# kkrt-labs/stwo-brainfuck

Measured on AMD Instinct MI355X. Metric: trace cells committed+proved/sec, higher is better.
Workload: dtype u32 (M31 / QM31 modular arithmetic)

## Files before the change

bindings/rust/bfhip_sys.rs:

```rust
#![allow(non_camel_case_types, dead_code)]
use std::ffi::{c_char, c_void};

#[repr(C)] pub struct BfhipCtx { _private: [u8; 0] }
#[repr(C)] pub struct BfhipTrace { _private: [u8; 0] }
#[repr(C)] #[derive(Clone, Copy, Default, Debug, PartialEq, Eq)] pub struct BfhipConventions { pub merkle_node_hash: u32, pub mix_u64: u32, pub logup_mask_order: u32, pub merkle_channel: u32, pub reserved: [u32; 4] }
#[repr(C)] #[derive(Clone, Copy, Debug, PartialEq, Eq)] pub struct BfhipPcsConfig { pub pow_bits: u32, pub log_blowup_factor: u32, pub log_last_layer_degree_bound: u32, pub n_queries: u32, pub reserved: [u32; 4] }
#[repr(C)] #[derive(Clone, Copy, Default, Debug, PartialEq, Eq)] pub struct BfhipCheckReport { pub component: u32, pub log_size: u32, pub n_bad_cells: u64, pub first_bad_cell: u64, pub first_bad_constraint: i32, pub first_bad_value: [u32; 4], pub bad_per_constraint: [u64; 16], pub claimed_sum: [u32; 4], pub reserved: [u32; 3] }
#[repr(C)] #[derive(Clone, Copy, Default, Debug, PartialEq, Eq)] pub struct BfhipRelationEntry { pub relation: u32, pub n_words: u32, pub tuple: [u32; 7], pub net: u32, pub n_yield: u64, pub n_use: u64, pub n_other: u64, pub first_yield_table: i32, pub first_use_table: i32, pub first_yield_row: u64, pub first_use_row: u64, pub reserved: [u32; 2] }
#[repr(C)] #[derive(Clone, Copy, Default, Debug, PartialEq, Eq)] pub struct BfhipRelationReport { pub relation: u32, pub n_words: u32, pub n_entries: u64, pub n_tuples: u64, pub n_unbalanced: u64, pub n_reported: u64, pub reserved: [u32; 2] }
#[repr(C)] #[derive(Clone, Copy, Debug)] pub struct BfhipRelationTable { pub component: i32, pub log_size: u32, pub main_rows_h: *const *const u32 }
#[repr(C)] pub struct BfhipLocalGroup { _private: [u8; 0] }
#[repr(C)] pub struct BfhipPool { _private: [u8; 0] }
#[repr(C)] #[derive(Clone, Copy, Debug)] pub struct BfhipPoolResult { pub ticket: u64, pub user_tag: u64, pub status: i32, pub worker: u32, pub flags: u32, pub log_max_rows: u32, pub proof_json: *mut c_char, pub proof_len: usize, pub error: *mut c_char, pub seconds_queued: f64, pub seconds_proving: f64, pub reserved: [u64; 2] }
#[repr(C)] #[derive(Clone, Copy, Debug)] pub struct BfhipPreflightReport { pub ran: u32, pub rejected: u32, pub n_bad_components: i32, pub n_entries: u32, pub logup_total: [u32; 4], pub components: [BfhipCheckReport; 13], pub relations: [BfhipRelationReport; 3], pub entries: [BfhipRelationEntry; 12], pub seconds: f64, pub reserved: [u64; 3] }
pub const BFHIP_TRACE_REJECTED: i32 = -3;
pub const BFHIP_JOB_CANCELLED: i32 = -2;
pub const BFHIP_POOL_MAX_OUTSTANDING: u32 = 4096;

#[link(name = "bfhip")]
extern "C" {
    pub fn bfhip_last_error() -> *const c_char;
    pub fn bfhip_device_count() -> i32;
    pub fn bfhip_device_memory(device_id: i32, free_bytes: *mut u64, total_bytes: *mut u64) -> i32;
    pub fn bfhip_ctx_create(device_id: i32, max_log_domain: u32, out: *mut *mut BfhipCtx) -> i32;
    pub fn bfhip_ctx_destroy(ctx: *mut BfhipCtx) -> i32;
    pub fn bfhip_ctx_sync(ctx: *mut BfhipCtx) -> i32;
    pub fn bfhip_ctx_set_overlap(ctx: *mut BfhipCtx, mask: u32) -> i32;
    pub fn bfhip_ctx_memory(ctx: *mut BfhipCtx, out: *mut u64) -> i32;
    pub fn bfhip_ctx_set_sync_policy(ctx: *mut BfhipCtx, blocking: i32) -> i32;
    pub fn bfhip_ctx_set_mailbox(ctx: *mut BfhipCtx, mode: i32, timeout_ms: u32, test_delay_ms: i32) -> i32;
    pub fn bfhip_ctx_set_conventions(ctx: *mut BfhipCtx, conv: *const BfhipConventions) -> i32;
    pub fn bfhip_ctx_get_conventions(ctx: *mut BfhipCtx, out: *mut BfhipConventions) -> i32;
    pub fn bfhip_ctx_set_pcs_config(ctx: *mut BfhipCtx, pcs: *const BfhipPcsConfig) -> i32;
    pub fn bfhip_ctx_get_pcs_config(ctx: *mut BfhipCtx, out: *mut BfhipPcsConfig) -> i32;
    pub fn bfhip_malloc(ctx: *mut BfhipCtx, bytes: usize, out_d: *mut *mut c_void) -> i32;
    pub fn bfhip_free(ctx: *mut BfhipCtx, ptr_d: *mut c_void) -> i32;
    pub fn bfhip_upload(ctx: *mut BfhipCtx, dst_d: *mut c_void, src_h: *const c_void, bytes: usize) -> i32;
    pub fn bfhip_download(ctx: *mut BfhipCtx, dst_h: *mut c_void, src_d: *const c_void, bytes: usize) -> i32;
    pub fn bfhip_memset_zero(ctx: *mut BfhipCtx, dst_d: *mut c_void, bytes: usize) -> i32;
    pub fn bfhip_twiddles(ctx: *mut BfhipCtx, tw_d: *mut *const u32, itw_d: *mut *const u32, root_log: *mut u32) -> i32;
    pub fn bfhip_interpolate(ctx: *mut BfhipCtx, src_cols_h: *const *mut u32, dst_cols_h: *const *mut u32, n_cols: u32, log_size: u32, replicated: i32) -> i32;
    pub fn bfhip_evaluate(ctx: *mut BfhipCtx, coeff_cols_h: *const *mut u32, dst_cols_h: *const *mut u32, n_cols: u32, log_size: u32, log_eval: u32, replicated: i32) -> i32;
    pub fn bfhip_is_first_coeffs(ctx: *mut BfhipCtx, log_min: u32, log_max: u32, dst_cols_h: *const *mut u32) -> i32;
    pub fn bfhip_broadcast16(ctx: *mut BfhipCtx, rows_d: *const u32, dst_d: *mut u32, n_rows: usize) -> i32;
    pub fn bfhip_bit_reverse(ctx: *mut BfhipCtx, src_d: *const u32, dst_d: *mut u32, log_size: u32) -> i32;
    pub fn bfhip_batch_inverse_m31(ctx: *mut BfhipCtx, src_d: *const u32, dst_d: *mut u32, n: usize) -> i32;
    pub fn bfhip_batch_inverse_qm31(ctx: *mut BfhipCtx, src_d: *const *const u32, dst_d: *const *mut u32, n: usize) -> i32;
    pub fn bfhip_accumulate(ctx: *mut BfhipCtx, dst_d: *mut u32, src_d: *const u32, n: usize) -> i32;
    pub fn bfhip_eval_at_point(ctx: *mut BfhipCtx, coeffs_d: *const u32, log_size: u32, replicated: i32, point_h: *const u32, out_h: *mut u32) -> i32;
    pub fn bfhip_merkle_commit_layer(ctx: *mut BfhipCtx, log_size: u32, prev_layer_d: *const c_void, cols_h: *const *const u32, col_shifts_h: *const u32, n_cols: u32, out_hashes_d: *mut c_void) -> i32;
    pub fn bfhip_merkle_commit_layer_poseidon252(ctx: *mut BfhipCtx, log_size: u32, prev_layer_d: *const c_void, cols_h: *const *const u32, col_shifts_h: *const u32, n_cols: u32, out_hashes_d: *mut c_void) -> i32;
    pub fn bfhip_hades_permutation(ctx: *mut BfhipCtx, in_h: *const u32, out_h: *mut u32) -> i32;
    pub fn bfhip_fold_line(ctx: *mut BfhipCtx, src_d: *const *const u32, dst_d: *const *mut u32, log_size: u32, alpha_h: *const u32) -> i32;
    pub fn bfhip_fold_circle_into_line(ctx: *mut BfhipCtx, dst_d: *const *mut u32, src_d: *const *const u32, log_size: u32, alpha_h: *const u32) -> i32;
    pub fn bfhip_fri_fold_leaf(ctx: *mut BfhipCtx, src_d: *const *const u32, quot_d: *const *const u32, dst_d: *const *mut u32, log_size: u32, alpha_h: *const u32, out_hashes_d: *mut c_void) -> i32;
    pub fn bfhip_grind(ctx: *mut BfhipCtx, digest_h: *const u8, pow_bits: u32, nonce: *mut u64) -> i32;
    pub fn bfhip_grind_poseidon252(ctx: *mut BfhipCtx, digest_h: *const u8, pow_bits: u32, start_nonce: u64, nonce: *mut u64, tried: *mut u64) -> i32;
    pub fn bfhip_gather(ctx: *mut BfhipCtx, col_d: *const u32, idx_h: *const u64, n: usize, out_h: *mut u32) -> i32;
    pub fn bfhip_component_shape(component: i32, n_main_cols: *mut u32, n_logup_cols: *mut u32, n_constraints: *mut u32) -> i32;
    pub fn bfhip_logup_generate(ctx: *mut BfhipCtx, component: i32, log_size: u32, main_rows_h: *const *const u32, lookup_h: *const u32, out_cols_h: *const *mut u32, claimed_sum_h: *mut u32) -> i32;
    pub fn bfhip_eval_constraints(ctx: *mut BfhipCtx, component: i32, log_size: u32, is_first_d: *const u32, main_lde_h: *const *const u32, main_shifts_h: *const u32, inter_lde_h: *const *const u32, inter_shifts_h: *const u32, lookup_h: *const u32, claimed_sum_h: *const u32, coeffs_h: *const u32, acc_d: *const *mut u32) -> i32;
    pub fn bfhip_check_constraints(ctx: *mut BfhipCtx, component: i32, log_size: u32, main_rows_h: *const *const u32, logup_cols_h: *const *const u32, lookup_h: *const u32, claimed_sum_h: *const u32, out: *mut BfhipCheckReport) -> i32;
    pub fn bfhip_accumulate_quotients(ctx: *mut BfhipCtx, log_size: u32, cols_h: *const *const u32, col_shifts_h: *const u32, n_cols: u32, n_samples_h: *const u32, sample_points_h: *const u32, sample_values_h: *const u32, random_coeff_h: *const u32, out_d: *const *mut u32) -> i32;
    pub fn bfhip_prove_brainfuck(ctx: *mut BfhipCtx, code: *const c_char, input_h: *const u8, n_input: usize, log_max_rows: u32, proof_json: *mut *mut c_char, proof_len: *mut usize, transcript: *mut *mut c_char, phase_seconds: *mut f64) -> i32;
    pub fn bfhip_free_host(p: *mut c_void);
    pub fn bfhip_ctx_last_proof_flags(ctx: *mut BfhipCtx, flags: *mut u32) -> i32;
    pub fn bfhip_local_group_create(count: u32, out: *mut *mut BfhipLocalGroup) -> i32;
    pub fn bfhip_local_group_destroy(group: *mut BfhipLocalGroup) -> i32;
    pub fn bfhip_ctx_join_local_group(ctx: *mut BfhipCtx, group: *mut BfhipLocalGroup, rank: u32) -> i32;
    pub fn bfhip_rccl_unique_id(id: *mut u8) -> i32;
    pub fn bfhip_ctx_join_rccl_group(ctx: *mut BfhipCtx, id: *const u8, rank: u32, count: u32) -> i32;
    pub fn bfhip_ctx_leave_group(ctx: *mut BfhipCtx) -> i32;
    pub fn bfhip_ctx_set_shard_policy(ctx: *mut BfhipCtx, policy: i32) -> i32;
    pub fn bfhip_ctx_group_stats(ctx: *mut BfhipCtx, out: *mut u64) -> i32;
    pub fn bfhip_ctx_group_times(ctx: *mut BfhipCtx, out_ms: *mut f64) -> i32;
    pub fn bfhip_ctx_group_latency(ctx: *mut BfhipCtx, reset: i32, out_us: *mut f64) -> i32;
    pub fn bfhip_rccl_exchange_raw(id: *const u8, rank: u32, count: u32, n_sends: u32, send_peer: *const u32, send_ptr: *const *mut c_void, send_bytes: *const usize, n_recvs: u32, recv_peer: *const u32, recv_ptr: *const *mut c_void, recv_bytes: *const usize, stats_out: *mut u64) -> i32;
    pub fn bfhip_rccl_selftest(ctx: *mut BfhipCtx) -> i32;
    pub fn bfhip_ctx_group_info(ctx: *mut BfhipCtx, rank: *mut u32, count: *mut u32, transport: *mut *const c_char) -> i32;
    pub fn bfhip_ctx_reuse_preprocessed(ctx: *mut BfhipCtx, on: i32) -> i32;
    pub fn bfhip_trace_create(ctx: *mut BfhipCtx, code: *const c_char, input_h: *const u8, n_input: usize, out: *mut *mut BfhipTrace, log_sizes: *mut u32, n_steps: *mut u64, main_cells: *mut u64, interaction_cells: *mut u64) -> i32;
    pub fn bfhip_trace_create_ram(ctx: *mut BfhipCtx, code: *const c_char, input_h: *const u8, n_input: usize, ram_size: usize, out: *mut *mut BfhipTrace, log_sizes: *mut u32, n_steps: *mut u64, main_cells: *mut u64, interaction_cells: *mut u64) -> i32;
    pub fn bfhip_trace_create_from_registers(ctx: *mut BfhipCtx, trace7_h: *const u32, n_rows: usize, code_words_h: *const u32, n_code: usize, out: *mut *mut BfhipTrace, log_sizes: *mut u32, main_cells: *mut u64, interaction_cells: *mut u64) -> i32;
    pub fn bfhip_trace_destroy(ctx: *mut BfhipCtx, trace: *mut BfhipTrace) -> i32;
    pub fn bfhip_ctx_set_table_builder(ctx: *mut BfhipCtx, on_gpu: i32) -> i32;
    pub fn bfhip_trace_column(ctx: *mut BfhipCtx, trace: *const BfhipTrace, component: u32, column: u32, out_h: *mut u32, cap: usize, n_rows: *mut usize) -> i32;
    pub fn bfhip_prove_trace(ctx: *mut BfhipCtx, trace: *const BfhipTrace, log_max_rows: u32, proof_json: *mut *mut c_char, proof_len: *mut usize, transcript: *mut *mut c_char, phase_seconds: *mut f64) -> i32;
    pub fn bfhip_prove_registers(ctx: *mut BfhipCtx, trace7_h: *const u32, n_rows: usize, code_words_h: *const u32, n_code: usize, log_max_rows: u32, proof_json: *mut *mut c_char, proof_len: *mut usize, transcript: *mut *mut c_char, phase_seconds: *mut f64) -> i32;
    pub fn bfhip_trace_check(ctx: *mut BfhipCtx, trace: *const BfhipTrace, lookup_h: *const u32, out: *mut BfhipCheckReport, logup_total_h: *mut u32, n_bad_components: *mut i32) -> i32;
    pub fn bfhip_relation_summary(ctx: *mut BfhipCtx, tables: *const BfhipRelationTable, n_tables: u32, out: *mut BfhipRelationReport, entries_h: *mut BfhipRelationEntry, cap_per_relation: u32) -> i32;
    pub fn bfhip_trace_relations(ctx: *mut BfhipCtx, trace: *const BfhipTrace, out: *mut BfhipRelationReport, entries_h: *mut BfhipRelationEntry, cap_per_relation: u32) -> i32;
    pub fn bfhip_ctx_set_preflight(ctx: *mut BfhipCtx, on: i32) -> i32;
    pub fn bfhip_ctx_get_preflight(ctx: *mut BfhipCtx, on: *mut i32) -> i32;
    pub fn bfhip_ctx_last_preflight(ctx: *mut BfhipCtx, out: *mut BfhipPreflightReport) -> i32;
    pub fn bfhip_format_preflight(rep: *const BfhipPreflightReport, buf: *mut c_char, cap: usize, need: *mut usize) -> i32;
    pub fn bfhip_pool_create(device_id: i32, n_in_flight: u32, max_log_domain: u32, out: *mut *mut BfhipPool) -> i32;
    pub fn bfhip_pool_destroy(pool: *mut BfhipPool) -> i32;
    pub fn bfhip_pool_size(pool: *mut BfhipPool, n_in_flight: *mut u32) -> i32;
    pub fn bfhip_pool_ctx(pool: *mut BfhipPool, i: u32, out: *mut *mut BfhipCtx) -> i32;
    pub fn bfhip_pool_set_conventions(pool: *mut BfhipPool, conv: *const BfhipConventions) -> i32;
    pub fn bfhip_pool_set_preprocessed(pool: *mut BfhipPool, mode: i32) -> i32;
    pub fn bfhip_pool_set_pcs_config(pool: *mut BfhipPool, pcs: *const BfhipPcsConfig) -> i32;
    pub fn bfhip_pool_set_preflight(pool: *mut BfhipPool, on: i32) -> i32;
    pub fn bfhip_prove_batch(pool: *mut BfhipPool, traces: *const *const BfhipTrace, n: u32, log_max_rows: u32, proofs_json: *mut *mut c_char, proof_lens: *mut usize, statuses: *mut i32, seconds: *mut f64) -> i32;
    pub fn bfhip_prove_batch_brainfuck(pool: *mut BfhipPool, codes: *const *const c_char, inputs_h: *const *const u8, n_inputs: *const usize, n: u32, log_max_rows: u32, proofs_json: *mut *mut c_char, proof_lens: *mut usize, statuses: *mut i32, seconds: *mut f64) -> i32;
    pub fn bfhip_pool_submit_trace(pool: *mut BfhipPool, trace: *const BfhipTrace, log_max_rows: u32, user_tag: u64, ticket: *mut u64) -> i32;
    pub fn bfhip_pool_submit_brainfuck(pool: *mut BfhipPool, code: *const c_char, input_h: *const u8, n_input: usize, log_max_rows: u32, user_tag: u64, ticket: *mut u64) -> i32;
    pub fn bfhip_pool_submit_registers(pool: *mut BfhipPool, trace7_h: *const u32, n_rows: usize, code_words_h: *const u32, n_code: usize, log_max_rows: u32, user_tag: u64, ticket: *mut u64) -> i32;
    pub fn bfhip_pool_wait(pool: *mut BfhipPool, timeout_ms: u32, out: *mut BfhipPoolResult) -> i32;
    pub fn bfhip_pool_outstanding(pool: *mut BfhipPool, queued: *mut u32, running: *mut u32, finished_not_taken: *mut u32) -> i32;
    pub fn bfhip_pool_cancel(pool: *mut BfhipPool, ticket: u64) -> i32;
    pub fn bfhip_verify_brainfuck(proof_json: *const c_char, proof_len: usize, log_max_rows: u32, err: *mut c_char, err_cap: usize) -> i32;
    pub fn bfhip_verify_brainfuck_conv(proof_json: *const c_char, proof_len: usize, log_max_rows: u32, conv: *const BfhipConventions, err: *mut c_char, err_cap: usize) -> i32;
    pub fn bfhip_verify_brainfuck_pcs(proof_json: *const c_char, proof_len: usize, log_max_rows: u32, conv: *const BfhipConventions, pcs: *const BfhipPcsConfig, err: *mut c_char, err_cap: usize) -> i32;
    pub fn bfhip_host_compile(code: *const c_char, out: *mut u32, cap: usize, n: *mut usize) -> i32;
    pub fn bfhip_host_run(code: *const c_char, input_h: *const u8, n_input: usize, out: *mut u8, out_cap: usize, n_out: *mut usize, trace7: *mut u32, trace_cap_rows: usize, n_rows: *mut usize) -> i32;
    pub fn bfhip_host_run_ram(code: *const c_char, input_h: *const u8, n_input: usize, ram_size: usize, out: *mut u8, out_cap: usize, n_out: *mut usize, trace7: *mut u32, trace_cap_rows: usize, n_rows: *mut usize) -> i32;
    pub fn bfhip_host_table(trace7: *const u32, n_trace: usize, code: *const u32, n_code: usize, component: i32, out_row_major: *mut u32, cap: usize, n_rows: *mut usize, n_cols: *mut usize) -> i32;
    pub fn bfhip_profile_enable(ctx: *mut BfhipCtx, mode: i32) -> i32;
    pub fn bfhip_profile_reset(ctx: *mut BfhipCtx) -> i32;
    pub fn bfhip_profile_report(ctx: *mut BfhipCtx, json: *mut *mut c_char) -> i32;
    pub fn bfhip_clock_probe(ctx: *mut BfhipCtx, seconds: f64, out: *mut f64) -> i32;
    pub fn bfhip_clock_probe_mix(ctx: *mut BfhipCtx, seconds: f64, log_nodes: u32, out: *mut f64) -> i32;
}
```

include/bfhip.h:

```cpp
#ifndef BFHIP_H
#define BFHIP_H
#include <stdint.h>
#include <stddef.h>

#ifdef __cplusplus
extern "C" {
#endif

typedef struct bfhip_ctx bfhip_ctx;
typedef struct bfhip_trace bfhip_trace;

enum { BFHIP_MERKLE_STWO_COMPRESS = 0, BFHIP_MERKLE_RFC7693 = 1 };
enum { BFHIP_MIX_U64_COMPRESS = 0, BFHIP_MIX_U64_HASH = 1 };
enum { BFHIP_LOGUP_MASK_CUR_PREV = 0, BFHIP_LOGUP_MASK_PREV_CUR = 1 };
enum { BFHIP_CHANNEL_BLAKE2S = 0, BFHIP_CHANNEL_POSEIDON252 = 1 };
typedef struct bfhip_conventions {
    uint32_t merkle_node_hash;
    uint32_t mix_u64;
    uint32_t logup_mask_order;
    uint32_t merkle_channel;
    uint32_t reserved[4];
} bfhip_conventions;

const char* bfhip_last_error(void);
int32_t bfhip_device_count(void);
int32_t bfhip_device_memory(int32_t device_id, uint64_t* free_bytes, uint64_t* total_bytes);

int32_t bfhip_ctx_create(int32_t device_id, uint32_t max_log_domain, bfhip_ctx** out);
int32_t bfhip_ctx_destroy(bfhip_ctx* ctx);
int32_t bfhip_ctx_sync(bfhip_ctx* ctx);
int32_t bfhip_ctx_set_overlap(bfhip_ctx* ctx, uint32_t mask);
int32_t bfhip_ctx_memory(bfhip_ctx* ctx, uint64_t out[4]);
int32_t bfhip_ctx_set_sync_policy(bfhip_ctx* ctx, int32_t blocking);
int32_t bfhip_ctx_set_mailbox(bfhip_ctx* ctx, int32_t mode, uint32_t timeout_ms, int32_t test_delay_ms);

int32_t bfhip_ctx_set_conventions(bfhip_ctx* ctx, const bfhip_conventions* conv);
int32_t bfhip_ctx_get_conventions(bfhip_ctx* ctx, bfhip_conventions* out);

enum { BFHIP_MAX_QUERIES = 256, BFHIP_MAX_LOG_BLOWUP = 16, BFHIP_MAX_POW_BITS = 32 };
typedef struct bfhip_pcs_config {
    uint32_t pow_bits;
    uint32_t log_blowup_factor;
    uint32_t log_last_layer_degree_bound;
    uint32_t n_queries;
    uint32_t reserved[4];
} bfhip_pcs_config;
int32_t bfhip_ctx_set_pcs_config(bfhip_ctx* ctx, const bfhip_pcs_config* pcs);
int32_t bfhip_ctx_get_pcs_config(bfhip_ctx* ctx, bfhip_pcs_config* out);

int32_t bfhip_malloc(bfhip_ctx* ctx, size_t bytes, void** out_d);
int32_t bfhip_free(bfhip_ctx* ctx, void* ptr_d);
int32_t bfhip_upload(bfhip_ctx* ctx, void* dst_d, const void* src_h, size_t bytes);
int32_t bfhip_download(bfhip_ctx* ctx, void* dst_h, const void* src_d, size_t bytes);
int32_t bfhip_memset_zero(bfhip_ctx* ctx, void* dst_d, size_t bytes);

int32_t bfhip_twiddles(bfhip_ctx* ctx, const uint32_t** tw_d, const uint32_t** itw_d, uint32_t* root_log);

int32_t bfhip_interpolate(bfhip_ctx* ctx, uint32_t* const* src_cols_h, uint32_t* const* dst_cols_h, uint32_t n_cols, uint32_t log_size, int32_t replicated);
int32_t bfhip_evaluate(bfhip_ctx* ctx, uint32_t* const* coeff_cols_h, uint32_t* const* dst_cols_h, uint32_t n_cols, uint32_t log_size, uint32_t log_eval, int32_t replicated);

int32_t bfhip_is_first_coeffs(bfhip_ctx* ctx, uint32_t log_min, uint32_t log_max, uint32_t* const* dst_cols_h);


int32_t bfhip_broadcast16(bfhip_ctx* ctx, const uint32_t* rows_d, uint32_t* dst_d, size_t n_rows);
int32_t bfhip_bit_reverse(bfhip_ctx* ctx, const uint32_t* src_d, uint32_t* dst_d, uint32_t log_size);
int32_t bfhip_batch_inverse_m31(bfhip_ctx* ctx, const uint32_t* src_d, uint32_t* dst_d, size_t n);
int32_t bfhip_batch_inverse_qm31(bfhip_ctx* ctx, const uint32_t* const src_d[4], uint32_t* const dst_d[4], size_t n);
int32_t bfhip_accumulate(bfhip_ctx* ctx, uint32_t* dst_d, const uint32_t* src_d, size_t n);
int32_t bfhip_eval_at_point(bfhip_ctx* ctx, const uint32_t* coeffs_d, uint32_t log_size, int32_t replicated, const uint32_t point_h[8], uint32_t out_h[4]);
int32_t bfhip_merkle_commit_layer(bfhip_ctx* ctx, uint32_t log_size, const void* prev_layer_d, const uint32_t* const* cols_h, const uint32_t* col_shifts_h,
                                  uint32_t n_cols, void* out_hashes_d);
int32_t bfhip_merkle_commit_layer_poseidon252(bfhip_ctx* ctx, uint32_t log_size, const void* prev_layer_d, const uint32_t* const* cols_h,
                                             const uint32_t* col_shifts_h, uint32_t n_cols, void* out_hashes_d);
int32_t bfhip_hades_permutation(bfhip_ctx* ctx, const uint32_t in_h[24], uint32_t out_h[24]);
int32_t bfhip_fold_line(bfhip_ctx* ctx, const uint32_t* const src_d[4], uint32_t* const dst_d[4], uint32_t log_size, const uint32_t alpha_h[4]);
int32_t bfhip_fold_circle_into_line(bfhip_ctx* ctx, uint32_t* const dst_d[4], const uint32_t* const src_d[4], uint32_t log_size, const uint32_t alpha_h[4]);
int32_t bfhip_fri_fold_leaf(bfhip_ctx* ctx, const uint32_t* const src_d[4], const uint32_t* const quot_d[4], uint32_t* const dst_d[4], uint32_t log_size,
                            const uint32_t alpha_h[4], void* out_hashes_d);
int32_t bfhip_grind(bfhip_ctx* ctx, const uint8_t digest_h[32], uint32_t pow_bits, uint64_t* nonce);
int32_t bfhip_grind_poseidon252(bfhip_ctx* ctx, const uint8_t digest_h[32], uint32_t pow_bits, uint64_t start_nonce,
                                uint64_t* nonce, uint64_t* tried);
int32_t bfhip_gather(bfhip_ctx* ctx, const uint32_t* col_d, const uint64_t* idx_h, size_t n, uint32_t* out_h);


int32_t bfhip_component_shape(int32_t component, uint32_t* n_main_cols, uint32_t* n_logup_cols, uint32_t* n_constraints);
int32_t bfhip_logup_generate(bfhip_ctx* ctx, int32_t component, uint32_t log_size, const uint32_t* const* main_rows_h, const uint32_t lookup_h[24],
                             uint32_t* const* out_cols_h, uint32_t claimed_sum_h[4]);
int32_t bfhip_eval_constraints(bfhip_ctx* ctx, int32_t component, uint32_t log_size, const uint32_t* is_first_d, const uint32_t* const* main_lde_h,
                               const uint32_t* main_shifts_h, const uint32_t* const* inter_lde_h, const uint32_t* inter_shifts_h, const uint32_t lookup_h[24],
                               const uint32_t claimed_sum_h[4], const uint32_t* coeffs_h, uint32_t* const acc_d[4]);
typedef struct bfhip_check_report {
    uint32_t component, log_size;
    uint64_t n_bad_cells;
    uint64_t first_bad_cell;
    int32_t  first_bad_constraint;
    uint32_t first_bad_value[4];
    uint64_t bad_per_constraint[16];
    uint32_t claimed_sum[4];
    uint32_t reserved[3];
} bfhip_check_report;
int32_t bfhip_check_constraints(bfhip_ctx* ctx, int32_t component, uint32_t log_size, const uint32_t* const* main_rows_h, const uint32_t* const* logup_cols_h,
                                const uint32_t lookup_h[24], const uint32_t claimed_sum_h[4], bfhip_check_report* out);
int32_t bfhip_accumulate_quotients(bfhip_ctx* ctx, uint32_t log_size, const uint32_t* const* cols_h, const uint32_t* col_shifts_h, uint32_t n_cols,
                                   const uint32_t* n_samples_h, const uint32_t* sample_points_h, const uint32_t* sample_values_h,
                                   const uint32_t random_coeff_h[4], uint32_t* const out_d[4]);

int32_t bfhip_prove_brainfuck(bfhip_ctx* ctx, const char* code, const uint8_t* input_h, size_t n_input, uint32_t log_max_rows,
                              char** proof_json, size_t* proof_len, char** transcript, double* phase_seconds);
void bfhip_free_host(void* p);
int32_t bfhip_ctx_last_proof_flags(bfhip_ctx* ctx, uint32_t* flags);
typedef struct bfhip_local_group bfhip_local_group;
int32_t bfhip_local_group_create(uint32_t count, bfhip_local_group** out);
int32_t bfhip_local_group_destroy(bfhip_local_group* group);
int32_t bfhip_ctx_join_local_group(bfhip_ctx* ctx, bfhip_local_group* group, uint32_t rank);
int32_t bfhip_rccl_unique_id(uint8_t id[128]);
int32_t bfhip_ctx_join_rccl_group(bfhip_ctx* ctx, const uint8_t id[128], uint32_t rank, uint32_t count);
int32_t bfhip_ctx_leave_group(bfhip_ctx* ctx);
int32_t bfhip_ctx_set_shard_policy(bfhip_ctx* ctx, int32_t policy);
int32_t bfhip_ctx_group_stats(bfhip_ctx* ctx, uint64_t out[4]);
int32_t bfhip_ctx_group_times(bfhip_ctx* ctx, double out_ms[3]);
int32_t bfhip_ctx_group_latency(bfhip_ctx* ctx, int32_t reset, double out_us[21]);
int32_t bfhip_rccl_exchange_raw(const uint8_t id[128], uint32_t rank, uint32_t count, uint32_t n_sends, const uint32_t* send_peer, void* const* send_ptr,
                                const size_t* send_bytes, uint32_t n_recvs, const uint32_t* recv_peer, void* const* recv_ptr, const size_t* recv_bytes,
                                uint64_t stats_out[4]);
int32_t bfhip_rccl_selftest(bfhip_ctx* ctx);
int32_t bfhip_ctx_group_info(bfhip_ctx* ctx, uint32_t* rank, uint32_t* count, const char** transport);

int32_t bfhip_ctx_reuse_preprocessed(bfhip_ctx* ctx, int32_t on);

int32_t bfhip_trace_create(bfhip_ctx* ctx, const char* code, const uint8_t* input_h, size_t n_input, bfhip_trace** out,
                           uint32_t log_sizes[13], uint64_t* n_steps, uint64_t* main_cells, uint64_t* interaction_cells);
int32_t bfhip_trace_create_ram(bfhip_ctx* ctx, const char* code, const uint8_t* input_h, size_t n_input, size_t ram_size, bfhip_trace** out,
                               uint32_t log_sizes[13], uint64_t* n_steps, uint64_t* main_cells, uint64_t* interaction_cells);
int32_t bfhip_trace_create_from_registers(bfhip_ctx* ctx, const uint32_t* trace7_h, size_t n_rows, const uint32_t* code_words_h, size_t n_code,
                                          bfhip_trace** out, uint32_t log_sizes[13], uint64_t* main_cells, uint64_t* interaction_cells);
int32_t bfhip_trace_destroy(bfhip_ctx* ctx, bfhip_trace* trace);
int32_t bfhip_ctx_set_table_builder(bfhip_ctx* ctx, int32_t on_gpu);
int32_t bfhip_trace_column(bfhip_ctx* ctx, const bfhip_trace* trace, uint32_t component, uint32_t column, uint32_t* out_h, size_t cap, size_t* n_rows);
int32_t bfhip_prove_trace(bfhip_ctx* ctx, const bfhip_trace* trace, uint32_t log_max_rows, char** proof_json, size_t* proof_len,
                          char** transcript, double* phase_seconds);
int32_t bfhip_prove_registers(bfhip_ctx* ctx, const uint32_t* trace7_h, size_t n_rows, const uint32_t* code_words_h, size_t n_code,
                              uint32_t log_max_rows, char** proof_json, size_t* proof_len, char** transcript, double* phase_seconds);
// ... 106 lines not shown
```

stwo-brainfuck_amd/__init__.py:

```python
import ctypes
import os
import weakref

import numpy as np

_HERE = os.path.dirname(os.path.abspath(__file__))
_LIB_PATH = os.environ.get("BFHIP_LIBRARY") or os.path.join(_HERE, "libbfhip.so")
TESTHOOKS_LIBRARY = os.path.join(_HERE, "libbfhip_testhooks.so")
_lib = None

P = (1 << 31) - 1


class BfhipError(RuntimeError):
    pass


def lib():
    global _lib
    if _lib is None:
        if not os.path.exists(_LIB_PATH):
            raise BfhipError(f"{_LIB_PATH} is missing: build it with __graft_entry__.build(); there is no CPU fallback")
        _lib = ctypes.CDLL(_LIB_PATH)
        _lib.bfhip_last_error.restype = ctypes.c_char_p
# ... 229 lines not shown
    if not getattr(check, "ran", True):
        return ["preflight: did not run"]
    if not getattr(check, "rejected", not check.ok):
        return ["preflight: ok"]
    what = []
    if check.n_bad_components:
        what.append("%d of 13 components violate their constraints" % check.n_bad_components)
    if any(check.logup_total):
        what.append("the logUp total is not zero")
    return ["TraceRejected: " + " and ".join(what)] + check.failures() + (relations.lines() if relations is not None else [])


def format_preflight(report):
    need = ctypes.c_size_t()
    rc = lib().bfhip_format_preflight(ctypes.byref(report), None, ctypes.c_size_t(0), ctypes.byref(need))
    if rc not in (0, -2):
        raise BfhipError(lib().bfhip_last_error().decode())
    buf = ctypes.create_string_buffer(need.value)
    _check(lib().bfhip_format_preflight(ctypes.byref(report), buf, ctypes.c_size_t(need.value), None))
    return buf.value.decode()


def _relation_result(call, max_entries, table_names=None):
    reps = (RelationReport * 3)()
    ents = (RelationEntry * (3 * max_entries))() if max_entries else None
    _check(call(reps, ents, max_entries))
    return RelationResult([r.as_dict() for r in reps], [ents[k * max_entries + i].as_dict() for k in range(3) for i in range(reps[k].n_reported)], table_names)


class Context:

    def __init__(self, device_id=0, max_log_domain=22):
        self._h = ctypes.c_void_p()
        _check(lib().bfhip_ctx_create(device_id, max_log_domain, ctypes.byref(self._h)))
        self.max_log_domain = max_log_domain
        _live_contexts.add(self)
        if _default_conventions != (0, 0, 0, 0):
            self.set_conventions(*_default_conventions)

    def close(self):
        if self._h:
            lib().bfhip_ctx_destroy(self._h)
            self._h = ctypes.c_void_p()

    def __del__(self):
        try:
            self.close()
        except Exception:
            pass

    def sync(self):
        _check(lib().bfhip_ctx_sync(self._h))

    def set_conventions(self, merkle_node_hash=0, mix_u64=0, logup_mask_order=0, merkle_channel=0):
        cv = Conventions(merkle_node_hash, mix_u64, logup_mask_order, merkle_channel)
        _check(lib().bfhip_ctx_set_conventions(self._h, ctypes.byref(cv)))

    def get_conventions(self):
        cv = Conventions()
        _check(lib().bfhip_ctx_get_conventions(self._h, ctypes.byref(cv)))
        return cv.merkle_node_hash, cv.mix_u64, cv.logup_mask_order, cv.merkle_channel

    def set_pcs_config(self, pcs_config=None):
        _check(lib().bfhip_ctx_set_pcs_config(self._h, _pcs_ref(pcs_config)))

    def pcs_config(self):
        out = PcsConfig()
        _check(lib().bfhip_ctx_get_pcs_config(self._h, ctypes.byref(out)))
        return out

    def set_overlap(self, mask=1):
        _check(lib().bfhip_ctx_set_overlap(self._h, int(mask)))

    def set_sync_policy(self, blocking):
        _check(lib().bfhip_ctx_set_sync_policy(self._h, 1 if blocking else 0))

    def set_mailbox(self, mode=-2, timeout_ms=0, test_delay_ms=-1):
        _check(lib().bfhip_ctx_set_mailbox(self._h, int(mode), int(timeout_ms), int(test_delay_ms)))

    def last_proof_flags(self):
        f = ctypes.c_uint32()
        _check(lib().bfhip_ctx_last_proof_flags(self._h, ctypes.byref(f)))
        return {"mailbox_order": bool(f.value & 1), "kept_preprocessed": bool(f.value & 2), "shared_preprocessed": bool(f.value & 4), "replicated_transforms": bool(f.value & 8),
                "split_gather": bool(f.value & 16), "fri_fold_leaf": bool(f.value & 32), "preflight": bool(f.value & 64)}

    def set_preflight(self, on=True):
        _check(lib().bfhip_ctx_set_preflight(self._h, 1 if on else 0))

    def preflight(self):
        on = ctypes.c_int32()
        _check(lib().bfhip_ctx_get_preflight(self._h, ctypes.byref(on)))
        return bool(on.value)

    def last_preflight_report(self):
        rep = PreflightReport()
        _check(lib().bfhip_ctx_last_preflight(self._h, ctypes.byref(rep)))
        return rep

    def last_preflight(self):
        return self.last_preflight_report().results()

    def clock_probe(self, seconds=0.6):
        out = (ctypes.c_double * 6)()
        _check(lib().bfhip_clock_probe(self._h, ctypes.c_double(seconds), out))
        return dict(zip(("ghz", "ghz_min", "ghz_max", "G_compressions_per_s", "launches", "ms_per_launch"), [float(v) for v in out]))

    def clock_probe_mix(self, seconds=0.5, log_nodes=22):
        out = (ctypes.c_double * 6)()
        _check(lib().bfhip_clock_probe_mix(self._h, ctypes.c_double(seconds), int(log_nodes), out))
        d = dict(zip(("ghz", "G_compressions_per_s", "launches", "us_per_launch", "sampler_spanned_the_window", "sampler_seconds"), [float(v) for v in out]))
        d["sampler_spanned_the_window"] = bool(d["sampler_spanned_the_window"])
        return d

    def memory(self):
        out = (ctypes.c_uint64 * 4)()
        _check(lib().bfhip_ctx_memory(self._h, out))
        return dict(zip(("arena_reserved", "arena_peak", "twiddles", "arena_in_use"), [int(v) for v in out]))

    def set_table_builder(self, on_gpu=True):
        _check(lib().bfhip_ctx_set_table_builder(self._h, int(on_gpu)))

    def join_local_group(self, group, rank):
        _check(lib().bfhip_ctx_join_local_group(self._h, group._h, rank))
        self._group = group

    def join_rccl_group(self, unique_id: bytes, rank, count):
        if len(unique_id) != 128:
            raise BfhipError("an RCCL unique id has 128 bytes")
        _check(lib().bfhip_ctx_join_rccl_group(self._h, unique_id, rank, count))

    def set_shard_policy(self, policy=-1):
        _check(lib().bfhip_ctx_set_shard_policy(self._h, int(policy)))

    def leave_group(self):
        _check(lib().bfhip_ctx_leave_group(self._h))
        self._group = None

    def group_stats(self):
        out = (ctypes.c_uint64 * 4)()
        _check(lib().bfhip_ctx_group_stats(self._h, out))
        return dict(zip(("all_gathers", "max_reduces", "exchanges", "bytes_sent"), [int(v) for v in out]))

    def group_times(self):
        out = (ctypes.c_double * 3)()
        _check(lib().bfhip_ctx_group_times(self._h, out))
        return dict(zip(("all_gather_ms", "max_reduce_ms", "exchange_ms"), [float(v) for v in out]))

    def group_latency(self, reset=False):
        out = (ctypes.c_double * 21)()
        _check(lib().bfhip_ctx_group_latency(self._h, 1 if reset else 0, out))
        res = {}
        for k, name in enumerate(("all_gather", "max_reduce", "exchange")):
            v = [float(x) for x in out[7 * k:7 * k + 7]]
            res[name] = {"count": int(v[0]), "gpu_us": {"p50": round(v[1], 1), "p90": round(v[2], 1), "max": round(v[3], 1)},
                         "host_us": {"p50": round(v[4], 1), "p90": round(v[5], 1), "max": round(v[6], 1)}}
        return res

    def group_info(self):
        r, n, t = ctypes.c_uint32(), ctypes.c_uint32(), ctypes.c_char_p()
        _check(lib().bfhip_ctx_group_info(self._h, ctypes.byref(r), ctypes.byref(n), ctypes.byref(t)))
        return r.value, n.value, (t.value or b"").decode()

    def malloc(self, nbytes):
        p = ctypes.c_void_p()
        _check(lib().bfhip_malloc(self._h, ctypes.c_size_t(nbytes), ctypes.byref(p)))
        return p.value

    def free(self, ptr):
        _check(lib().bfhip_free(self._h, ctypes.c_void_p(ptr)))

    def upload(self, arr):
        arr = np.ascontiguousarray(arr)
        ptr = self.malloc(arr.nbytes)
        _check(lib().bfhip_upload(self._h, ctypes.c_void_p(ptr), arr.ctypes.data_as(ctypes.c_void_p), ctypes.c_size_t(arr.nbytes)))
        return ptr

    def download(self, ptr, n, dtype=np.uint32):
        out = np.empty(n, dtype=dtype)
        _check(lib().bfhip_download(self._h, out.ctypes.data_as(ctypes.c_void_p), ctypes.c_void_p(ptr), ctypes.c_size_t(out.nbytes)))
        return out

    @staticmethod
    def _ptr_array(ptrs):
        return (ctypes.c_void_p * len(ptrs))(*ptrs)

    def interpolate(self, src_ptrs, dst_ptrs, log_size, replicated=False):
        _check(lib().bfhip_interpolate(self._h, self._ptr_array(src_ptrs), self._ptr_array(dst_ptrs), len(src_ptrs), log_size, int(replicated)))

    def evaluate(self, coeff_ptrs, dst_ptrs, log_size, log_eval, replicated=False):
        _check(lib().bfhip_evaluate(self._h, self._ptr_array(coeff_ptrs), self._ptr_array(dst_ptrs), len(coeff_ptrs), log_size, log_eval, int(replicated)))

    def is_first_coeffs(self, log_min, log_max, dst_ptrs):
        arr = (ctypes.c_void_p * len(dst_ptrs))(*[p or None for p in dst_ptrs])
        _check(lib().bfhip_is_first_coeffs(self._h, log_min, log_max, arr))

    def eval_at_point(self, coeff_ptr, log_size, point8, replicated=False):
        pt = (ctypes.c_uint32 * 8)(*[int(v) for v in point8])
        out = (ctypes.c_uint32 * 4)()
        _check(lib().bfhip_eval_at_point(self._h, ctypes.c_void_p(coeff_ptr), log_size, int(replicated), pt, out))
        return list(out)

    def broadcast16(self, rows_ptr, dst_ptr, n_rows):
        _check(lib().bfhip_broadcast16(self._h, ctypes.c_void_p(rows_ptr), ctypes.c_void_p(dst_ptr), ctypes.c_size_t(n_rows)))

    def bit_reverse(self, src_ptr, dst_ptr, log_size):
        _check(lib().bfhip_bit_reverse(self._h, ctypes.c_void_p(src_ptr), ctypes.c_void_p(dst_ptr), log_size))

    def batch_inverse_m31(self, src_ptr, dst_ptr, n):
        _check(lib().bfhip_batch_inverse_m31(self._h, ctypes.c_void_p(src_ptr), ctypes.c_void_p(dst_ptr), ctypes.c_size_t(n)))

    def batch_inverse_qm31(self, src_ptrs, dst_ptrs, n):
        _check(lib().bfhip_batch_inverse_qm31(self._h, self._ptr_array(src_ptrs), self._ptr_array(dst_ptrs), ctypes.c_size_t(n)))

    def accumulate(self, dst_ptr, src_ptr, n):
        _check(lib().bfhip_accumulate(self._h, ctypes.c_void_p(dst_ptr), ctypes.c_void_p(src_ptr), ctypes.c_size_t(n)))

    def merkle_commit_layer(self, log_size, prev_ptr, col_ptrs, out_ptr, col_shifts=None):
        sh = None if col_shifts is None else (ctypes.c_uint32 * len(col_shifts))(*col_shifts)
        _check(lib().bfhip_merkle_commit_layer(self._h, log_size, ctypes.c_void_p(prev_ptr) if prev_ptr else None, self._ptr_array(col_ptrs), sh, len(col_ptrs), ctypes.c_void_p(out_ptr)))

    def merkle_commit_layer_poseidon252(self, log_size, prev_ptr, col_ptrs, out_ptr, col_shifts=None):
        sh = None if col_shifts is None else (ctypes.c_uint32 * len(col_shifts))(*col_shifts)
        _check(lib().bfhip_merkle_commit_layer_poseidon252(self._h, log_size, ctypes.c_void_p(prev_ptr) if prev_ptr else None, self._ptr_array(col_ptrs), sh, len(col_ptrs), ctypes.c_void_p(out_ptr)))

    def hades_permutation(self, state3):
        words = []
        for x in state3:
            words += [(int(x) >> (32 * i)) & 0xFFFFFFFF for i in range(8)]
        out = (ctypes.c_uint32 * 24)()
        _check(lib().bfhip_hades_permutation(self._h, (ctypes.c_uint32 * 24)(*words), out))
        return [sum(int(out[8 * k + i]) << (32 * i) for i in range(8)) for k in range(3)]

    def fold_line(self, src_ptrs, dst_ptrs, log_size, alpha4):
        _check(lib().bfhip_fold_line(self._h, self._ptr_array(src_ptrs), self._ptr_array(dst_ptrs), log_size, (ctypes.c_uint32 * 4)(*[int(v) for v in alpha4])))

    def fri_fold_leaf(self, src_ptrs, quot_ptrs, dst_ptrs, log_size, alpha4, out_ptr):
        _check(lib().bfhip_fri_fold_leaf(self._h, self._ptr_array(src_ptrs) if src_ptrs is not None else None, self._ptr_array(quot_ptrs) if quot_ptrs is not None else None,
                                         self._ptr_array(dst_ptrs), log_size, (ctypes.c_uint32 * 4)(*[int(v) for v in alpha4]), ctypes.c_void_p(out_ptr)))

    def fold_circle_into_line(self, dst_ptrs, src_ptrs, log_size, alpha4):
        _check(lib().bfhip_fold_circle_into_line(self._h, self._ptr_array(dst_ptrs), self._ptr_array(src_ptrs), log_size, (ctypes.c_uint32 * 4)(*[int(v) for v in alpha4])))

    def grind(self, digest32, pow_bits):
        nonce = ctypes.c_uint64()
        _check(lib().bfhip_grind(self._h, bytes(digest32), pow_bits, ctypes.byref(nonce)))
        return nonce.value

    def grind_poseidon252(self, digest32, pow_bits, start_nonce=0, with_tried=False):
        digest32 = bytes(digest32)
        if len(digest32) != 32:
            raise ValueError("grind_poseidon252: the digest is 32 bytes")
        nonce, tried = ctypes.c_uint64(), ctypes.c_uint64()
        _check(lib().bfhip_grind_poseidon252(self._h, digest32, ctypes.c_uint32(pow_bits), ctypes.c_uint64(start_nonce), ctypes.byref(nonce), ctypes.byref(tried)))
        return (nonce.value, tried.value) if with_tried else nonce.value

    def gather(self, col_ptr, indices):
        idx = np.ascontiguousarray(indices, dtype=np.uint64)
        out = np.empty(idx.size, dtype=np.uint32)
        _check(lib().bfhip_gather(self._h, ctypes.c_void_p(col_ptr), idx.ctypes.data_as(ctypes.c_void_p), ctypes.c_size_t(idx.size), out.ctypes.data_as(ctypes.c_void_p)))
        return out

    @staticmethod
    def _u32s(values):
        values = [int(v) for v in values]
        return (ctypes.c_uint32 * len(values))(*values)

    def logup_generate(self, component, log_size, main_row_ptrs, lookup24, out_col_ptrs):
        claimed = (ctypes.c_uint32 * 4)()
        _check(lib().bfhip_logup_generate(self._h, component, log_size, self._ptr_array(main_row_ptrs), self._u32s(lookup24), self._ptr_array(out_col_ptrs), claimed))
        return list(claimed)

    def eval_constraints(self, component, log_size, is_first_ptr, main_lde_ptrs, inter_lde_ptrs, lookup24, claimed4, coeffs, acc_ptrs, main_shifts=None, inter_shifts=None):
        _check(lib().bfhip_eval_constraints(self._h, component, log_size, ctypes.c_void_p(is_first_ptr), self._ptr_array(main_lde_ptrs),
# ... 189 lines not shown
        arr = (ctypes.c_void_p * max(n, 1))(*[t._h for t in traces])
        js, lens, st, sec = self._outputs(n, want_json)
        rc = lib().bfhip_prove_batch(self._h, arr, n, log_max_rows, js, lens, st, sec)
        return self._collect(rc, n, js, lens, st, sec, want_json)

    def prove_batch_brainfuck(self, programs, log_max_rows=24, want_json=True):
        n = len(programs)
        codes = (ctypes.c_char_p * max(n, 1))(*[c.encode() for c, _ in programs])
        bufs = [ctypes.create_string_buffer(bytes(i), max(len(i), 1)) for _, i in programs]
        inputs = (ctypes.c_void_p * max(n, 1))(*[ctypes.addressof(b) for b in bufs])
        nin = (ctypes.c_size_t * max(n, 1))(*[len(i) for _, i in programs])
        js, lens, st, sec = self._outputs(n, want_json)
        rc = lib().bfhip_prove_batch_brainfuck(self._h, codes, inputs, nin, n, log_max_rows, js, lens, st, sec)
        return self._collect(rc, n, js, lens, st, sec, want_json)


PHASES = ("preprocessed", "tables_host", "main_trace", "interaction", "composition", "oods", "quotients", "fri", "decommit", "total")


def prove_brainfuck(code, input_bytes=b"", ctx=None, log_max_rows=24, with_transcript=False, with_timings=False, pcs_config=None):
    own = ctx is None
    if own:
        blowup = 1 if pcs_config is None else pcs_config.log_blowup_factor
        ctx = Context(0, max_log_domain=log_max_rows + blowup + 1)
    try:
        if pcs_config is not None:
            ctx.set_pcs_config(pcs_config)
        js, n, tr = ctypes.c_void_p(), ctypes.c_size_t(), ctypes.c_void_p()
        times = (ctypes.c_double * 10)()
        _check_proof(lib().bfhip_prove_brainfuck(ctx._h, code.encode(), input_bytes, ctypes.c_size_t(len(input_bytes)), log_max_rows,
                                                 ctypes.byref(js), ctypes.byref(n), ctypes.byref(tr) if with_transcript else None, times), ctx)
        proof = ctypes.string_at(js, n.value)
        lib().bfhip_free_host(js)
        out = [proof]
        if with_transcript:
            t = ctypes.string_at(tr).decode()
            lib().bfhip_free_host(tr)
            out.append(dict(line.split(":") for line in t.strip().split("\n")))
        if with_timings:
            out.append(dict(zip(PHASES, list(times))))
        return out[0] if len(out) == 1 else tuple(out)
    finally:
        if own:
            ctx.close()


def prove_registers(rows, code_words, ctx=None, log_max_rows=24, with_transcript=False, with_timings=False):
    own = ctx is None
    if own:
        ctx = Context(0, max_log_domain=log_max_rows + 2)
    try:
        tr = np.ascontiguousarray(rows, dtype=np.uint32).reshape(-1, 7)
        code = np.ascontiguousarray(code_words, dtype=np.uint32)
        js, n, t = ctypes.c_void_p(), ctypes.c_size_t(), ctypes.c_void_p()
        times = (ctypes.c_double * 10)()
        _check_proof(lib().bfhip_prove_registers(ctx._h, tr.ctypes.data_as(ctypes.c_void_p), ctypes.c_size_t(tr.shape[0]), code.ctypes.data_as(ctypes.c_void_p),
                                                 ctypes.c_size_t(code.size), log_max_rows, ctypes.byref(js), ctypes.byref(n),
                                                 ctypes.byref(t) if with_transcript else None, times), ctx)
        proof = ctypes.string_at(js, n.value)
        lib().bfhip_free_host(js)
        out = [proof]
        if with_transcript:
            text = ctypes.string_at(t).decode()
            lib().bfhip_free_host(t)
            out.append(dict(line.split(":") for line in text.strip().split("\n")))
        if with_timings:
            out.append(dict(zip(PHASES, list(times))))
        return out[0] if len(out) == 1 else tuple(out)
    finally:
        if own:
            ctx.close()


def verify_brainfuck(proof_json: bytes, log_max_rows=24, conventions=None, pcs_config=None):
    err = ctypes.create_string_buffer(512)
    cv = ctypes.byref(Conventions(*(_default_conventions if conventions is None else conventions)))
    rc = lib().bfhip_verify_brainfuck_pcs(proof_json, ctypes.c_size_t(len(proof_json)), log_max_rows, cv, _pcs_ref(pcs_config), err,
                                          ctypes.c_size_t(512))
    if rc < 0:
        raise BfhipError(lib().bfhip_last_error().decode())
    return rc == 0, err.value.decode()


def host_compile(code):
    out = np.zeros(2 * len(code) + 4, dtype=np.uint32)
    n = ctypes.c_size_t()
    _check(lib().bfhip_host_compile(code.encode(), out.ctypes.data_as(ctypes.c_void_p), ctypes.c_size_t(out.size), ctypes.byref(n)))
    return out[: n.value].copy()


def host_run(code, input_bytes=b"", ram_size=0):
    n_out, n_rows = ctypes.c_size_t(), ctypes.c_size_t()
    args = (code.encode(), input_bytes, ctypes.c_size_t(len(input_bytes)), ctypes.c_size_t(ram_size))
    _check(lib().bfhip_host_run_ram(*args, None, ctypes.c_size_t(0), ctypes.byref(n_out), None, ctypes.c_size_t(0), ctypes.byref(n_rows)))
    out = (ctypes.c_ubyte * max(1, n_out.value))()
    rows = np.zeros((n_rows.value, 7), dtype=np.uint32)
    _check(lib().bfhip_host_run_ram(*args, out, ctypes.c_size_t(n_out.value), ctypes.byref(n_out), rows.ctypes.data_as(ctypes.c_void_p),
                                    ctypes.c_size_t(rows.shape[0]), ctypes.byref(n_rows)))
    return bytes(out[: n_out.value]), rows


class Trace:

    def __init__(self, ctx, code, input_bytes=b"", ram_size=0):
        self.ctx = ctx
        self._h = ctypes.c_void_p()
        ls = (ctypes.c_uint32 * 13)()
        steps, mc, ic = ctypes.c_uint64(), ctypes.c_uint64(), ctypes.c_uint64()
        _check(lib().bfhip_trace_create_ram(ctx._h, code.encode(), input_bytes, ctypes.c_size_t(len(input_bytes)), ctypes.c_size_t(ram_size),
                                            ctypes.byref(self._h), ls, ctypes.byref(steps), ctypes.byref(mc), ctypes.byref(ic)))
        self.log_sizes = list(ls)
        self.n_steps, self.main_cells, self.interaction_cells = steps.value, mc.value, ic.value

    @classmethod
    def from_registers(cls, ctx, trace7, code_words):
        self = cls.__new__(cls)
        self.ctx = ctx
        self._h = ctypes.c_void_p()
        tr = np.ascontiguousarray(trace7, dtype=np.uint32).reshape(-1, 7)
        code = np.ascontiguousarray(code_words, dtype=np.uint32)
        ls = (ctypes.c_uint32 * 13)()
        mc, ic = ctypes.c_uint64(), ctypes.c_uint64()
        _check(lib().bfhip_trace_create_from_registers(ctx._h, tr.ctypes.data_as(ctypes.c_void_p), ctypes.c_size_t(tr.shape[0]), code.ctypes.data_as(ctypes.c_void_p),
                                                       ctypes.c_size_t(code.size), ctypes.byref(self._h), ls, ctypes.byref(mc), ctypes.byref(ic)))
        self.log_sizes = list(ls)
        self.n_steps, self.main_cells, self.interaction_cells = tr.shape[0], mc.value, ic.value
        return self

    @property
    def cells(self):
        return self.main_cells + self.interaction_cells

    def prove(self, log_max_rows=24, want_json=True):
        js, n = ctypes.c_void_p(), ctypes.c_size_t()
        times = (ctypes.c_double * 10)()
        _check_proof(lib().bfhip_prove_trace(self.ctx._h, self._h, log_max_rows, ctypes.byref(js) if want_json else None, ctypes.byref(n), None, times), self.ctx)
        proof = None
        if want_json:
            proof = ctypes.string_at(js, n.value)
            lib().bfhip_free_host(js)
        return proof, dict(zip(PHASES, list(times)))

    def check(self, lookup24=None):
        reps = (CheckReport * 13)()
        total = (ctypes.c_uint32 * 4)()
        n_bad = ctypes.c_int32()
        _check(lib().bfhip_trace_check(self.ctx._h, self._h, None if lookup24 is None else Context._u32s(lookup24), reps, total, ctypes.byref(n_bad)))
        res = CheckResult(r.as_dict() for r in reps)
        res.logup_total, res.n_bad_components = tuple(int(v) for v in total), n_bad.value
        return res

    def relations(self, max_entries=64):
        return _relation_result(lambda reps, ents, cap: lib().bfhip_trace_relations(self.ctx._h, self._h, reps, ents, cap), max_entries)

    def column(self, component, column):
        n = ctypes.c_size_t()
        _check(lib().bfhip_trace_column(self.ctx._h, self._h, component, column, None, ctypes.c_size_t(0), ctypes.byref(n)))
        out = np.empty(n.value, dtype=np.uint32)
        _check(lib().bfhip_trace_column(self.ctx._h, self._h, component, column, out.ctypes.data_as(ctypes.c_void_p), ctypes.c_size_t(out.size), ctypes.byref(n)))
        return out

    def close(self):
        if self._h:
            lib().bfhip_trace_destroy(self.ctx._h, self._h)
            self._h = ctypes.c_void_p()
```

stwo-brainfuck_amd/csrc/api.hip:

```cpp
#include "../../include/bfhip.h"
#include "api_guard.h"
#include "prover.h"
#include <cstdlib>
#include "host/circle.h"
#include "host/quotients.h"
#include "host/hash.h"
#include <cstdio>
#include <vector>
#include <algorithm>
#include <chrono>

using namespace bf;

static thread_local std::string g_err;
void bfhip_set_error(const std::string& s) { g_err = s; }

namespace bf {

void Ctx::ensure_aux() { for (auto& a : aux) if (!a) BF_HIP(hipStreamCreateWithFlags(&a, hipStreamNonBlocking)); }
void Ctx::ensure_side() { if (!stream2) BF_HIP(hipStreamCreateWithFlags(&stream2, hipStreamNonBlocking)); }

void Ctx::init(int dev, u32 max_log_domain, const Ctx* tables_from) {
    int n = 0;
    if (hipGetDeviceCount(&n) != hipSuccess || n == 0) throw HipError("no HIP device: the bfhip backend has no CPU fallback");
// ... 415 lines not shown
    ctx->c.overlap_user_set = true;
    return 0;
    API_CATCH
}
int32_t bfhip_ctx_memory(bfhip_ctx* ctx, uint64_t out[4]) {
    API_CTX(ctx)
    if (!out) throw HipError("null argument");
    uint64_t reserved = 0;
    for (auto& ch : ctx->c.arena.chunks) reserved += ch.size;
    out[0] = reserved; out[1] = ctx->c.arena.peak; out[2] = ctx->c.owns_tables ? (uint64_t)(2 * sizeof(u32)) << ctx->c.tw_root_log : 0;
    return 0;
    API_CATCH
}
int32_t bfhip_ctx_get_conventions(bfhip_ctx* ctx, bfhip_conventions* out) {
    API_CTX(ctx)
    if (!out) throw HipError("null argument");
    bfhip_conventions r{};
    r.merkle_node_hash = ctx->c.conv.merkle_node_hash; r.mix_u64 = ctx->c.conv.mix_u64; r.logup_mask_order = ctx->c.conv.logup_mask_order; r.merkle_channel = ctx->c.conv.merkle_channel;
    *out = r;
    return 0;
    API_CATCH
}
int32_t bfhip_ctx_sync(bfhip_ctx* ctx) { API_CTX(ctx) ctx->c.sync(); return 0; API_CATCH }

int32_t bfhip_malloc(bfhip_ctx* ctx, size_t bytes, void** out_d) { API_CTX(ctx) BF_HIP(hipSetDevice(ctx->c.device)); BF_HIP(hipMalloc(out_d, bytes ? bytes : 4)); return 0; API_CATCH }
int32_t bfhip_free(bfhip_ctx* ctx, void* p) { API_CTX(ctx) (void)ctx; BF_HIP(hipFree(p)); return 0; API_CATCH }
int32_t bfhip_upload(bfhip_ctx* ctx, void* dst_d, const void* src_h, size_t bytes) {
    API_CTX(ctx) BF_HIP(hipMemcpyAsync(dst_d, src_h, bytes, hipMemcpyHostToDevice, ctx->c.stream)); ctx->c.sync(); return 0; API_CATCH
}
int32_t bfhip_download(bfhip_ctx* ctx, void* dst_h, const void* src_d, size_t bytes) {
    API_CTX(ctx) BF_HIP(hipMemcpyAsync(dst_h, src_d, bytes, hipMemcpyDeviceToHost, ctx->c.stream)); ctx->c.sync(); return 0; API_CATCH
}
int32_t bfhip_memset_zero(bfhip_ctx* ctx, void* dst_d, size_t bytes) { API_CTX(ctx) BF_HIP(hipMemsetAsync(dst_d, 0, bytes, ctx->c.stream)); return 0; API_CATCH }

int32_t bfhip_twiddles(bfhip_ctx* ctx, const uint32_t** tw_d, const uint32_t** itw_d, uint32_t* root_log) {
    API_CTX(ctx) if (!tw_d || !itw_d || !root_log) throw HipError("null argument"); *tw_d = ctx->c.d_tw; *itw_d = ctx->c.d_itw; *root_log = ctx->c.tw_root_log; return 0; API_CATCH
}

int32_t bfhip_interpolate(bfhip_ctx* ctx, uint32_t* const* src_cols_h, uint32_t* const* dst_cols_h, uint32_t n_cols, uint32_t log_size, int32_t replicated) {
    API_CTX(ctx)
    Ctx& c = ctx->c;
    if (replicated && log_size < 4) throw HipError("replicated columns need log_size >= 4");
    if (!replicated && log_size < 3) throw HipError("circle transforms need log_size >= 3");
    if (log_size > c.tw_root_log + 1) throw HipError("log_size exceeds the context's twiddle tree");
    u32 log = replicated ? log_size - 4 : log_size;
    c.stage_checkpoint();
    StageBatch sb(c);
    auto* s = c.stage(src_cols_h, n_cols);
    auto* d = c.stage(dst_cols_h, n_cols);
    const FftJob job{(const u32* const*)s, (u32* const*)d, n_cols, log, log, !replicated};
    FftPlan plan;
    fft_plan(plan, true, &job, 1, c.d_tw, c.d_itw, c.tw_root_log);
    plan.d_groups = c.stage(plan.groups.data(), plan.groups.size());
    sb.end();
    fft_run(c.stream, plan);
    BF_HIP(hipGetLastError());
    return 0;
    API_CATCH
}

int32_t bfhip_evaluate(bfhip_ctx* ctx, uint32_t* const* coeff_cols_h, uint32_t* const* dst_cols_h, uint32_t n_cols, uint32_t log_size, uint32_t log_eval, int32_t replicated) {
    API_CTX(ctx)
    Ctx& c = ctx->c;
    if (log_eval < log_size) throw HipError("log_eval < log_size");
    if (replicated && log_size < 4) throw HipError("replicated columns need log_size >= 4");
    if (!replicated && log_eval < 3) throw HipError("circle transforms need log_eval >= 3");
    if (log_eval > c.tw_root_log + 1) throw HipError("log_eval exceeds the context's twiddle tree");
    u32 sh = replicated ? 4 : 0;
    c.stage_checkpoint();
    StageBatch sb(c);
    auto* s = c.stage(coeff_cols_h, n_cols);
    auto* d = c.stage(dst_cols_h, n_cols);
    const FftJob job{(const u32* const*)s, (u32* const*)d, n_cols, log_eval - sh, log_size - sh, !replicated};
    FftPlan plan;
    fft_plan(plan, false, &job, 1, c.d_tw, c.d_itw, c.tw_root_log);
    plan.d_groups = c.stage(plan.groups.data(), plan.groups.size());
    sb.end();
    fft_run(c.stream, plan);
    BF_HIP(hipGetLastError());
    return 0;
    API_CATCH
}


int32_t bfhip_is_first_coeffs(bfhip_ctx* ctx, uint32_t log_min, uint32_t log_max, uint32_t* const* dst_cols_h) {
    API_CTX(ctx)
    if (!dst_cols_h) throw HipError("null argument");
    if (log_min < 4 || log_max < log_min || log_max - log_min >= 28) throw HipError("is_first_coeffs: need 4 <= log_min <= log_max < log_min + 28");
    if (log_max > ctx->c.tw_root_log + 1) throw HipError("log_max exceeds the context's twiddle tree");
    IsFirstCols a{}; a.log_min = log_min; a.log_max = log_max;
    for (u32 n = log_min; n <= log_max; n++) a.ptr[n - log_min] = dst_cols_h[n - log_min];
    is_first_coeffs(ctx->c.stream, a, ctx->c.d_itw, ctx->c.tw_root_log);
    BF_HIP(hipGetLastError());
    return 0;
    API_CATCH
}
int32_t bfhip_broadcast16(bfhip_ctx* ctx, const uint32_t* rows_d, uint32_t* dst_d, size_t n_rows) {
    API_CTX(ctx) broadcast16(ctx->c.stream, rows_d, dst_d, (u32)(n_rows * 16)); BF_HIP(hipGetLastError()); return 0; API_CATCH
}
int32_t bfhip_bit_reverse(bfhip_ctx* ctx, const uint32_t* src_d, uint32_t* dst_d, uint32_t log_size) {
    API_CTX(ctx) if (src_d == dst_d) throw HipError("bit_reverse is out of place"); bit_reverse(ctx->c.stream, src_d, dst_d, log_size); BF_HIP(hipGetLastError()); return 0; API_CATCH
}
int32_t bfhip_batch_inverse_m31(bfhip_ctx* ctx, const uint32_t* src_d, uint32_t* dst_d, size_t n) {
    API_CTX(ctx) batch_inverse_m31(ctx->c.stream, src_d, dst_d, (u32)n); BF_HIP(hipGetLastError()); return 0; API_CATCH
}
int32_t bfhip_batch_inverse_qm31(bfhip_ctx* ctx, const uint32_t* const src_d[4], uint32_t* const dst_d[4], size_t n) {
    API_CTX(ctx) batch_inverse_qm31(ctx->c.stream, src_d, dst_d, (u32)n); BF_HIP(hipGetLastError()); return 0; API_CATCH
}
int32_t bfhip_accumulate(bfhip_ctx* ctx, uint32_t* dst_d, const uint32_t* src_d, size_t n) {
    API_CTX(ctx) accumulate(ctx->c.stream, dst_d, src_d, (u32)n); BF_HIP(hipGetLastError()); return 0; API_CATCH
}
int32_t bfhip_eval_at_point(bfhip_ctx* ctx, const uint32_t* coeffs_d, uint32_t log_size, int32_t replicated, const uint32_t point_h[8], uint32_t out_h[4]) {
    API_CTX(ctx)
    Ctx& c = ctx->c;
    if (replicated && log_size < 4) throw HipError("replicated columns need log_size >= 4");
    c.stage_checkpoint();
    uint4 factors[32];
    Q31 x = q_make(point_h[0], point_h[1], point_h[2], point_h[3]);
    factors[0] = make_uint4(point_h[4], point_h[5], point_h[6], point_h[7]);
    for (u32 b = 1; b < 32; b++) { factors[b] = make_uint4(x.a.a, x.a.b, x.b.a, x.b.b); Q31 s = q_mul(x, x); x = q_subm(q_add(s, s), 1); }
    EvalJob job{coeffs_d, replicated ? log_size - 4 : log_size, 0, replicated ? 4u : 0u, 0};
    const EvalJob* dj = c.stage(&job, 1);
    const uint4* df = c.stage(factors, 32);
    u32 nchunks = job.log_n > 12 ? 1u << (job.log_n - 12) : 1u;
    uint4* partials = nullptr; uint4* dout = nullptr;
    BF_HIP(hipMalloc((void**)&partials, sizeof(uint4) * (nchunks + 1)));
    dout = partials + nchunks;
    eval_at_points(c.stream, dj, 1, nchunks, df, partials, dout);
    uint4 r;
    hipError_t e = hipMemcpyAsync(&r, dout, sizeof(uint4), hipMemcpyDeviceToHost, c.stream);
    if (e == hipSuccess) e = hipStreamSynchronize(c.stream);
    (void)hipFree(partials);
    BF_HIP(e);
    out_h[0] = r.x; out_h[1] = r.y; out_h[2] = r.z; out_h[3] = r.w;
    return 0;
    API_CATCH
}
int32_t bfhip_merkle_commit_layer(bfhip_ctx* ctx, uint32_t log_size, const void* prev_layer_d, const uint32_t* const* cols_h, const uint32_t* col_shifts_h,
                                  uint32_t n_cols, void* out_hashes_d) {
    API_CTX(ctx)
    Ctx& c = ctx->c;
    c.stage_checkpoint();
    std::vector<ColDesc> d(n_cols);
    for (u32 k = 0; k < n_cols; k++) d[k] = ColDesc{cols_h[k], col_shifts_h ? col_shifts_h[k] : 0u, 0};
    const ColDesc* dd = n_cols ? c.stage(d.data(), n_cols) : nullptr;
    merkle_layer(c.stream, out_hashes_d, prev_layer_d, dd, n_cols, log_size, 0.0, 0, 0, c.conv.merkle_node_hash);
    BF_HIP(hipGetLastError());
    return 0;
    API_CATCH
}
int32_t bfhip_merkle_commit_layer_poseidon252(bfhip_ctx* ctx, uint32_t log_size, const void* prev_layer_d, const uint32_t* const* cols_h, const uint32_t* col_shifts_h,
                                             uint32_t n_cols, void* out_hashes_d) {
    API_CTX(ctx)
    Ctx& c = ctx->c;
    c.stage_checkpoint();
    std::vector<ColDesc> d(n_cols);
    for (u32 k = 0; k < n_cols; k++) d[k] = ColDesc{cols_h[k], col_shifts_h ? col_shifts_h[k] : 0u, 0};
    const ColDesc* dd = n_cols ? c.stage(d.data(), n_cols) : nullptr;
    merkle_layer_poseidon(c.stream, out_hashes_d, prev_layer_d, dd, n_cols, log_size);
    BF_HIP(hipGetLastError());
    return 0;
    API_CATCH
}
int32_t bfhip_hades_permutation(bfhip_ctx* ctx, const uint32_t in_h[24], uint32_t out_h[24]) {
    API_CTX(ctx)
    Ctx& c = ctx->c;
// ... 378 lines not shown
```

stwo-brainfuck_amd/csrc/fft.hip:

```cpp
#include "kernels.h"
#include <cstdio>
#include <cstdlib>
#include <stdexcept>
#include <algorithm>
#include <vector>
#include <mutex>
#include <set>
#include <string>

namespace bf {

static constexpr int TILE_LOG = 12;
static constexpr int TILE = 1 << TILE_LOG;
static constexpr int CHUNK_LOG = 5;
static constexpr int STRIDED_K = TILE_LOG - CHUNK_LOG;
static constexpr int FFT_THREADS = 256;
__device__ __forceinline__ u32 scale_shift(u32 scale) { return (u32)__builtin_ctz(scale); }

__device__ __forceinline__ void point_of_index(u32 idx, const uint2* __restrict__ tlo, const uint2* __restrict__ thi, u32& x, u32& y) {
    uint2 a = tlo[idx & 0xffffu], b = thi[(idx >> 16) & 0x7fffu];
    x = m_sub(m_mul(a.x, b.x), m_mul(a.y, b.y));
    y = m_add(m_mul(a.x, b.y), m_mul(a.y, b.x));
}

__global__ void k_gen_twiddles(u32* __restrict__ tw, u32* __restrict__ itw, u32 R, const uint2* __restrict__ tlo, const uint2* __restrict__ thi) {
    u32 g = blockIdx.x * blockDim.x + threadIdx.x;
    u32 total = 1u << R;
    if (g >= total) return;
    if (g == total - 1) { tw[g] = 1; itw[g] = 1; return; }
    u32 j = __clz(~(g << (32 - R)));
    u32 off = total - (1u << (R - j));
    u32 k = g - off;
    u32 bits = R - 1 - j;
    u32 init = (1u << (31 - R - 2)) << j, step = (1u << (31 - R)) << j;
    u32 idx = (init + step * bit_rev(k, bits)) & 0x7fffffffu;
    u32 x, y;
    point_of_index(idx, tlo, thi, x, y);
    tw[g] = x;
    itw[g] = m_inv(x);
}

__global__ void __launch_bounds__(256) k_is_first_coeffs(IsFirstCols a, const u32* __restrict__ itw, u32 tw_total) {
    const u32 u = blockIdx.x * blockDim.x + threadIdx.x + (1u << (a.log_min - 4));
    if (u >= (1u << (a.log_max - 3))) return;
    const u32 n = 35u - __clz(u);
    u32* __restrict__ dst = a.ptr[n - a.log_min];
    if (!dst) return;
    const u32 jhi = u - (1u << (n - 4));
    auto t = [&](u32 i) -> u32 { return i == 0 ? itw[tw_total - (1u << (n - 1)) + 1] : itw[tw_total - (1u << (n - i))]; };
    u32 v[16];
    v[0] = m_inv_pow2(n);
    for (u32 i = 4; i < n; i++) if ((jhi >> (i - 4)) & 1) v[0] = m_mul(v[0], t(i));
#pragma unroll
    for (u32 b = 0; b < 4; b++) {
        const u32 tb = t(b);
#pragma unroll
        for (u32 e = 0; e < (1u << b); e++) v[e + (1u << b)] = m_mul(v[e], tb);
    }
    uint4* o = reinterpret_cast<uint4*>(dst + 16 * (size_t)jhi);
#pragma unroll
    for (int q = 0; q < 4; q++) o[q] = make_uint4(v[4 * q], v[4 * q + 1], v[4 * q + 2], v[4 * q + 3]);
}
void is_first_coeffs(hipStream_t stream, const IsFirstCols& a, const u32* itw, u32 tw_root_log) {
    if (a.log_min < 4 || a.log_max < a.log_min || a.log_max - a.log_min >= 28 || a.log_max > tw_root_log + 1) throw std::runtime_error("is_first_coeffs: unsupported sizes");
    const u32 lanes = (1u << (a.log_max - 3)) - (1u << (a.log_min - 4));
    hipLaunchKernelGGL(k_is_first_coeffs, dim3((lanes + 255) / 256), dim3(256), 0, stream, a, itw, 1u << tw_root_log);
}

enum { K_TILE12 = 0, K_STRIDED5 = 1, K_STRIDED6 = 2, K_PASS = 3, K_TINY = 4, K_STRIDED_K8 = 5, K_STRIDED_K9 = 6, K_STRIDED_K10 = 7, K_KINDS = 8 };
struct BlockOfGroup { u32 g, tile, by; };
template <bool INV> __device__ __forceinline__ void fft_tiny_body(const PassArgs& a, const BlockOfGroup& bg);
__device__ __forceinline__ BlockOfGroup find_group(const PassArgs* __restrict__ groups, u32 ngroups) {
    u32 g = 0;
    while (g + 1 < ngroups && groups[g + 1].block0 <= blockIdx.x) g++;
    const u32 local = blockIdx.x - groups[g].block0, gx = groups[g].grid_x;
    return {g, local % gx, local / gx};
}
__device__ __forceinline__ const u32* layer_table(const PassArgs& a, u32 layer) {
    u32 eff = a.circle ? layer : layer + 1;
    u32 lg = a.circle ? a.log : a.log + 1;
    u32 len = 1u << (lg - 1 - eff);
    return a.tw + (a.tw_total - 2 * len);
}

template <bool INV>
__device__ __forceinline__ void fft_pass_body(const PassArgs& a, const BlockOfGroup& bg, u32* __restrict__ s_val, u32* __restrict__ s_tw) {
    const u32 t = threadIdx.x;
    const u32 lo = a.lo, k = a.k;
    const u32 c = lo == 0 ? 0 : CHUNK_LOG;
    const u32 tile_log = lo == 0 ? a.tile_log : k + c;
    const u32 tile_n = 1u << tile_log;
    const u32 kt = tile_log - c;
    const u32 tile = bg.tile;
    const u32 n_lhi_log = lo - c;
    const u32 H = lo ? (tile >> n_lhi_log) : 0, Lhi = lo ? (tile & ((1u << n_lhi_log) - 1)) : 0;
    const u32 base = lo ? ((H << (lo + k)) | (Lhi << c)) : (tile << tile_log);

    for (u32 e = t; e < (1u << kt) - (1u << (kt - k)); e += FFT_THREADS) {
        u32 j = __clz(~((e) << (32 - kt)));
        u32 off = (1u << kt) - (1u << (kt - j));
        u32 q = e - off;
        u32 gl = lo + j;
        u32 hbase = lo ? (H << (kt - 1 - j)) : (tile << (kt - 1 - j));
        u32 v;
        if (a.circle && gl == 0) {
            const u32* l0 = layer_table(a, 1);
            u32 h = hbase + q;
            u32 x = l0[(h >> 2) * 2], y = l0[(h >> 2) * 2 + 1];
            u32 sel = h & 3;
            v = sel == 0 ? y : sel == 1 ? m_neg(y) : sel == 2 ? m_neg(x) : x;
        } else {
            v = layer_table(a, gl)[hbase + q];
        }
        s_tw[e] = v;
    }

    const u32 col0 = bg.by * a.cols_per_block;
    const u32 col1 = min(a.ncols, col0 + a.cols_per_block);
    for (u32 col = col0; col < col1; col++) {
        g_cu32p src = as_global(a.src[col]);
        g_u32p dst = as_global(a.dst[col]);
        __syncthreads();
        for (u32 e4 = t * 4; e4 < tile_n; e4 += 4 * FFT_THREADS) {
            u32 gidx = lo ? (base | ((e4 >> c) << lo) | (e4 & ((1u << c) - 1))) : (base + e4);
            uint4 v = a.src_mask < 3u ? make_uint4(src[0], a.src_mask ? src[1] : 0u, 0u, 0u) : ld16(src + (gidx & a.src_mask));
            *reinterpret_cast<uint4*>(&s_val[e4]) = v;
        }
        __syncthreads();
        const u32 nb = tile_n >> 1;
        if (INV) {
            for (u32 j = 0; j < k; j++) {
                u32 dist = 1u << (j + c);
                u32 toff = (1u << kt) - (1u << (kt - j));
                for (u32 b = t; b < nb; b += FFT_THREADS) {
                    u32 i0 = ((b >> (j + c)) << (j + c + 1)) | (b & (dist - 1));
                    u32 tw = s_tw[toff + (b >> (j + c))];
                    u32 v0 = s_val[i0], v1 = s_val[i0 + dist];
                    s_val[i0] = m_add(v0, v1);
                    s_val[i0 + dist] = m_mul(m_sub(v0, v1), tw);
                }
                __syncthreads();
            }
        } else {
            for (int j = (int)k - 1; j >= 0; j--) {
                u32 dist = 1u << (j + c);
                u32 toff = (1u << kt) - (1u << (kt - j));
                for (u32 b = t; b < nb; b += FFT_THREADS) {
                    u32 i0 = ((b >> (j + c)) << (j + c + 1)) | (b & (dist - 1));
                    u32 tw = s_tw[toff + (b >> (j + c))];
                    u32 v0 = s_val[i0], v1 = m_mul(s_val[i0 + dist], tw);
                    s_val[i0] = m_add(v0, v1);
                    s_val[i0 + dist] = m_sub(v0, v1);
// ... 171 lines not shown
    else if (k == 11) fft_tile12_body<INV, 11>(a, bg, s_val, s_tw);
    else if (k == 10) fft_tile12_body<INV, 10>(a, bg, s_val, s_tw);
    else if (k == 9) fft_tile12_body<INV, 9>(a, bg, s_val, s_tw);
    else fft_tile12_body<INV, 0>(a, bg, s_val, s_tw);
}

template <bool INV, int CL>
__global__ void __launch_bounds__(4 << CL, 3) k_fft_strided7(const PassArgs* __restrict__ groups, u32 ngroups) {
    const BlockOfGroup bg = find_group(groups, ngroups);
    const PassArgs a = groups[bg.g];
    constexpr u32 C = 1u << CL, NT = 4u << CL;
    __shared__ __attribute__((aligned(16))) u32 s_val[128 * C];
    __shared__ u32 s_tw[128];
    const u32 t = threadIdx.x, lo = a.lo, tile = bg.tile;
    const u32 n_lhi_log = lo - CL;
    const u32 H = tile >> n_lhi_log, Lhi = tile & ((1u << n_lhi_log) - 1);
    const u32 base = (H << (lo + 7)) | (Lhi << CL);
    if (t < 127) {
        u32 j = __clz(~(t << 25));
        u32 q = t - (128u - (128u >> j));
        s_tw[t] = 2u * layer_table(a, lo + j)[(H << (6 - j)) + q];
    }
    auto TW = [&](u32 layer, u32 idx) -> u32 { return s_tw[128u - (128u >> layer) + idx]; };
    const u32 col0 = bg.by * a.cols_per_block, col1 = min(a.ncols, col0 + a.cols_per_block);
    const u32 l4 = 4 * (t & (C / 4 - 1)), r4 = t >> (CL - 2);
    for (u32 col = col0; col < col1; col++) {
        g_cu32p src = as_global(a.src[col]);
        g_u32p dst = as_global(a.dst[col]);
        __syncthreads();
        auto wide_stage = [&](u32 (&r)[8][4]) {
#pragma unroll
            for (int s = 0; s < 3; s++) {
                const int jl = INV ? s : 2 - s;
#pragma unroll
                for (int b = 0; b < 4; b++) {
                    const int q0 = ((b >> jl) << (jl + 1)) | (b & ((1 << jl) - 1));
                    u32 w = TW(jl, (8 * r4 + q0) >> (jl + 1));
#pragma unroll
                    for (int j = 0; j < 4; j++) bfly<INV>(r[q0][j], r[q0 | (1 << jl)][j], w);
                }
            }
        };
        auto narrow_task = [&](u32 id, bool from_global, bool to_global) {
            u32 l = id & (C - 1), mlow = id >> CL;
            u32 v[16];
#pragma unroll
            for (int e = 0; e < 16; e++) {
                u32 m = 8 * e + mlow;
                v[e] = from_global ? __builtin_nontemporal_load(src + ((base | (m << lo) | l) & a.src_mask)) : s_val[C * m + l];
            }
            radix16<INV>(v, 4, [&](int jl, int pe) -> u32 { return TW(3 + jl, pe); });
#pragma unroll
            for (int e = 0; e < 16; e++) {
                u32 m = 8 * e + mlow;
                if (to_global) __builtin_nontemporal_store((INV && a.scale != 1) ? m_mul_pow2(v[e], scale_shift(a.scale)) : v[e], dst + (base | (m << lo) | l));
                else s_val[C * m + l] = v[e];
            }
        };
        if (INV) {
            u32 r[8][4];
#pragma unroll
            for (int q = 0; q < 8; q++) { uint4 v = ld16_stream(src + ((base | ((8 * r4 + q) << lo) | l4) & a.src_mask)); r[q][0] = v.x; r[q][1] = v.y; r[q][2] = v.z; r[q][3] = v.w; }
            wide_stage(r);
#pragma unroll
            for (int q = 0; q < 8; q++) *reinterpret_cast<uint4*>(&s_val[C * (8 * r4 + q) + l4]) = make_uint4(r[q][0], r[q][1], r[q][2], r[q][3]);
            __syncthreads();
            narrow_task(t, false, true);
            narrow_task(t + NT, false, true);
        } else {
            narrow_task(t, true, false);
            __builtin_amdgcn_sched_barrier(0);
            narrow_task(t + NT, true, false);
            __syncthreads();
            u32 r[8][4];
#pragma unroll
            for (int q = 0; q < 8; q++) { uint4 v = *reinterpret_cast<uint4*>(&s_val[C * (8 * r4 + q) + l4]); r[q][0] = v.x; r[q][1] = v.y; r[q][2] = v.z; r[q][3] = v.w; }
            wide_stage(r);
#pragma unroll
            for (int q = 0; q < 8; q++) st16(dst + (base | ((8 * r4 + q) << lo) | l4), make_uint4(r[q][0], r[q][1], r[q][2], r[q][3]));
        }
    }
}

template <bool INV, class TW> __device__ __forceinline__ void radix16_range(u32 (&v)[16], int jl_lo, TW tw) {
#pragma unroll
    for (int s = 0; s < 4; s++) {
        const int jl = INV ? s : 3 - s;
        if (jl >= jl_lo) {
#pragma unroll
            for (int b = 0; b < 8; b++) {
                const int e0 = ((b >> jl) << (jl + 1)) | (b & ((1 << jl) - 1));
                bfly<INV>(v[e0], v[e0 | (1 << jl)], tw(jl, e0 >> (jl + 1)));
            }
        }
    }
}
template <bool INV, int K, int CL>
__global__ void __launch_bounds__((1 << (K + CL)) / 32) k_fft_stridedK(const PassArgs* __restrict__ groups, u32 ngroups) {
    constexpr u32 C = 1u << CL, ROWS = 1u << K, CELLS = ROWS * C, NT = CELLS / 32;
    constexpr int NR = (K + 3) / 4;
    const BlockOfGroup bg = find_group(groups, ngroups);
    const PassArgs a = groups[bg.g];
    __shared__ __attribute__((aligned(16))) u32 s_val[CELLS];
    __shared__ u32 s_tw[ROWS];
    const u32 t = threadIdx.x, lo = a.lo, tile = bg.tile;
    const u32 n_lhi_log = lo - CL;
    const u32 H = tile >> n_lhi_log, Lhi = tile & ((1u << n_lhi_log) - 1);
    const u32 base = (H << (lo + K)) | (Lhi << CL);
    for (u32 e = t; e < ROWS - 1; e += NT) {
        const u32 j = __clz(~(e << (32 - K)));
        const u32 q = e - (ROWS - (ROWS >> j));
        s_tw[e] = 2u * layer_table(a, lo + j)[(H << (K - 1 - j)) + q];
    }
    auto TW = [&](u32 layer, u32 idx) -> u32 { return s_tw[ROWS - (ROWS >> layer) + idx]; };
    const u32 col0 = bg.by * a.cols_per_block, col1 = min(a.ncols, col0 + a.cols_per_block);
    for (u32 col = col0; col < col1; col++) {
        g_cu32p src = as_global(a.src[col]);
        g_u32p dst = as_global(a.dst[col]);
        __syncthreads();
#pragma unroll
        for (u32 i = 0; i < 8; i++) {
            const u32 idx = 4 * (t + NT * i), m = idx >> CL, l = idx & (C - 1);
            const uint4 v = ld16_stream(src + ((base | (m << lo) | l) & a.src_mask));
            *reinterpret_cast<uint4*>(&s_val[idx]) = v;
        }
        __syncthreads();
#pragma unroll
        for (int rr = 0; rr < NR; rr++) {
            const int r = INV ? rr : NR - 1 - rr;
            const int b = (4 * r + 4 <= K) ? 4 * r : K - 4;
            const int jl_lo = 4 * r - b;
#pragma unroll
            for (u32 g2 = 0; g2 < 2; g2++) {
                const u32 id = t + NT * g2, l = id & (C - 1), rest = id >> CL;
                const u32 rest_lo = rest & ((1u << b) - 1), rest_hi = rest >> b;
                const u32 m0 = (rest_hi << (b + 4)) | rest_lo;
                u32 v[16];
#pragma unroll
                for (int e = 0; e < 16; e++) v[e] = s_val[((m0 | ((u32)e << b)) << CL) | l];
                radix16_range<INV>(v, jl_lo, [&](int jl, int pe) -> u32 { return TW(b + jl, (rest_hi << (3 - jl)) + pe); });
#pragma unroll
                for (int e = 0; e < 16; e++) s_val[((m0 | ((u32)e << b)) << CL) | l] = v[e];
            }
            __syncthreads();
        }
#pragma unroll
        for (u32 i = 0; i < 8; i++) {
            const u32 idx = 4 * (t + NT * i), m = idx >> CL, l = idx & (C - 1);
            uint4 v = *reinterpret_cast<uint4*>(&s_val[idx]);
            if (INV && a.scale != 1) { const u32 sk = scale_shift(a.scale); v.x = m_mul_pow2(v.x, sk); v.y = m_mul_pow2(v.y, sk); v.z = m_mul_pow2(v.z, sk); v.w = m_mul_pow2(v.w, sk); }
            st16(dst + (base | (m << lo) | l), v);
        }
    }
}

template <bool INV>
__device__ __forceinline__ void fft_tiny_body(const PassArgs& a, const BlockOfGroup& bg) {
    const u32 n = 1u << a.log, wave = threadIdx.x >> 6, lane = threadIdx.x & 63u, i = lane & (n - 1);
    const u32 col = (bg.tile * (blockDim.x >> 6) + wave) * (64u >> a.log) + (lane >> a.log);
    const bool act = col < a.ncols;
    u32 v = act ? a.src[col][i & a.src_mask] : 0u;
    u32 tw[5];
#pragma unroll
    for (u32 j = 0; j < 5; j++) {
        tw[j] = 1u;
        if (j < a.k) {
            const u32 h = i >> (j + 1);
            if (a.circle && j == 0) {
                const u32* l0 = layer_table(a, 1);
                const u32 x = l0[(h >> 2) * 2], y = l0[(h >> 2) * 2 + 1], sel = h & 3;
                tw[j] = sel == 0 ? y : sel == 1 ? m_neg(y) : sel == 2 ? m_neg(x) : x;
            } else tw[j] = layer_table(a, j)[h];
        }
    }
#pragma unroll
    for (u32 jj = 0; jj < 5; jj++) {
        if (jj >= a.k) break;
        const u32 j = INV ? jj : a.k - 1 - jj;
        const u32 other = (u32)__shfl_xor((int)v, 1 << j);
        const bool hi = (i >> j) & 1u;
        const u32 x = hi ? other : v, y = hi ? v : other;
        u32 t = 0;
#pragma unroll
        for (u32 q = 0; q < 5; q++) if (q == j) t = tw[q];
        if (INV) v = hi ? m_mul(m_sub(x, y), t) : m_add(x, y);
        else { const u32 w = m_mul(y, t); v = hi ? m_sub(x, w) : m_add(x, w); }
    }
    if (act) a.dst[col][i] = INV ? m_mul(v, a.scale) : v;
}
template <bool INV>
__global__ void __launch_bounds__(256) k_fft_tiny(const PassArgs* __restrict__ groups, u32 ngroups) {
    const BlockOfGroup bg = find_group(groups, ngroups);
    const PassArgs a = groups[bg.g];
    fft_tiny_body<INV>(a, bg);
}


void fft_plan(FftPlan& plan, bool inverse, const FftJob* jobs, size_t njobs, const u32* tw, const u32* itw, u32 tw_root_log) {
    plan.inverse = inverse; plan.groups.clear(); plan.launches.clear(); plan.d_groups = nullptr;
    struct Item { int pi, kind; PassArgs a; double bytes, alg; bool single = false; double bfly() const { return 0.5 * a.ncols * (double)(1u << a.log) * a.k; } };
    std::vector<Item> items;
    int max_np = 0;
    for (size_t ji = 0; ji < njobs; ji++) {
        const FftJob& job = jobs[ji];
        const u32 ncols = job.ncols, log = job.log, src_log = job.src_log;
        if (ncols == 0) continue;
        PassArgs a{};
        a.ncols = ncols; a.log = log; a.circle = job.circle ? 1 : 0; a.tw = inverse ? itw : tw; a.tw_total = 1u << tw_root_log; a.scale = 1;
        const u32 nl = inverse ? log : (log > 5 && src_log < 2) ? 2u : src_log;
        if (log <= 5) {
            a.dst = job.d_dst; a.src = job.d_src; a.src_mask = (1u << src_log) - 1; a.lo = 0; a.k = nl;
            a.scale = inverse ? m_inv(1u << log) : 1;
            a.grid_x = (ncols + (256u >> log) - 1) / (256u >> log); a.cols_per_block = 1;
            items.push_back({0, K_TINY, a, 0.0, 0.0, true});
            max_np = std::max(max_np, 1);
            continue;
        }
        if (log >= 12 && nl >= 6) {
            u32 ns = nl > 12 ? (nl - 12 + 6) / 7 : 0;
            u32 k0 = nl - 7 * ns;
            static const bool two_pass = [] { const char* v = getenv("BFHIP_FFT_TWO_PASS"); return !v || v[0] != '0'; }();
            const u32 big_k = (two_pass && nl >= 20 && nl <= 22) ? nl - 12 : 0;
            if (big_k) { ns = 1; k0 = 12; }
            int np = 1 + (int)ns;
            max_np = std::max(max_np, np);
            const double alg = 4.0 * ncols * ((double)(1u << src_log) + (double)(1u << log)) / np;
            for (int pi = 0; pi < np; pi++) {
                int p = inverse ? pi : np - 1 - pi;
                bool first = pi == 0, last = pi == np - 1;
                a.src = first ? job.d_src : (const u32* const*)job.d_dst;
                a.dst = job.d_dst;
                a.src_mask = first ? ((1u << src_log) - 1) : 0xffffffffu;
                a.scale = (inverse && last) ? m_inv(1u << log) : 1;
                u32 ntiles = 1u << (log - 12);
                u32 cpb = ncols;
                while (cpb > 1 && (u64)ntiles * ((ncols + cpb - 1) / cpb) < 2048) cpb = (cpb + 1) / 2;
                a.cols_per_block = cpb;
                const u32 gy = (ncols + cpb - 1) / cpb;
                const double bytes = 8.0 * ncols * (double)(1u << log);
                if (p == 0) {
                    a.lo = 0; a.k = k0; a.tile_log = 12; a.grid_x = ntiles;
                    PassArgs b = a; b.block0 = gy;
                    items.push_back({pi, K_TILE12, b, bytes, alg});
                } else if (big_k) {
                    a.lo = 12; a.k = big_k;
                    const u32 cl = big_k == 10 ? 4 : 5;
                    PassArgs b = a; b.grid_x = 1u << (log - big_k - cl); b.block0 = gy;
                    items.push_back({pi, big_k == 8 ? K_STRIDED_K8 : big_k == 9 ? K_STRIDED_K9 : K_STRIDED_K10, b, bytes, alg});
                } else {
                    a.lo = k0 + 7 * (p - 1); a.k = 7;
#ifndef BF_STRIDED_WIDE_MIN_LOG
#define BF_STRIDED_WIDE_MIN_LOG 20
#endif
                    const bool wide = a.lo >= 6 && log >= BF_STRIDED_WIDE_MIN_LOG;
                    PassArgs b = a; b.grid_x = wide ? ntiles / 2 : ntiles; b.block0 = gy;
                    items.push_back({pi, wide ? K_STRIDED6 : K_STRIDED5, b, bytes, alg});
                }
            }
            continue;
        }
        u32 bounds[8]; int np = 0;
        bounds[0] = 0;
        a.tile_log = log < (u32)TILE_LOG ? log : (u32)TILE_LOG;
        u32 k0 = nl < a.tile_log ? nl : a.tile_log;
        bounds[++np] = k0;
        while (bounds[np] < nl) {
            u32 rem = nl - bounds[np];
            u32 passes_left = (rem + STRIDED_K - 1) / STRIDED_K;
            u32 kk = (rem + passes_left - 1) / passes_left;
            bounds[np + 1] = bounds[np] + kk; np++;
        }
        max_np = std::max(max_np, np);
        const double alg = 4.0 * ncols * ((double)(1u << src_log) + (double)(1u << log)) / np;
        for (int pi = 0; pi < np; pi++) {
            int p = inverse ? pi : np - 1 - pi;
            bool first = pi == 0, last = pi == np - 1;
            a.lo = bounds[p]; a.k = bounds[p + 1] - bounds[p];
            u32 tl = a.lo == 0 ? a.tile_log : a.k + CHUNK_LOG;
            u32 ntiles = 1u << (log - tl);
            a.src = first ? job.d_src : (const u32* const*)job.d_dst;
            a.dst = job.d_dst;
            a.src_mask = first ? ((1u << src_log) - 1) : 0xffffffffu;
            a.scale = (inverse && last) ? m_inv(1u << log) : 1;
            u32 cpb = 1;
            while ((u64)ntiles * ((ncols + cpb - 1) / cpb) > 8192 && cpb < ncols) cpb *= 2;
            a.cols_per_block = cpb;
            PassArgs b = a; b.grid_x = ntiles; b.block0 = (ncols + cpb - 1) / cpb;
            items.push_back({pi, K_PASS, b, 8.0 * ncols * (double)(1u << log), alg, np == 1 && log < (u32)TILE_LOG});
        }
    }
    {
        static const bool fuse = [] { const char* v = getenv("BFHIP_FFT_FUSE_SMALL"); return !v || v[0] != '0'; }();
        int host_pi = -1;
        for (auto& it : items) if (it.kind == K_TILE12 && (host_pi < 0 || it.pi < host_pi)) host_pi = it.pi;
        if (fuse && host_pi >= 0)
            for (auto& it : items)
                if (it.single && (it.kind == K_PASS || it.kind == K_TINY)) { it.a.kind = (u32)it.kind; it.kind = K_TILE12; it.pi = host_pi; }
    }
    for (int pi = 0; pi < max_np; pi++)
        for (int kind = 0; kind < K_KINDS; kind++) {
            FftLaunch L{}; L.kind = kind; L.first_group = (u32)plan.groups.size();
            u32 blocks = 0;
            for (auto& it : items) {
                if (it.pi != pi || it.kind != kind) continue;
                PassArgs a = it.a;
                const u32 gy = (kind == K_TINY || a.kind == K_TINY) ? 1u : a.block0;
                a.block0 = blocks; blocks += a.grid_x * gy;
                plan.groups.push_back(a);
                L.bytes += it.bytes; L.alg += it.alg; L.bfly += it.bfly();
            }
            L.ngroups = (u32)plan.groups.size() - L.first_group; L.total_blocks = blocks;
            if (L.ngroups) plan.launches.push_back(L);
        }
}

static const char* fft_prof_name(const char* base, const FftLaunch& L) {
    static const bool detail = [] { const char* v = getenv("BFHIP_FFT_PROF_DETAIL"); return v && v[0] == '1'; }();
    if (!detail) return base;
    static std::mutex mu; static std::set<std::string> names;
    std::lock_guard<std::mutex> g(mu);
    return names.insert(std::string(base) + "/b" + std::to_string(L.total_blocks) + "/g" + std::to_string(L.ngroups)).first->c_str();
}

void fft_run(hipStream_t stream, const FftPlan& plan) {
    if (plan.launches.empty()) return;
    if (!plan.d_groups) throw std::runtime_error("fft_run: the plan's group table has not been staged");
    const bool inverse = plan.inverse;
    for (const FftLaunch& L : plan.launches) {
        const PassArgs* g = plan.d_groups + L.first_group;
        const dim3 grid(L.total_blocks);
        switch (L.kind) {
            case K_TILE12: {
                ProfScope ps(stream, fft_prof_name(inverse ? "k_fft_tile12<true>" : "k_fft_tile12<false>", L), L.bytes, L.alg, false, L.bfly);
                static const u32 generic = [] { const char* v = getenv("BFHIP_FFT_TILE12_GENERIC"); return (v && v[0] == '1') ? 1u : 0u; }();
                if (inverse) hipLaunchKernelGGL(k_fft_tile12<true>, grid, dim3(256), 0, stream, g, L.ngroups, generic);
                else hipLaunchKernelGGL(k_fft_tile12<false>, grid, dim3(256), 0, stream, g, L.ngroups, generic);
                break; }
            case K_STRIDED5: {
                ProfScope ps(stream, fft_prof_name(inverse ? "k_fft_strided7<true>" : "k_fft_strided7<false>", L), L.bytes, L.alg, false, L.bfly);
                if (inverse) hipLaunchKernelGGL((k_fft_strided7<true, 5>), grid, dim3(128), 0, stream, g, L.ngroups);
                else hipLaunchKernelGGL((k_fft_strided7<false, 5>), grid, dim3(128), 0, stream, g, L.ngroups);
                break; }
            case K_STRIDED6: {
                ProfScope ps(stream, fft_prof_name(inverse ? "k_fft_strided7<true>" : "k_fft_strided7<false>", L), L.bytes, L.alg, false, L.bfly);
                if (inverse) hipLaunchKernelGGL((k_fft_strided7<true, 6>), grid, dim3(256), 0, stream, g, L.ngroups);
                else hipLaunchKernelGGL((k_fft_strided7<false, 6>), grid, dim3(256), 0, stream, g, L.ngroups);
                break; }
            case K_STRIDED_K8: {
                ProfScope ps(stream, fft_prof_name(inverse ? "k_fft_stridedK<true>" : "k_fft_stridedK<false>", L), L.bytes, L.alg, false, L.bfly);
                if (inverse) hipLaunchKernelGGL((k_fft_stridedK<true, 8, 5>), grid, dim3(256), 0, stream, g, L.ngroups);
                else hipLaunchKernelGGL((k_fft_stridedK<false, 8, 5>), grid, dim3(256), 0, stream, g, L.ngroups);
                break; }
            case K_STRIDED_K9: {
                ProfScope ps(stream, fft_prof_name(inverse ? "k_fft_stridedK<true>" : "k_fft_stridedK<false>", L), L.bytes, L.alg, false, L.bfly);
                if (inverse) hipLaunchKernelGGL((k_fft_stridedK<true, 9, 5>), grid, dim3(512), 0, stream, g, L.ngroups);
                else hipLaunchKernelGGL((k_fft_stridedK<false, 9, 5>), grid, dim3(512), 0, stream, g, L.ngroups);
                break; }
            case K_STRIDED_K10: {
                ProfScope ps(stream, fft_prof_name(inverse ? "k_fft_stridedK<true>" : "k_fft_stridedK<false>", L), L.bytes, L.alg, false, L.bfly);
                if (inverse) hipLaunchKernelGGL((k_fft_stridedK<true, 10, 4>), grid, dim3(512), 0, stream, g, L.ngroups);
                else hipLaunchKernelGGL((k_fft_stridedK<false, 10, 4>), grid, dim3(512), 0, stream, g, L.ngroups);
                break; }
            case K_PASS: {
                ProfScope ps(stream, fft_prof_name(inverse ? "k_fft_pass<true>" : "k_fft_pass<false>", L), L.bytes, L.alg, false, L.bfly);
                if (inverse) hipLaunchKernelGGL(k_fft_pass<true>, grid, dim3(FFT_THREADS), 0, stream, g, L.ngroups);
                else hipLaunchKernelGGL(k_fft_pass<false>, grid, dim3(FFT_THREADS), 0, stream, g, L.ngroups);
                break; }
            default:
                if (inverse) hipLaunchKernelGGL(k_fft_tiny<true>, grid, dim3(256), 0, stream, g, L.ngroups);
                else hipLaunchKernelGGL(k_fft_tiny<false>, grid, dim3(256), 0, stream, g, L.ngroups);
        }
    }
}

void gen_twiddles(hipStream_t stream, u32* d_tw, u32* d_itw, u32 R, const uint2* d_tlo, const uint2* d_thi) {
    u32 total = 1u << R;
    hipLaunchKernelGGL(k_gen_twiddles, dim3((total + 255) / 256), dim3(256), 0, stream, d_tw, d_itw, R, d_tlo, d_thi);
}

}
```

stwo-brainfuck_amd/csrc/kernels.h:

```cpp
#pragma once
#include <hip/hip_runtime.h>
#include "m31.h"
#include "air.h"
#include <string>
#include <vector>

struct bfhip_trace;

namespace bf {

struct ColDesc { const u32* ptr; u32 shift; u32 pad_; };

int prof_mode(hipStream_t s);
void prof_enable(hipStream_t s, int mode);
void prof_run_begin(hipStream_t s, const char* name);
void prof_run_end(hipStream_t s);
void prof_begin(hipStream_t s, const char* name, double bytes, double units, double aux = 0.0);
void prof_end(hipStream_t s);
void prof_reset(hipStream_t s);
std::string prof_report_json(const hipStream_t* streams, int n);
void prof_forget(hipStream_t s);
struct ProfScope {
    hipStream_t s; bool on;
    ProfScope(hipStream_t s_, const char* name, double bytes, double units = 0.0, bool dominant = false, double aux = 0.0) : s(s_) {
        int m = prof_mode(s);
        on = m == 1 || (m == 2 && dominant);
        if (on) prof_begin(s, name, bytes, units, aux);
    }
    ~ProfScope() { if (on) prof_end(s); }
};

#if defined(__HIPCC__)
#define BF_GLOBAL __attribute__((address_space(1)))
typedef u32 bf_u32x4 __attribute__((ext_vector_type(4)));
typedef BF_GLOBAL u32* g_u32p;
typedef const BF_GLOBAL u32* g_cu32p;
__device__ __forceinline__ g_cu32p as_global(const u32* p) { return (g_cu32p)(unsigned long long)p; }
__device__ __forceinline__ g_u32p as_global(u32* p) { return (g_u32p)(unsigned long long)p; }
__device__ __forceinline__ uint4 ld16(g_cu32p p) { bf_u32x4 v = *(const BF_GLOBAL bf_u32x4*)p; return make_uint4(v.x, v.y, v.z, v.w); }
__device__ __forceinline__ uint4 ld16_stream(g_cu32p p) { bf_u32x4 v = __builtin_nontemporal_load((const BF_GLOBAL bf_u32x4*)p); return make_uint4(v.x, v.y, v.z, v.w); }
__device__ __forceinline__ void st16(g_u32p p, uint4 v) { bf_u32x4 w = {v.x, v.y, v.z, v.w}; __builtin_nontemporal_store(w, (BF_GLOBAL bf_u32x4*)p); }
#define BF_CONSTANT __attribute__((address_space(4)))
template <class T> __device__ __forceinline__ T ld_constant(const T* p) {
    static_assert(sizeof(T) % 4 == 0 && alignof(T) >= 4, "word-sized parameter blocks only");
    T out;
    const BF_CONSTANT u32* s = (const BF_CONSTANT u32*)(unsigned long long)p;
#pragma unroll
    for (u32 i = 0; i < sizeof(T) / 4; i++) reinterpret_cast<u32*>(&out)[i] = s[i];
    return out;
}
__device__ __forceinline__ u32 ld_col(const ColDesc& d, u32 i) {
    const u32 byte_off = (i >> d.shift) << 2;
    return *(g_cu32p)((const BF_GLOBAL char*)(unsigned long long)d.ptr + byte_off);
}
#endif

void gen_twiddles(hipStream_t stream, u32* d_tw, u32* d_itw, u32 R, const uint2* d_tlo, const uint2* d_thi);
struct FftJob { const u32* const* d_src; u32* const* d_dst; u32 ncols, log, src_log; bool circle; };
struct PassArgs {
    u32* const* dst;
    const u32* const* src;
    u32 ncols, cols_per_block;
    u32 log;
    u32 lo, k;
    u32 tile_log;
    u32 src_mask;
    u32 circle;
    u32 scale;
    u32 tw_total;
    const u32* tw;
    u32 block0, grid_x;
    u32 kind;
};
struct FftLaunch { int kind; u32 first_group, ngroups, total_blocks; double bytes, alg, bfly; };
struct FftPlan { bool inverse = false; std::vector<PassArgs> groups; std::vector<FftLaunch> launches; const PassArgs* d_groups = nullptr; };
void fft_plan(FftPlan& plan, bool inverse, const FftJob* jobs, size_t njobs, const u32* tw, const u32* itw, u32 tw_root_log);
void fft_run(hipStream_t stream, const FftPlan& plan);

struct IsFirstCols { u32* ptr[28]; u32 log_min, log_max; };
void is_first_coeffs(hipStream_t stream, const IsFirstCols& a, const u32* itw, u32 tw_root_log);

void merkle_layer(hipStream_t stream, void* out, const void* prev, const ColDesc* d_cols, u32 ncols, u32 log, double col_bytes, u32 out_shift, u32 prev_shift,
                  u32 node_conv, u32 first = 0, u32 count = 0);
struct MerkleTreeDesc { uint4* layers[32]; u32 shifts[32]; u32 col_off[32]; const ColDesc* cols; u32 n_cols, max_log; };
static constexpr u32 MERKLE_SUBTREE_ROOT_LEVEL = 9;
void merkle_subtree(hipStream_t stream, const MerkleTreeDesc& tree, u32 hi, u32 node_conv, double bytes, double compressions);
void merkle_subtree_share(hipStream_t stream, const MerkleTreeDesc& tree, u32 hi, u32 stop, u32 lo, u32 wg0, u32 n_wg, u32 node_conv, double bytes, double compressions);
void merkle_top(hipStream_t stream, const MerkleTreeDesc& tree, u32 top_hi, u32 node_conv, u32* d_chan, u32* d_alpha8, u32* d_root_copy, double bytes, double compressions,
                u32* d_stamp = nullptr, u32 stamp_value = 0);
struct FriTailLayer {
    u32* ev[4];
    const u32* quot[4];
    uint4* tree[11];
};
struct FriTailArgs {
    u32 n_layers, top_log;
    u32 alpha_idx, root_idx;
    u32* ev_last[4];
    u32* chan; u32* alpha; u32* roots;
    const u32* itw; u32 tw_total, rfc;
    FriTailLayer layer[10];
};
void fri_tail(hipStream_t stream, const FriTailArgs* d_args, double bytes, double compressions);
struct FriLayerArgs {
    const u32* src[4]; const u32* quot[4]; u32* dst[4]; uint4* tree[18];
    const u32* alpha8; const u32* itw; u32 tw_total, log, rfc, pad_;
    u32* counter; u32* chan; u32* alpha_out; u32* root_out;
};
void fri_layer(hipStream_t stream, const FriLayerArgs& a);
enum FriFoldMode : int { FF_LINE = 0, FF_LINE_CIRCLE = 1, FF_CIRCLE = 2 };
struct FriFoldLeafArgs { const u32* src[4]; const u32* quot[4]; u32* dst[4]; const u32* alpha8; const u32* itw; u32 tw_total, log; };
void fri_fold_leaf(hipStream_t stream, void* out, const FriFoldLeafArgs& a, int mode, u32 node_conv);
void grind_span(hipStream_t stream, const u32* d_digest, u64 base, u32 span, u32 pow_bits, unsigned long long* d_best, u32 mix_u64_conv);
void clock_probe_launch(hipStream_t stream, uint4* d_stamps, u32* d_sink, u32 blocks, u32 iters);
void clock_sampler_launch(hipStream_t stream, uint4* d_out, const u32* d_stop_alias, unsigned long long max_ticks);
void fill_mix(hipStream_t stream, u32* p, size_t n);
void channel_mix_root_draw(hipStream_t stream, u32* d_chan, const u32* d_root, u32* d_alpha8, u32* d_root_copy);

void merkle_layer_poseidon(hipStream_t stream, void* out, const void* prev, const ColDesc* d_cols, u32 ncols, u32 log, u32 out_shift = 0, u32 prev_shift = 0,
                           u32 first = 0, u32 count = 0);
void hades_once(hipStream_t stream, const u32* d_in24, u32* d_out24);
void grind_poseidon_span(hipStream_t stream, const u32* d_digest, u64 base, u32 span, u32 pow_bits, unsigned long long* d_best);

struct ConstraintLaunch {
    const u32* is_first; ColDesc trace[13]; ColDesc inter[12]; u32* acc[4]; Q31 coeff[12]; Lookups el; Q31 total_sum; u32 denom_inv[2]; u32 log_size;
    u32 overwrite;
    u32 row0, n_rows;
    const u32* inter_prev[4];
};
void eval_constraints(hipStream_t stream, int comp, const ConstraintLaunch* d_args, u32 log_size, u32 n_rows = 0, u32 group_rows = 0);
u32 constraint_group_rows(const ConstraintLaunch& L, int comp);
struct ConstraintClass { u32 n_comps, block0, group_rows, pad_; u32 comp[13]; u32 pad2_[3]; };
struct ConstraintBatch { u32 n_classes, total_blocks, pad_[2]; ConstraintClass cls[13]; };
void constraint_batch_init(ConstraintBatch& b, const ConstraintLaunch* launches, u32 n);
void eval_constraints_batch(hipStream_t stream, const ConstraintBatch* d_batch, const ConstraintBatch& h_batch, const ConstraintLaunch* d_args);
struct LogupLaunch {
    const u32* cols[13];
    u32* out_rep[8];
    u32* out_last[4];
    void* vrow; void* wloc; void* totals; void* claimed;
    Lookups el; u32 log_rows; int comp;
};
struct LogupItem { const u32* cols[13]; u32* out_rep[8]; u32* out_last[4]; uint4* vrow; uint4* wloc; uint4* totals; uint4* claimed; u32 log_rows; int comp; u32 nb; u32 pad_; };
struct LogupBatch { Lookups el; u32 n; u32 rows_blk0[14], scan_blk0[14], last_blk0[14]; u32 pad_; LogupItem item[13]; };
void logup_batch_init(LogupBatch& b, const Lookups& el, const LogupLaunch* L, u32 n);
void logup_batch_run(hipStream_t stream, const LogupBatch* d_batch, const LogupBatch& h_batch);
void broadcast16(hipStream_t stream, const u32* d_rows, u32* d_out, u32 n_cells);

struct CheckReportDev { u64 n_bad_cells, first_bad_cell; u64 bad_per_constraint[16]; u32 first_bad_constraint; u32 first_bad_value[4]; u32 pad_[3]; };
struct CheckLaunch { ColDesc trace[13]; ColDesc inter[12]; Lookups el; Q31 total_sum; u32 log_size; u32 pad_; CheckReportDev* report; };
void check_constraints_launch(hipStream_t stream, int comp, const CheckLaunch* d_args, u32 log_size);
struct CheckReadback { CheckReportDev report[N_COMPONENTS]; uint4 claimed[N_COMPONENTS]; uint4 total; };
struct CheckBatch { u32 blk0[N_COMPONENTS + 1]; u32 pad_[2]; CheckReadback* out; };
void check_batch_init(CheckBatch& b, const u32 log_sizes[N_COMPONENTS], CheckReadback* d_out);
void check_batch_run(hipStream_t stream, const CheckBatch* d_batch, const CheckBatch& h_batch, const CheckLaunch* d_launches);
// ... 35 lines not shown
```

stwo-brainfuck_amd/csrc/prover.h:

```cpp
#pragma once
#include "../../include/bfhip.h"
#include "ctx.h"
#include "host/circle.h"
#include "host/quotients.h"
#include "host/proof.h"
#include <chrono>
#include <functional>
#include <map>
#include <string>
#include <vector>

namespace bf {

void build_tables_device(Ctx& c, const std::vector<u32> trace7_soa[7], u32 n, const std::vector<u32>& code, const std::function<u32*(size_t)>& alloc,
                         std::vector<std::vector<u32*>>& cols_out, u32 log_sizes_out[13]);
void build_tables_device(Ctx& c, const TraceSoA& t, const std::vector<u32>& code, const std::function<u32*(size_t)>& alloc,
                         std::vector<std::vector<u32*>>& cols_out, u32 log_sizes_out[13]);

static constexpr u32 OWNER_ALL = 0xFFFFFFFFu;

struct DCol {
    u32* ptr = nullptr; u32 log_size = 0; u32 shift = 0;
    u32 lc = 0;
    bool sliced() const { return lc != 0; }
    size_t stored() const { return size_t(1) << (log_size - shift - lc); }
    ColDesc desc() const { return ColDesc{ptr, shift, 0}; }
    bool mine(u64 cell, u32 rank) const { return lc == 0 || (cell >> (log_size - lc)) == rank; }
};
struct DevMerkle { std::vector<u32*> layers; std::vector<u32> shifts; u32 max_log = 0; Hash32 root; int band_lo = 0, band_hi = -1; std::vector<DCol> cols; };
struct DTree { std::vector<DCol> polys, evals, prev; std::vector<u32> owner; DevMerkle mk; };
struct DSecure {
    u32* c[4]; u32 log_size; u32 lc = 0;
    bool mine(u64 cell, u32 rank) const { return lc == 0 || (cell >> (log_size - lc)) == rank; }
};

struct Gather {
    std::vector<GatherReq> reqs;
    u32 n_words = 0;
    size_t add(const u32* base, u64 idx, bool mine = true) { reqs.push_back({mine ? base : nullptr, idx, n_words, 1u}); n_words += 1; return n_words - 1; }
    size_t add_hash(const u32* layer, u64 node_slot, bool mine) { reqs.push_back({mine ? layer : nullptr, node_slot * 8, n_words, 8u}); n_words += 8; return n_words - 8; }
    size_t add_col(const DCol& col, u64 cell, u32 rank) { return add(col.ptr, cell >> col.shift, col.mine(cell, rank)); }
    std::vector<u32> run(Ctx& c, int stamp_slot = -1);
};

struct TraceInput {
    std::vector<std::vector<DCol>> rows;
    u32 log_sizes[N_COMPONENTS];
    u64 n_steps = 0, main_cells = 0, interaction_cells = 0;
    std::vector<u32*> owned;
    void release() { for (u32* p : owned) (void)hipFree(p); owned.clear(); rows.clear(); }
};

struct PreprocessedCache {
    bool enabled = false, valid = false, replicate = false; u32 lmr = 0, node_conv = 0, channel = 0, log_blowup = 0, shard_rank = 0, shard_count = 1; DTree tree; Arena keep;
    bool matches(const Ctx& c, u32 log_max_rows) const {
        return enabled && valid && lmr == log_max_rows && node_conv == c.conv.merkle_node_hash && channel == c.conv.merkle_channel && log_blowup == c.pcs.log_blowup &&
               shard_rank == c.shard.rank && shard_count == c.shard.count && replicate == (c.shard.count > 1 && c.shard_replicate);
    }
};

struct SharedPreprocessed {
    bool valid = false; u32 lmr = 0, node_conv = 0, channel = 0, log_blowup = 0;
    DTree tree;
    hipEvent_t ready = nullptr;
    const Hash32* pinned_root = nullptr;
    u32 root_slot = 0;
    bool matches(const Ctx& c, u32 log_max_rows) const {
        return valid && lmr == log_max_rows && node_conv == c.conv.merkle_node_hash && channel == c.conv.merkle_channel && log_blowup == c.pcs.log_blowup &&
               c.shard.count == 1;
    }
};

inline CheckReportDev check_report_init() { CheckReportDev r{}; r.first_bad_cell = ~u64(0); r.first_bad_constraint = 0xffffffffu; return r; }
inline void check_report_fill(bfhip_check_report& out, const CheckReportDev& r, int component, u32 log_size, Q31 claimed) {
    out = bfhip_check_report{};
    out.component = (u32)component; out.log_size = log_size;
    out.n_bad_cells = r.n_bad_cells; out.first_bad_cell = r.first_bad_cell; out.first_bad_constraint = (int32_t)r.first_bad_constraint;
    for (int w = 0; w < 4; w++) out.first_bad_value[w] = r.first_bad_value[w];
    for (int j = 0; j < 16; j++) out.bad_per_constraint[j] = r.bad_per_constraint[j];
    out.claimed_sum[0] = claimed.a.a; out.claimed_sum[1] = claimed.a.b; out.claimed_sum[2] = claimed.b.a; out.claimed_sum[3] = claimed.b.b;
}
inline CheckLaunch check_launch_of(int component, u32 log_size, const u32* const* main_rows, const u32* const* logup_cols, const Lookups& el, Q31 total_sum,
                                   CheckReportDev* d_report) {
    CheckLaunch L{};
    const u32 n_inter = 4 * n_logup_cols(component);
    for (u32 j = 0; j < n_main_cols(component); j++) L.trace[j] = ColDesc{main_rows[j], LOG_N_LANES, 0};
    for (u32 j = 0; j < n_inter; j++) L.inter[j] = ColDesc{logup_cols[j], j + 4 < n_inter ? LOG_N_LANES : 0u, 0};
    L.el = el; L.total_sum = total_sum; L.log_size = log_size; L.report = d_report;
    return L;
}
inline Lookups default_check_lookups() {
    Lookups el;
    Channel ch;
    { Q31 z, a; ch.draw_two_felts(z, a); el.memory = make_lookup(z, a); }
    { Q31 z, a; ch.draw_two_felts(z, a); el.instruction = make_lookup(z, a); }
    { Q31 z, a; ch.draw_two_felts(z, a); el.processor = make_lookup(z, a); }
    return el;
}

inline void sync_both(Ctx& c) { c.sync(); if (c.stream2) BF_HIP(hipStreamSynchronize(c.stream2)); for (auto a : c.aux) if (a) BF_HIP(hipStreamSynchronize(a)); }

struct PhaseTimes { double preprocessed = 0, main_trace = 0, interaction = 0, composition = 0, oods = 0, quotients = 0, fri = 0, decommit = 0, tables = 0, total = 0; };

struct HipProver {
    Ctx& c;
    PcsConfig cfg;
    u32 log_max_rows;
    Channel ch;
    PhaseTimes tm;
    std::string transcript;
    bool want_transcript = false;

    HipProver(Ctx& ctx, u32 lmr) : c(ctx), cfg(ctx.pcs), log_max_rows(lmr) {}

    void tap(const char* name);
    static double now() { return std::chrono::duration<double>(std::chrono::steady_clock::now().time_since_epoch()).count(); }
    std::vector<std::pair<const char*, double>> host_marks;
    bool trace_host = [] { const char* v = getenv("BFHIP_TRACE_HOST"); return v && (v[0] == '1' || v[0] == '2'); }();
    bool trace_host_mean = [] { const char* v = getenv("BFHIP_TRACE_HOST"); return v && v[0] == '2'; }();
    double mark_t0 = 0;
    void mark(const char* label) { if (trace_host) host_marks.push_back({label, (now() - mark_t0) * 1e6}); }
    void print_marks();
    void check_config() const;
    BrainfuckProof prove(const TraceInput& in) { return prove([&]() -> const TraceInput& { return in; }); }
    BrainfuckProof prove(const std::function<const TraceInput&()>& get_input);
    void preflight(const TraceInput& in);

    FftPlan fft_prepare(bool inverse, const std::vector<DCol>& src, const std::vector<DCol>& dst);
    void fft_launch(const FftPlan& plan);
    void fft_cols(bool inverse, const std::vector<DCol>& src, const std::vector<DCol>& dst);
    template <class F> void stage_blocks(Mailbox* mbx, F&& f) {
        if (mbx) { mbx->begin(); f(); mbx->arm(); }
        else { StageBatch sb(c); f(); sb.end(); }
    }

    struct ChannelStep { u32* chan; u32* alpha8; u32* root_copy; };
    struct MerklePlan {
        DevMerkle mk; std::vector<DCol> cols; std::vector<size_t> off; std::vector<double> bytes; size_t n_all = 0;
        const ColDesc* d_all = nullptr; MerkleTreeDesc tree{}; bool poseidon = false;
        u32 fused_top = 0, sub_hi = 0;
        double top_bytes = 0, top_comp = 0, sub_bytes = 0, sub_comp = 0;
        int band_fuse_hi = -1; u32 band_fuse_r = 0; double band_bytes = 0, band_comp = 0;
        bool folded_leaves = false; FriFoldLeafArgs fold{}; int fold_mode = -1;
    };
    MerklePlan merkle_plan(const std::vector<DCol>& cols_in, bool folded_leaves = false);
    struct LevelWait { int level; hipEvent_t ev; };
    DevMerkle merkle_run(MerklePlan& p, Hash32* pinned_root = nullptr, bool no_readback = false, const ChannelStep* step = nullptr, const std::vector<LevelWait>* waits = nullptr,
                         int stamp_slot = -1, bool* stamped = nullptr);
    DevMerkle merkle_commit(const std::vector<DCol>& cols_in, Hash32* pinned_root = nullptr, bool no_readback = false, const ChannelStep* step = nullptr);

    static constexpr u32 SLICE_MIN_LOG_PER_RANK = 14;
    static constexpr u32 SHARE_MIN_LOG_PER_RANK = 14;
    bool sharded() const { return c.shard.count > 1; }
    u32 lc() const { return c.shard.log_count; }
    bool slice_log(u32 log) const { return sharded() && log >= lc() + SLICE_MIN_LOG_PER_RANK; }
    bool replicate() const { return sharded() && c.shard_replicate; }
    bool transforms_here(u32 owner) const { return owner == OWNER_ALL || owner == c.shard.rank || replicate(); }
    bool slice_col(u32 log, u32 shift) const { return sharded() && log >= shift + lc() + SLICE_MIN_LOG_PER_RANK; }
    size_t slice_cells(u32 log) const { return size_t(1) << (log - lc()); }
    size_t slice_first(u32 log) const { return (size_t)c.shard.rank << (log - lc()); }
    u32* alloc_slice(u32 log, u32 shift = 0);
    std::vector<u32> assign_owners(const std::vector<DCol>& polys, u32 log_blowup) const;
    void commit_tree(DTree& t, Hash32* pinned_root = nullptr, bool with_prev = false);
    void commit_tree_overlapped(DTree& t, Hash32* pinned_root, const std::vector<DCol>* interp_src = nullptr, int stamp_slot = -1);
    static void upload_trace(Ctx& c, const std::vector<Registers>& vm_trace, const std::vector<u32>& code, TraceInput& in, bool use_arena = false, bool on_gpu = true);
    static void upload_registers(Ctx& c, const u32* trace7_h, size_t n_rows, const u32* code_words_h, size_t n_code, TraceInput& in, bool use_arena, bool with_place);
    void build_preprocessed(DTree& tree, Hash32* pinned_root);
    void build_shared_preprocessed(SharedPreprocessed& sp);

    struct CompositionPlan {
        std::vector<ConstraintLaunch> launches; std::vector<DSecure> acc; std::vector<bool> have; u32 total = 0, max_log = 0;
        ConstraintLaunch* h_staged = nullptr;
    };
    CompositionPlan composition_prepare(std::vector<DTree>& trees, const BrainfuckProof& bp, const size_t* main_off, const size_t* inter_off, const Lookups& el);
    static void composition_challenge_fields(const BrainfuckProof& bp, u32 total, Q31 random_coeff, ConstraintLaunch* launches);
    void composition_fill(const BrainfuckProof& bp, CompositionPlan& cp, Q31 random_coeff);
    void compute_composition(std::vector<DTree>& trees, const BrainfuckProof& bp, CompositionPlan& cp, Q31 random_coeff, Mailbox* mbx = nullptr);
    struct SamplePlan { std::vector<EvalJob> jobs; u32 partial_off = 0, n_all = 0; };
    SamplePlan sample_prepare(const std::vector<DTree>& trees, const std::vector<std::vector<std::vector<u32>>>& mask);
    static void sample_factors(const std::vector<PtQ>& points, uint4* factors);
    struct SampleRun { uint4* h_factors = nullptr; uint4* d_out = nullptr; };
    SampleRun sample_launch(const SamplePlan& sp, const std::vector<PtQ>& points, Mailbox* mbx);
    const uint4* sample_results() const { return reinterpret_cast<const uint4*>(c.h_small + 4096); }
    void sample_unpack(const std::vector<DTree>& trees, const std::vector<std::vector<std::vector<u32>>>& mask, const uint4* out, u32 n_all, StarkProof& pf);
    void sample(const std::vector<DTree>& trees, const std::vector<std::vector<std::vector<u32>>>& mask, const std::vector<PtQ>& points, StarkProof& pf, const SamplePlan& sp);
    struct QuotientGroup {
        u32 log = 0; std::vector<ColDesc> descs; std::vector<ColSamples> cols; std::vector<std::pair<size_t, size_t>> src;
        QuotientBatch* h_batches = nullptr; QuotientEntry* h_entries = nullptr; size_t n_batches = 0, n_entries = 0;
    };
    struct QuotientRun { std::vector<QuotientGroup> groups; std::vector<DSecure> out; };
    std::vector<QuotientGroup> quotient_groups(const std::vector<DTree>& trees, const std::vector<std::vector<std::vector<u32>>>& mask);
    static void quotient_constants(QuotientGroup& g, const std::vector<PtQ>& points, const StarkProof* pf, Q31 random_coeff,
                                   std::vector<QuotientBatch>& batches, std::vector<QuotientEntry>& entries);
    QuotientRun compute_quotients(const std::vector<DTree>& trees, const std::vector<std::vector<std::vector<u32>>>& mask, const std::vector<PtQ>& points,
                                  const StarkProof* pf, Q31 random_coeff, std::vector<LevelWait>* q_waits, Mailbox* mb0 = nullptr, Mailbox* mb1 = nullptr);
    void quotients_fill(QuotientRun& qr, const std::vector<PtQ>& points, const StarkProof& pf, Q31 random_coeff, Mailbox* mb0, Mailbox* mb1);

    typedef std::function<void(const std::vector<u32>&)> Finisher;
    Finisher decommit(Gather& g, const DevMerkle& mk, const std::vector<DCol>& cols_in, const std::map<u32, std::vector<size_t>>& queries_per_log,
                      std::vector<u32>* queried_values, MerkleDecommitment* dec);
    static std::vector<size_t> fold_queries(const std::vector<size_t>& q, u32 n);
    static void positions_and_witness(const std::vector<size_t>& queries, std::vector<size_t>& positions, std::vector<size_t>& witness_pos);
    Finisher gather_secure_deferred(Gather& g, const DSecure& s, const std::vector<size_t>& pos, std::vector<Q31>* out);
    static std::vector<DCol> secure_cols(const DSecure& s);
    struct FriCommitted { struct Inner { DSecure ev; DevMerkle tree; }; DevMerkle first_tree; std::vector<DCol> first_cols; std::vector<Inner> inner; };
    FriCommitted fri_commit(std::vector<DSecure>& quotients, StarkProof& pf, const std::vector<LevelWait>& q_waits, const std::function<void()>& while_the_commit_phase_runs);
    void grind(StarkProof& pf);
    void decommit_queries(std::vector<DTree>& trees, const std::vector<DSecure>& quotients, const FriCommitted& fc, StarkProof& pf);
};

}
// ... 3 lines not shown
```

stwo-brainfuck_amd/csrc/prover.hip:

```cpp
#include <atomic>
#include "prover.h"
#include "host/verifier.h"
#include <algorithm>
#include <cstdio>
#include <mutex>
#include <thread>

namespace bf {

void HipProver::tap(const char* name) {
    if (!want_transcript) return;
    char buf[3]; transcript += name; transcript += ':';
    for (int i = 0; i < 32; i++) { snprintf(buf, sizeof buf, "%02x", ch.digest.b[i]); transcript += buf; }
    transcript += '\n';
}
void HipProver::print_marks() {
    if (!trace_host) return;
    if (trace_host_mean) {
        static std::mutex mu; static std::vector<std::pair<const char*, double>> sum; static int n = 0;
        std::lock_guard<std::mutex> g(mu);
        if (sum.size() != host_marks.size()) { sum.assign(host_marks.size(), {nullptr, 0.0}); n = 0; }
        double prev = 0;
        for (size_t i = 0; i < host_marks.size(); i++) { sum[i].first = host_marks[i].first; sum[i].second += host_marks[i].second - prev; prev = host_marks[i].second; }
        if (++n == 20) {
// ... 323 lines not shown
        tap("root3");
        tm.composition = now() - t0;
        t0 = now();
        draw_oods();
        sample_factors(points, sr.h_factors);
        mb_samples.post();
        mark("out-of-domain point posted");
        QuotientRun qr = compute_quotients(trees, mask, points, nullptr, q_one(), nullptr, &mb_quot0, &mb_quot1);
        BF_HIP(hipEventRecord(c.ev[5], c.stream));
        quotients = qr.out;
        mark("quotients enqueued behind their mailboxes");
        c.wait_stamp(4);
        sample_unpack(trees, mask, sample_results(), sample_plan.n_all, bp.proof);
        mark("sampled values arrived");
        mix_samples();
        tap("sampled");
        tm.oods = now() - t0;
        t0 = now();
        Q31 q_coeff = ch.draw_felt();
        mark("sampled values mixed, quotient coefficient drawn");
        quotients_fill(qr, points, bp.proof, q_coeff, &mb_quot0, &mb_quot1);
        mark("quotient constants posted");
    } else {
        if (!sharded()) {
            c.sync();
            mark("composition root arrived");
            trees[3].mk.root = *pinned_root3;
            ch.mix_root(trees[3].mk.root);
        }
        tap("root3");
        tm.composition = now() - t0;
        t0 = now();
        draw_oods();
        if (sharded()) sample_plan = sample_prepare(trees, mask);
        sample(trees, mask, points, bp.proof, sample_plan);
        mark("sampled values arrived");
        mix_samples();
        tap("sampled");
        tm.oods = now() - t0;

        t0 = now();
        Q31 q_coeff = ch.draw_felt();
        mark("sampled values mixed, quotient coefficient drawn");
        BF_HIP(hipEventRecord(c.ev[4], c.stream));
        quotients = compute_quotients(trees, mask, points, &bp.proof, q_coeff, &q_waits).out;
        BF_HIP(hipEventRecord(c.ev[5], c.stream));
        mark("quotients launched");
    }


    auto mailbox_gave_up = [&]() { for (int k = 1; k <= 5; k++) if (c.mailbox_err_host()[2 * k]) return true; return false; };
    const char* mailbox_msg = "a mailbox kernel gave up waiting for the host (BFHIP_MAILBOX_TIMEOUT_MS): the proof was computed from stale challenge words";
    auto sanity_check = [&]() {
        if (mb && mailbox_gave_up()) throw HipError(mailbox_msg);
        Q31 want = eval_composition_at_point(bp.log_sizes, bp.claimed_sums, log_max_rows, el, oods, bp.proof.sampled_values, random_coeff, c.conv);
        const auto& cv = bp.proof.sampled_values[3];
        std::vector<Q31> ce[4] = {cv[0], cv[1], cv[2], cv[3]};
        if (!q_eq(HostPointEval::combine(ce, 0), want)) throw HipError("ConstraintsNotSatisfied");
    };
    const FriCommitted fri = fri_commit(quotients, bp.proof, q_waits, sanity_check);
    grind(bp.proof);
    decommit_queries(trees, quotients, fri, bp.proof);
    for (int k = 1; k <= 5; k++) if (c.mailbox_err_host()[2 * k]) *c.mailbox_err_host() = c.mailbox_err_host()[2 * k];
    if (mb && trace_host) {
        static const char* const waited[5] = {"mailbox 1 waited for the host (GPU clock, 10 ns ticks):", "mailbox 2 waited", "mailbox 3 waited", "mailbox 4 waited", "mailbox 5 waited"};
        for (int k = 1; k <= 5; k++) host_marks.push_back({waited[k - 1], host_marks.back().second + c.mailbox_err_host()[2 * k + 1] * 0.01});
    }
    if (*c.mailbox_err_host()) throw HipError(mailbox_msg);
    {
        float ms0 = 0.f, ms1 = 0.f;
        if (!reuse) BF_HIP(hipEventElapsedTime(&ms0, c.ev[0], c.ev[1]));
        BF_HIP(hipEventElapsedTime(&ms1, c.ev[0], c.ev[2]));
        const double tot = (double)ms0 + (double)ms1;
        tm.preprocessed = tot > 0 ? wall_phase01 * ms0 / tot : 0.0;
        tm.main_trace = wall_phase01 - tm.preprocessed;
    }
    {
        float ms_q = 0.f;
        BF_HIP(hipEventElapsedTime(&ms_q, c.ev[4], c.ev[5]));
        tm.quotients = ms_q * 1e-3;
        tm.fri = (now() - t0) - tm.quotients;
    }

    c.last_proof_flags = (c.last_proof_flags & 48u) | (mb ? 1u : 0u) | (reuse && !shared ? 2u : 0u) | (shared ? 4u : 0u) | (replicate() ? 8u : 0u) | (preflight_ran ? 64u : 0u);
    tm.total = now() - t_start;
    mark("done");
    print_marks();
    return bp;
}

}

void bf::trace_columns(const bfhip_trace* t, const u32* cols[N_COMPONENTS][13], u32 log_sizes[N_COMPONENTS]) {
    for (int k = 0; k < N_COMPONENTS; k++) {
        log_sizes[k] = t->in.log_sizes[k];
        for (u32 j = 0; j < n_main_cols(k); j++) cols[k][j] = t->in.rows[k][j].ptr;
    }
}
```

stwo-brainfuck_amd/csrc/prover_commit.hip:

```cpp
#include "prover.h"
#include <algorithm>

namespace bf {

FftPlan HipProver::fft_prepare(bool inverse, const std::vector<DCol>& src, const std::vector<DCol>& dst) {
    std::map<std::pair<u32, u32>, std::vector<size_t>> groups;
    for (size_t i = 0; i < dst.size(); i++) groups[{dst[i].log_size, dst[i].shift}].push_back(i);
    struct Job { size_t off, n; u32 log, src_log, sh; };
    std::vector<Job> jobs; std::vector<const u32*> ptrs;
    for (auto it = groups.rbegin(); it != groups.rend(); ++it) {
        const auto& idx = it->second;
        u32 log = it->first.first, sh = it->first.second;
        std::map<u32, std::vector<size_t>> by_src;
        for (size_t i : idx) by_src[src[i].log_size].push_back(i);
        for (auto& kv : by_src) {
            jobs.push_back({ptrs.size(), kv.second.size(), log, kv.first, sh});
            for (size_t i : kv.second) ptrs.push_back(src[i].ptr);
            for (size_t i : kv.second) ptrs.push_back(dst[i].ptr);
        }
    }
    FftPlan plan;
    if (jobs.empty()) return plan;
    StageBatch sb(c);
    const u32* const* d_ptrs = c.stage(ptrs.data(), ptrs.size());
    std::vector<FftJob> fj;
    for (auto& j : jobs) fj.push_back({d_ptrs + j.off, (u32* const*)(d_ptrs + j.off + j.n), (u32)j.n, j.log - j.sh, j.src_log - j.sh, j.sh == 0});
    fft_plan(plan, inverse, fj.data(), fj.size(), c.d_tw, c.d_itw, c.tw_root_log);
    plan.d_groups = c.stage(plan.groups.data(), plan.groups.size());
    sb.end();
    return plan;
}
void HipProver::fft_launch(const FftPlan& plan) { fft_run(c.stream, plan); BF_HIP(hipGetLastError()); }
void HipProver::fft_cols(bool inverse, const std::vector<DCol>& src, const std::vector<DCol>& dst) {
    c.stage_checkpoint();
    fft_launch(fft_prepare(inverse, src, dst));
}

HipProver::MerklePlan HipProver::merkle_plan(const std::vector<DCol>& cols_in, bool folded_leaves) {
    if (cols_in.empty()) throw HipError("merkle_commit: no columns");
    MerklePlan p;
    p.cols = cols_in;
    std::vector<DCol>& cols = p.cols;
    std::stable_sort(cols.begin(), cols.end(), [](const DCol& a, const DCol& b) { return a.log_size > b.log_size; });
    DevMerkle& mk = p.mk;
    mk.cols = cols;
    mk.max_log = cols[0].log_size;
    mk.layers.resize(mk.max_log + 1);
    mk.shifts.assign(mk.max_log + 1, 0);
    u32 min_col_log = cols.back().log_size;
    std::vector<ColDesc> all; p.off.assign(mk.max_log + 2, 0); p.bytes.assign(mk.max_log + 1, 0.0);
    {
        size_t ci = 0;
        for (int log = (int)mk.max_log; log >= 0; log--) {
            p.off[log] = all.size();
            u32 sh = log < (int)mk.max_log ? (mk.shifts[log + 1] ? mk.shifts[log + 1] - 1 : 0) : 32;
            while (ci < cols.size() && cols[ci].log_size == (u32)log) { sh = std::min(sh, cols[ci].shift); p.bytes[log] += 4.0 * cols[ci].stored(); all.push_back(cols[ci++].desc()); }
            mk.shifts[log] = std::min<u32>(sh == 32 ? 0 : sh, (u32)log);
        }
    }
    p.n_all = all.size();
    p.poseidon = c.conv.merkle_channel == 1;
    (void)min_col_log;
    u32 fused_top = std::min<u32>(mk.max_log + 1, 10);
    while (fused_top > 0 && mk.shifts[std::min(fused_top, mk.max_log)] != 0) fused_top--;
    if (p.poseidon) fused_top = 0;
    p.fused_top = fused_top;
    const ShardGroup& sg = c.shard;
    if (sg.count > 1) {
        const int share_min = p.poseidon ? 8 : (int)SHARE_MIN_LOG_PER_RANK;
        int lo = std::max<int>((int)sg.log_count + share_min, (int)fused_top);
        while (lo <= (int)mk.max_log && (int)lo - (int)mk.shifts[lo] < (int)sg.log_count + share_min) lo++;
        const bool worth = (int)mk.max_log - (int)mk.shifts[mk.max_log] >= (int)sg.log_count + (int)SLICE_MIN_LOG_PER_RANK;
        if (worth && lo <= (int)mk.max_log) { mk.band_hi = (int)mk.max_log; mk.band_lo = lo; }
        for (auto& col : cols) if (col.sliced() && ((int)col.log_size < mk.band_lo || (int)col.log_size > mk.band_hi)) throw HipError("shard group: a row-sharded column lies outside the share-wise Merkle band");
    }
    const bool banded = mk.band_hi >= mk.band_lo;
    for (int log = (int)mk.max_log; log >= 0; log--) {
        const size_t stored = (size_t(1) << log) >> mk.shifts[log];
        if (banded && log > mk.band_lo && log <= mk.band_hi) {
            const size_t per_rank = stored >> sg.log_count;
            mk.layers[log] = reinterpret_cast<u32*>(reinterpret_cast<uintptr_t>(c.arena.alloc(32 * per_rank)) - 32 * per_rank * sg.rank);
        } else mk.layers[log] = (u32*)c.arena.alloc(32 * stored);
    }
    if (fused_top == 10 && mk.max_log >= 11) {
        u32 hi = std::min<u32>(banded ? (u32)mk.band_lo - 1 : mk.max_log, 17);
        if (folded_leaves && hi == mk.max_log) hi--;
        while (hi > 10 && mk.shifts[hi] != 0) hi--;
        if (hi > 10) { p.sub_hi = hi; p.fused_top = fused_top = MERKLE_SUBTREE_ROOT_LEVEL; }
    }
    auto level_cols = [&](int log) { return (log > 0 ? p.off[log - 1] : all.size()) - p.off[log]; };
    auto level_cost = [&](int log, double& bytes, double& comp) {
        const double nodes = (double)(1u << log), nc = (double)level_cols(log);
        const bool has = log < (int)mk.max_log;
        bytes += nodes * ((has ? 64.0 : 0.0) + 32.0) + p.bytes[log];
        comp += nodes * ((has ? 1.0 : 0.0) + (double)(((u32)nc + 15) / 16) + ((!has && nc == 0) ? 1.0 : 0.0));
    };
    if (banded && !p.poseidon && fused_top > 0 && mk.band_hi > mk.band_lo && c.shard.band_fusion) {
        const int hi = std::min(mk.band_hi, mk.band_lo + 3);
        bool plain = true;
        for (int lg = mk.band_lo; lg <= std::min(hi + 1, (int)mk.max_log); lg++) plain = plain && mk.shifts[lg] == 0;
        const u32 r = 8 - (u32)(hi - mk.band_lo);
        if (plain && (u32)mk.band_lo >= sg.log_count + r) {
            p.band_fuse_hi = hi; p.band_fuse_r = r;
            for (int lg = hi; lg >= mk.band_lo; lg--) level_cost(lg, p.band_bytes, p.band_comp);
            p.band_bytes /= sg.count; p.band_comp /= sg.count;
        }
    }
    for (int log = (int)fused_top - 1; log >= 0; log--) level_cost(log, p.top_bytes, p.top_comp);
    if (p.sub_hi) for (int log = (int)p.sub_hi; log >= (int)MERKLE_SUBTREE_ROOT_LEVEL; log--) level_cost(log, p.sub_bytes, p.sub_comp);
// ... 104 lines not shown
    std::vector<DCol> fsrc, fdst, full(n), fullprev(n);
    for (size_t i = 0; i < n; i++) {
        DCol e; e.log_size = t.polys[i].log_size + cfg.log_blowup; e.shift = t.polys[i].shift;
        if (t.owner[i] == OWNER_ALL) { e.ptr = c.alloc_u32(e.stored()); fsrc.push_back(t.polys[i]); fdst.push_back(e); }
        else if (replicate()) {
            e.ptr = c.alloc_u32(e.stored()); fsrc.push_back(t.polys[i]); fdst.push_back(e);
            e.lc = lc();
        } else {
            if (t.owner[i] == c.shard.rank) {
                full[i] = e; full[i].ptr = c.alloc_u32(e.stored()); fsrc.push_back(t.polys[i]); fdst.push_back(full[i]);
                if (with_prev && e.shift == 0) { fullprev[i] = e; fullprev[i].ptr = c.alloc_u32(e.stored()); }
            }
            e.lc = lc(); e.ptr = alloc_slice(e.log_size, e.shift);
            if (with_prev && e.shift == 0) { t.prev[i] = e; t.prev[i].ptr = alloc_slice(e.log_size); }
        }
        t.evals[i] = e;
    }
    auto exchange_columns = [&](hipStream_t comm_stream, const std::vector<size_t>& idx, hipEvent_t after_copies) {
        std::vector<Xfer> sends, recvs;
        for (size_t i : idx) {
            const u32 el = t.evals[i].log_size, sh = t.evals[i].shift;
            const size_t cells = slice_cells(el) >> sh, bytes = cells * sizeof(u32), first = slice_first(el) >> sh;
            const bool wp = with_prev && sh == 0;
            if (t.owner[i] == c.shard.rank) {
                if (wp) prev_row_copy(c.stream, fullprev[i].ptr, full[i].ptr, t.polys[i].log_size);
                for (u32 r = 0; r < c.shard.count; r++) {
                    sends.push_back({r, full[i].ptr + r * cells, bytes});
                    if (wp) sends.push_back({r, fullprev[i].ptr + r * cells, bytes});
                }
            }
            recvs.push_back({t.owner[i], t.evals[i].ptr + first, bytes});
            if (wp) recvs.push_back({t.owner[i], t.prev[i].ptr + first, bytes});
        }
        if (recvs.empty()) return;
        if (comm_stream != c.stream) { BF_HIP(hipEventRecord(after_copies, c.stream)); BF_HIP(hipStreamWaitEvent(comm_stream, after_copies, 0)); }
        c.shard.comm->exchange(comm_stream, sends, recvs);
    };
    std::vector<size_t> owned;
    u32 big = 0;
    for (size_t i = 0; i < n; i++) if (t.owner[i] != OWNER_ALL && !replicate()) { owned.push_back(i); big = std::max(big, t.evals[i].log_size); }
    std::vector<size_t> first_wave, second_wave;
    for (size_t i : owned) (t.evals[i].log_size == big ? first_wave : second_wave).push_back(i);
    if (sharded() && c.exchange_overlapped() && !second_wave.empty() && c.aux[0]) {
        std::vector<DCol> sa, da, sb2, db2;
        {
            size_t k = 0;
            for (size_t i = 0; i < n; i++) {
                const bool mine = t.owner[i] == OWNER_ALL || t.owner[i] == c.shard.rank;
                if (!mine) continue;
                const bool wave_a = t.owner[i] != OWNER_ALL && t.evals[i].log_size == big;
                (wave_a ? sa : sb2).push_back(fsrc[k]); (wave_a ? da : db2).push_back(fdst[k]);
                k++;
            }
        }
        c.stage_checkpoint();
        FftPlan pa = fft_prepare(false, sa, da), pb = fft_prepare(false, sb2, db2);
        try {
            fft_launch(pa);
            exchange_columns(c.aux[0], first_wave, c.next_event());
            fft_launch(pb);
            exchange_columns(c.aux[0], second_wave, c.next_event());
            hipEvent_t done = c.next_event();
            BF_HIP(hipEventRecord(done, c.aux[0]));
            BF_HIP(hipStreamWaitEvent(c.stream, done, 0));
        } catch (...) {
            (void)hipStreamSynchronize(c.aux[0]);
            throw;
        }
    } else {
        fft_cols(false, fsrc, fdst);
        if (sharded() && !replicate()) exchange_columns(c.stream, owned, nullptr);
    }
    BF_HIP(hipGetLastError());
    t.mk = merkle_commit(t.evals, pinned_root);
    if (!pinned_root) ch.mix_root(t.mk.root);
}

void HipProver::commit_tree_overlapped(DTree& t, Hash32* pinned_root, const std::vector<DCol>* interp_src, int stamp_slot) {
    const size_t n = t.polys.size();
    t.owner.assign(n, OWNER_ALL);
    t.evals.resize(n); t.prev.assign(n, DCol());
    u32 max_log = 0;
    for (size_t i = 0; i < n; i++) {
        DCol e; e.log_size = t.polys[i].log_size + cfg.log_blowup; e.shift = t.polys[i].shift; e.ptr = c.alloc_u32(e.stored());
        t.evals[i] = e; max_log = std::max(max_log, e.log_size);
    }
    std::vector<DCol> src[2], pol[2], ev[2];
    u32 next_log = 0;
    for (size_t i = 0; i < n; i++) {
        const int w = t.evals[i].log_size == max_log ? 0 : 1;
        if (interp_src) src[w].push_back((*interp_src)[i]);
        pol[w].push_back(t.polys[i]); ev[w].push_back(t.evals[i]);
        if (w) next_log = std::max(next_log, t.evals[i].log_size);
    }
    const bool overlap = (c.overlap & 1u) && !ev[1].empty() && max_log >= 19;
    c.stage_checkpoint();
    FftPlan fi[2], fe[2];
    MerklePlan mp;
    {
        StageBatch sb(c);
        for (int w = 0; w < 2; w++) {
            if (interp_src) fi[w] = fft_prepare(true, src[w], pol[w]);
            fe[w] = fft_prepare(false, pol[w], ev[w]);
        }
        mp = merkle_plan(t.evals);
        sb.end();
    }
    hipStream_t main = c.stream, aux = c.aux_of(main);
    if (interp_src) fft_launch(fi[0]);
    fft_launch(fe[0]);
    if (!overlap) {
        if (interp_src) fft_launch(fi[1]);
        fft_launch(fe[1]);
        bool stamped = false;
        t.mk = merkle_run(mp, pinned_root, false, nullptr, nullptr, stamp_slot, &stamped);
        if (stamp_slot >= 0 && !stamped) c.post_stamp(stamp_slot);
    } else {
        hipEvent_t e1 = c.next_event(), e2 = c.next_event(), e3 = c.next_event();
        BF_HIP(hipEventRecord(e1, main));
        if (interp_src) fft_launch(fi[1]);
        fft_launch(fe[1]);
        BF_HIP(hipEventRecord(e2, main));
        BF_HIP(hipStreamWaitEvent(aux, e1, 0));
        std::vector<LevelWait> waits = {{(int)next_log, e2}};
        c.stream = aux;
        try { t.mk = merkle_run(mp, nullptr, true, nullptr, &waits); } catch (...) { c.stream = main; (void)hipStreamSynchronize(aux); throw; }
        c.stream = main;
        BF_HIP(hipEventRecord(e3, aux));
        BF_HIP(hipStreamWaitEvent(main, e3, 0));
        if (pinned_root) BF_HIP(hipMemcpyAsync(pinned_root->b, t.mk.layers[0], 32, hipMemcpyDeviceToHost, main));
        else c.read_back(t.mk.root.b, t.mk.layers[0], 32);
        if (stamp_slot >= 0) c.post_stamp(stamp_slot);
    }
    if (!pinned_root) ch.mix_root(t.mk.root);
}

void HipProver::upload_trace(Ctx& c, const std::vector<Registers>& vm_trace, const std::vector<u32>& code, TraceInput& in, bool use_arena, bool on_gpu) {
    in.rows.assign(N_COMPONENTS, {});
    in.n_steps = vm_trace.size();
    in.main_cells = in.interaction_cells = 0;
    auto alloc = [&](size_t words) -> u32* {
        if (use_arena) return c.alloc_u32(words);
        u32* p = nullptr; BF_HIP(hipMalloc((void**)&p, (words ? words : 1) * sizeof(u32))); in.owned.push_back(p); return p;
    };
    if (on_gpu) {
        std::vector<u32> soa[7];
        size_t n = vm_trace.size();
        for (auto& v : soa) v.resize(n);
        for (size_t i = 0; i < n; i++) { const Registers& r = vm_trace[i]; soa[0][i] = r.clk; soa[1][i] = r.ip; soa[2][i] = r.ci; soa[3][i] = r.ni; soa[4][i] = r.mp; soa[5][i] = r.mv; soa[6][i] = r.mvi; }
        std::vector<std::vector<u32*>> cols;
        build_tables_device(c, soa, (u32)n, code, alloc, cols, in.log_sizes);
        for (int k = 0; k < N_COMPONENTS; k++)
            for (u32 j = 0; j < n_main_cols(k); j++) { DCol r; r.log_size = in.log_sizes[k]; r.shift = LOG_N_LANES; r.ptr = cols[k][j]; in.rows[k].push_back(r); }
    } else {
        std::vector<Table> tables = build_tables(vm_trace, code);
        for (int k = 0; k < N_COMPONENTS; k++) {
            in.log_sizes[k] = tables[k].log_size();
            for (u32 j = 0; j < n_main_cols(k); j++) {
                DCol r; r.log_size = in.log_sizes[k]; r.shift = LOG_N_LANES;
                r.ptr = alloc(r.stored());
                BF_HIP(hipMemcpyAsync(r.ptr, tables[k].cols[j].data(), r.stored() * sizeof(u32), hipMemcpyHostToDevice, c.stream));
                in.rows[k].push_back(r);
            }
        }
    }
    for (int k = 0; k < N_COMPONENTS; k++) {
        in.main_cells += (u64)n_main_cols(k) << in.log_sizes[k];
        in.interaction_cells += (u64)(4 * n_logup_cols(k)) << in.log_sizes[k];
    }
    c.sync();
}

void HipProver::upload_registers(Ctx& c, const u32* trace7_h, size_t n_rows, const u32* code_words_h, size_t n_code, TraceInput& in, bool use_arena, bool with_place) {
    auto bad_register = [&](size_t row, int reg) {
        std::string m = "register value is not a canonical M31";
        if (with_place) m += " (row " + std::to_string(row) + ", register " + std::to_string(reg) + ")";
        return HipError(m);
    };
    auto check_code = [&]() {
        std::vector<u32> ins(code_words_h, code_words_h + n_code);
        for (u32 w : ins) if (w >= P31) throw HipError("program word is not a canonical M31");
        return ins;
    };
    if (!c.tables_on_gpu) {
        std::vector<Registers> tr(n_rows);
        for (size_t i = 0; i < n_rows; i++) {
// ... 89 lines not shown
```

stwo-brainfuck_amd/csrc/prover_oods.hip:

```cpp
#include "prover.h"
#include <algorithm>

namespace bf {

HipProver::CompositionPlan HipProver::composition_prepare(std::vector<DTree>& trees, const BrainfuckProof& bp, const size_t* main_off, const size_t* inter_off, const Lookups& el) {
    CompositionPlan cp;
    for (int k = 0; k < N_COMPONENTS; k++) { cp.total += n_constraints(k); cp.max_log = std::max(cp.max_log, bp.log_sizes[k] + 1); }
    const bool own_domain = cfg.log_blowup != 1;
    std::vector<DCol> cd_src, cd_dst;
    auto on_constraint_domain = [&](const DCol& poly) {
        if (poly.sliced()) throw HipError("composition: a row-sharded polynomial on the constraint domain");
        DCol e; e.log_size = poly.log_size + 1; e.shift = poly.shift; e.ptr = c.alloc_u32(e.stored());
        cd_src.push_back(poly); cd_dst.push_back(e);
        return e;
    };
    cp.acc.resize(cp.max_log + 1); cp.have.assign(cp.max_log + 1, false); cp.launches.resize(N_COMPONENTS);
    for (int k = 0; k < N_COMPONENTS; k++) {
        u32 log = bp.log_sizes[k], eval_log = log + 1;
        const bool sl = slice_log(eval_log) && !replicate();
        if (!cp.have[eval_log]) {
            cp.acc[eval_log].log_size = eval_log; cp.acc[eval_log].lc = sl ? lc() : 0;
            for (int w = 0; w < 4; w++) cp.acc[eval_log].c[w] = sl ? alloc_slice(eval_log) : c.alloc_u32(size_t(1) << eval_log);
        }
        ConstraintLaunch L{};
        L.overwrite = cp.have[eval_log] ? 0u : 1u;
        cp.have[eval_log] = true;
        const u32 ni = 4 * n_logup_cols(k);
        if (!own_domain) {
            L.is_first = trees[0].evals[log_max_rows - log].ptr;
            for (u32 j = 0; j < n_main_cols(k); j++) L.trace[j] = trees[1].evals[main_off[k] + j].desc();
            for (u32 j = 0; j < ni; j++) L.inter[j] = trees[2].evals[inter_off[k] + j].desc();
        } else {
            const DCol& isf = trees[0].polys[log_max_rows - log];
            if (isf.shift != 0 || isf.log_size != log) throw HipError("composition: unexpected IsFirst polynomial layout");
            L.is_first = on_constraint_domain(isf).ptr;
            for (u32 j = 0; j < n_main_cols(k); j++) L.trace[j] = on_constraint_domain(trees[1].polys[main_off[k] + j]).desc();
            for (u32 j = 0; j < ni; j++) L.inter[j] = on_constraint_domain(trees[2].polys[inter_off[k] + j]).desc();
        }
        for (int w = 0; w < 4; w++) { const DCol& pv = trees[2].prev[inter_off[k] + ni - 4 + w]; L.inter_prev[w] = pv.ptr; }
        if (sl) { L.row0 = (u32)slice_first(eval_log); L.n_rows = (u32)slice_cells(eval_log); }
        for (int w = 0; w < 4; w++) L.acc[w] = cp.acc[eval_log].c[w];
        L.el = el; L.log_size = log;
        for (u32 i = 0; i < 2; i++) L.denom_inv[i] = m_inv(coset_vanishing_m(log, canonic_domain_at(eval_log, i)));
        cp.launches[k] = L;
    }
    if (own_domain) fft_cols(false, cd_src, cd_dst);
    return cp;
}
void HipProver::composition_challenge_fields(const BrainfuckProof& bp, u32 total, Q31 random_coeff, ConstraintLaunch* launches) {
    std::vector<Q31> powers(total);
    { Q31 cur = q_one(); for (u32 i = 0; i < total; i++) { powers[i] = cur; cur = q_mul(cur, random_coeff); } }
    u32 remaining = total;
    for (int k = 0; k < N_COMPONENTS; k++) {
        const u32 nc = n_constraints(k);
        for (u32 j = 0; j < nc; j++) launches[k].coeff[j] = powers[remaining - 1 - j];
        remaining -= nc;
        launches[k].total_sum = bp.claimed_sums[k];
    }
}
void HipProver::composition_fill(const BrainfuckProof& bp, CompositionPlan& cp, Q31 random_coeff) {
    if (!cp.h_staged) throw HipError("composition_fill without a staged launch table");
    composition_challenge_fields(bp, cp.total, random_coeff, cp.h_staged);
}
void HipProver::compute_composition(std::vector<DTree>& trees, const BrainfuckProof& bp, CompositionPlan& cp, Q31 random_coeff, Mailbox* mbx) {
    const u32 max_log = cp.max_log;
    std::vector<DSecure>& acc = cp.acc;
    std::vector<bool>& have = cp.have;
    std::vector<ConstraintLaunch>& launches = cp.launches;
    if (!mbx) composition_challenge_fields(bp, cp.total, random_coeff, launches.data());
    c.stage_checkpoint();
    {
        ConstraintBatch cb;
        constraint_batch_init(cb, launches.data(), N_COMPONENTS);
        const ConstraintLaunch* d_launches = nullptr; const ConstraintBatch* d_cb = nullptr;
        stage_blocks(mbx, [&] {
            d_launches = c.stage(launches.data(), launches.size());
            d_cb = c.stage(&cb, 1);
        });
        if (mbx) cp.h_staged = mbx->host(d_launches);
        eval_constraints_batch(c.stream, d_cb, cb, d_launches);
    }
    BF_HIP(hipGetLastError());
    if (!sharded() || replicate()) {
        std::vector<DCol> all_vals;
        std::vector<u32> logs;
        for (u32 log = max_log; log >= 1; log--) {
            if (!have[log]) continue;
            logs.push_back(log);
            for (int w = 0; w < 4; w++) { DCol v; v.ptr = acc[log].c[w]; v.log_size = log; v.shift = 0; all_vals.push_back(v); }
        }
        if (logs.size() > 13) throw HipError("composition: too many distinct sizes");
        fft_cols(true, all_vals, all_vals);
        AccumulateSizes as{};
        for (int w = 0; w < 4; w++) as.dst[w] = acc[logs[0]].c[w];
        for (size_t k = 1; k < logs.size(); k++) { for (int w = 0; w < 4; w++) as.src[k - 1][w] = acc[logs[k]].c[w]; as.log[k - 1] = logs[k]; }
        as.n = (u32)logs.size() - 1;
        accumulate_sizes(c.stream, as);
        BF_HIP(hipGetLastError());
        trees[3].polys.assign(all_vals.begin(), all_vals.begin() + 4);
        trees[3].owner.assign(4, OWNER_ALL);
        if (replicate() && slice_log(all_vals[0].log_size + cfg.log_blowup)) for (int w = 0; w < 4; w++) trees[3].owner[w] = (u32)w % c.shard.count;
        return;
    }
    bool cur_have = false; std::vector<DCol> cur(4);
    bool cur_owned = false;
    auto owner_of = [&](int w) { return (u32)w % c.shard.count; };
    for (u32 log = 1; log <= max_log; log++) {
        if (!have[log]) continue;
        std::vector<DCol> vals(4), mine_vals;
        const bool sl = acc[log].lc != 0;
        if (sl) {
            const size_t cells = slice_cells(log), bytes = cells * sizeof(u32), first = slice_first(log);
            std::vector<Xfer> sends, recvs;
            for (int w = 0; w < 4; w++) {
                vals[w].log_size = log; vals[w].shift = 0;
                sends.push_back({owner_of(w), acc[log].c[w] + first, bytes});
                if (owner_of(w) == c.shard.rank) {
                    vals[w].ptr = c.alloc_u32(size_t(1) << log);
                    for (u32 r = 0; r < c.shard.count; r++) recvs.push_back({r, vals[w].ptr + r * cells, bytes});
                    mine_vals.push_back(vals[w]);
                }
            }
            std::stable_sort(recvs.begin(), recvs.end(), [](const Xfer& a, const Xfer& b) { return a.peer < b.peer; });
            c.shard.comm->exchange(c.stream, sends, recvs);
        } else {
            if (cur_owned) throw HipError("composition: a replicated accumulator above a row-sharded one");
            for (int w = 0; w < 4; w++) { vals[w].ptr = acc[log].c[w]; vals[w].log_size = log; vals[w].shift = 0; mine_vals.push_back(vals[w]); }
        }
        fft_cols(true, mine_vals, mine_vals);
        if (cur_have)
            for (int w = 0; w < 4; w++) if (!sl || owner_of(w) == c.shard.rank) accumulate(c.stream, vals[w].ptr, cur[w].ptr, 1u << cur[w].log_size);
        cur = vals; cur_have = true; cur_owned = sl;
    }
    trees[3].polys = cur;
    trees[3].owner.assign(4, OWNER_ALL);
    if (cur_owned || (sharded() && slice_log(cur[0].log_size + cfg.log_blowup))) for (int w = 0; w < 4; w++) trees[3].owner[w] = owner_of(w);
}

HipProver::SamplePlan HipProver::sample_prepare(const std::vector<DTree>& trees, const std::vector<std::vector<std::vector<u32>>>& mask) {
    SamplePlan sp;
    for (size_t t = 0; t < trees.size(); t++)
        for (size_t col = 0; col < trees[t].polys.size(); col++)
            for (u32 pt : mask[t][col]) {
                const u32 ji = sp.n_all++;
                const u32 owner = trees[t].owner.empty() ? OWNER_ALL : trees[t].owner[col];
                if (sharded() && ((owner == OWNER_ALL || replicate()) ? ji % c.shard.count : owner) != c.shard.rank) continue;
                const DCol& p = trees[t].polys[col];
                EvalJob j{}; j.coeffs = p.ptr; j.log_n = p.log_size - p.shift; j.point = pt; j.factor_shift = p.shift; j.partial_off = sp.partial_off; j.out_idx = ji;
                sp.partial_off += j.log_n > 12 ? 1u << (j.log_n - 12) : 1u;
                sp.jobs.push_back(j);
            }
    return sp;
}
void HipProver::sample_factors(const std::vector<PtQ>& points, uint4* factors) {
    for (size_t p = 0; p < points.size(); p++) {
        Q31 x = points[p].x;
        auto pk = [](Q31 q) { return make_uint4(q.a.a, q.a.b, q.b.a, q.b.b); };
        factors[p * 32 + 0] = pk(points[p].y);
        for (u32 b = 1; b < 32; b++) { factors[p * 32 + b] = pk(x); x = q_double_x(x); }
    }
}
HipProver::SampleRun HipProver::sample_launch(const SamplePlan& sp, const std::vector<PtQ>& points, Mailbox* mbx) {
    SampleRun sr;
    const bool pinned = !sharded() && sp.n_all * sizeof(uint4) <= c.h_small_bytes - 4096;
    if (mbx && !pinned) throw HipError("sampling: too many samples for the pinned result buffer");
    std::vector<uint4> factors(points.size() * 32, make_uint4(0, 0, 0, 0));
    if (!mbx) sample_factors(points, factors.data());
    c.stage_checkpoint();
    const uint4* d_factors = nullptr; const EvalJob* d_jobs = nullptr;
    stage_blocks(mbx, [&] {
        d_factors = c.stage(factors.data(), factors.size());
        d_jobs = sp.jobs.empty() ? nullptr : c.stage(sp.jobs.data(), sp.jobs.size());
    });
    if (mbx) sr.h_factors = mbx->host(d_factors);
    void* d_partials = c.arena.alloc(size_t(sp.partial_off ? sp.partial_off : 1) * sizeof(uint4));
    if (!pinned) {
        sr.d_out = (uint4*)c.arena.alloc(sp.n_all * sizeof(uint4));
        if (sharded()) BF_HIP(hipMemsetAsync(sr.d_out, 0, sp.n_all * sizeof(uint4), c.stream));
    }
    eval_at_points(c.stream, d_jobs, (u32)sp.jobs.size(), sp.partial_off, d_factors, d_partials, pinned ? (void*)(c.d_small_alias + 4096) : sr.d_out);
// ... 128 lines not shown
```

Measured before the change: 14.54 billion.

## Fuse inverse FFT last layers with forward LDE first layers in a seam kernel

Adds a K_SEAM FFT kernel that, at the boundary between the inverse transform and the blowup-1 forward extension, takes coefficients held in shared memory and writes both the coefficients and the first forward layers of the LDE. It also folds the composition polynomial's cross-size accumulation into that kernel. The aim is to skip a full global-memory round trip and separate accumulate launches in commit and composition. The cost is a larger, more complex kernel with heavy shared-memory and register use, and new plan and pointer plumbing that applies only when the prover is unsharded with log_blowup 1.

Result: no change. 14.63 billion, median of 6 (+0.6%).

```diff
diff --git a/bindings/rust/bfhip_sys.rs b/bindings/rust/bfhip_sys.rs
--- a/bindings/rust/bfhip_sys.rs
+++ b/bindings/rust/bfhip_sys.rs
@@ -41,6 +41,9 @@
     pub fn bfhip_twiddles(ctx: *mut BfhipCtx, tw_d: *mut *const u32, itw_d: *mut *const u32, root_log: *mut u32) -> i32;
     pub fn bfhip_interpolate(ctx: *mut BfhipCtx, src_cols_h: *const *mut u32, dst_cols_h: *const *mut u32, n_cols: u32, log_size: u32, replicated: i32) -> i32;
     pub fn bfhip_evaluate(ctx: *mut BfhipCtx, coeff_cols_h: *const *mut u32, dst_cols_h: *const *mut u32, n_cols: u32, log_size: u32, log_eval: u32, replicated: i32) -> i32;
+    pub fn bfhip_interpolate_extend(ctx: *mut BfhipCtx, eval_cols_h: *const *mut u32, coeff_cols_h: *const *mut u32, lde_cols_h: *const *mut u32, n_cols: u32, log_size: u32, log_eval: u32, add_cols_h: *const *const u32, add_log_sizes: *const u32, n_add: u32) -> i32;
+    pub fn bfhip_fft_seam_map(log_size: u32, tw_root_log: u32, workgroup: u32, coeff_rows: *mut u32, lde_rows: *mut u32, tw_inverse: *mut u32, tw_forward: *mut u32) -> i32;
+    pub fn bfhip_fft_seam_plan(log_size: u32, log_eval: u32, launches: *mut u32, capacity: u32, n_launches: *mut u32) -> i32;
     pub fn bfhip_is_first_coeffs(ctx: *mut BfhipCtx, log_min: u32, log_max: u32, dst_cols_h: *const *mut u32) -> i32;
     pub fn bfhip_broadcast16(ctx: *mut BfhipCtx, rows_d: *const u32, dst_d: *mut u32, n_rows: usize) -> i32;
     pub fn bfhip_bit_reverse(ctx: *mut BfhipCtx, src_d: *const u32, dst_d: *mut u32, log_size: u32) -> i32;
diff --git a/include/bfhip.h b/include/bfhip.h
--- a/include/bfhip.h
+++ b/include/bfhip.h
@@ -58,6 +58,10 @@
 
 int32_t bfhip_interpolate(bfhip_ctx* ctx, uint32_t* const* src_cols_h, uint32_t* const* dst_cols_h, uint32_t n_cols, uint32_t log_size, int32_t replicated);
 int32_t bfhip_evaluate(bfhip_ctx* ctx, uint32_t* const* coeff_cols_h, uint32_t* const* dst_cols_h, uint32_t n_cols, uint32_t log_size, uint32_t log_eval, int32_t replicated);
+int32_t bfhip_interpolate_extend(bfhip_ctx* ctx, uint32_t* const* eval_cols_h, uint32_t* const* coeff_cols_h, uint32_t* const* lde_cols_h, uint32_t n_cols, uint32_t log_size,
+                                 uint32_t log_eval, const uint32_t* const* add_cols_h, const uint32_t* add_log_sizes, uint32_t n_add);
+int32_t bfhip_fft_seam_map(uint32_t log_size, uint32_t tw_root_log, uint32_t workgroup, uint32_t* coeff_rows, uint32_t* lde_rows, uint32_t* tw_inverse, uint32_t* tw_forward);
+int32_t bfhip_fft_seam_plan(uint32_t log_size, uint32_t log_eval, uint32_t* launches, uint32_t capacity, uint32_t* n_launches);
 
 int32_t bfhip_is_first_coeffs(bfhip_ctx* ctx, uint32_t log_min, uint32_t log_max, uint32_t* const* dst_cols_h);
 
diff --git a/stwo-brainfuck_amd/__init__.py b/stwo-brainfuck_amd/__init__.py
--- a/stwo-brainfuck_amd/__init__.py
+++ b/stwo-brainfuck_amd/__init__.py
@@ -335,7 +335,7 @@
         f = ctypes.c_uint32()
         _check(lib().bfhip_ctx_last_proof_flags(self._h, ctypes.byref(f)))
         return {"mailbox_order": bool(f.value & 1), "kept_preprocessed": bool(f.value & 2), "shared_preprocessed": bool(f.value & 4), "replicated_transforms": bool(f.value & 8),
-                "split_gather": bool(f.value & 16), "fri_fold_leaf": bool(f.value & 32), "preflight": bool(f.value & 64)}
+                "split_gather": bool(f.value & 16), "fri_fold_leaf": bool(f.value & 32), "preflight": bool(f.value & 64), "fft_seam": bool(f.value & 128)}
 
     def set_preflight(self, on=True):
         _check(lib().bfhip_ctx_set_preflight(self._h, 1 if on else 0))
@@ -442,6 +442,14 @@
 
     def evaluate(self, coeff_ptrs, dst_ptrs, log_size, log_eval, replicated=False):
         _check(lib().bfhip_evaluate(self._h, self._ptr_array(coeff_ptrs), self._ptr_array(dst_ptrs), len(coeff_ptrs), log_size, log_eval, int(replicated)))
+
+    def interpolate_extend(self, eval_ptrs, coeff_ptrs, lde_ptrs, log_size, log_eval, add_ptrs=(), add_log_sizes=()):
+        n, n_add = len(eval_ptrs), len(add_log_sizes)
+        if len(coeff_ptrs) != n or len(lde_ptrs) != n or len(add_ptrs) != n_add or any(len(a) != n for a in add_ptrs): raise ValueError("interpolate_extend: column lists of different lengths")
+        flat = [p for a in add_ptrs for p in a]
+        logs = (ctypes.c_uint32 * max(n_add, 1))(*[int(v) for v in add_log_sizes])
+        _check(lib().bfhip_interpolate_extend(self._h, self._ptr_array(eval_ptrs), self._ptr_array(coeff_ptrs), self._ptr_array(lde_ptrs), n, log_size, log_eval,
+                                              self._ptr_array(flat) if n_add else None, logs if n_add else None, n_add))
 
     def is_first_coeffs(self, log_min, log_max, dst_ptrs):
         arr = (ctypes.c_void_p * len(dst_ptrs))(*[p or None for p in dst_ptrs])
@@ -797,6 +805,20 @@
     return rc == 0, err.value.decode()
 
 
+def fft_seam_map(log_size, tw_root_log, workgroup):
+    cr, lr, ti, tf = np.empty(128, np.uint32), np.empty(256, np.uint32), np.empty(127, np.uint32), np.empty(254, np.uint32)
+    ptr = lambda a: a.ctypes.data_as(ctypes.c_void_p)
+    _check(lib().bfhip_fft_seam_map(int(log_size), int(tw_root_log), int(workgroup), ptr(cr), ptr(lr), ptr(ti), ptr(tf)))
+    return {"coeff_rows": cr, "lde_rows": lr.reshape(2, 128), "tw_inverse": ti, "tw_forward": tf.reshape(2, 127)}
+
+
+def fft_seam_plan(log_size, log_eval):
+    out, n = np.zeros(5 * 32, np.uint32), ctypes.c_uint32()
+    _check(lib().bfhip_fft_seam_plan(int(log_size), int(log_eval), out.ctypes.data_as(ctypes.c_void_p), 32, ctypes.byref(n)))
+    if n.value > 32: raise BfhipError("fft_seam_plan: more than 32 launches")
+    return [{"inverse": bool(r[0]), "kind": int(r[1]), "lo": int(r[2]), "k": int(r[3]), "seam": bool(r[4])} for r in out.reshape(32, 5)[: n.value]]
+
+
 def host_compile(code):
     out = np.zeros(2 * len(code) + 4, dtype=np.uint32)
     n = ctypes.c_size_t()
diff --git a/stwo-brainfuck_amd/csrc/api.hip b/stwo-brainfuck_amd/csrc/api.hip
--- a/stwo-brainfuck_amd/csrc/api.hip
+++ b/stwo-brainfuck_amd/csrc/api.hip
@@ -521,6 +521,82 @@
     API_CATCH
 }
 
+int32_t bfhip_interpolate_extend(bfhip_ctx* ctx, uint32_t* const* eval_cols_h, uint32_t* const* coeff_cols_h, uint32_t* const* lde_cols_h, uint32_t n_cols, uint32_t log_size,
+                                 uint32_t log_eval, const uint32_t* const* add_cols_h, const uint32_t* add_log_sizes, uint32_t n_add) {
+    API_CTX(ctx)
+    Ctx& c = ctx->c;
+    if (!eval_cols_h || !coeff_cols_h || !lde_cols_h || (n_add && (!add_cols_h || !add_log_sizes))) throw HipError("null argument");
+    if (log_size < 3) throw HipError("circle transforms need log_size >= 3");
+    if (log_eval < log_size) throw HipError("log_eval < log_size");
+    if (log_eval > c.tw_root_log + 1) throw HipError("log_eval exceeds the context's twiddle tree");
+    if (n_add > 12) throw HipError("at most 12 added coefficient arrays");
+    for (u32 s = 0; s < n_add; s++)
+        if (add_log_sizes[s] >= log_size || add_log_sizes[s] < 2 || (s && add_log_sizes[s] >= add_log_sizes[s - 1])) throw HipError("added coefficient arrays must be smaller than the columns, in strictly descending sizes");
+    if (n_cols == 0) return 0;
+    const bool seam = fft_seam_covers(log_size, log_eval, true);
+    c.stage_checkpoint();
+    StageBatch sb(c);
+    auto* s = c.stage(eval_cols_h, n_cols);
+    auto* d = c.stage(coeff_cols_h, n_cols);
+    auto* e = c.stage(lde_cols_h, n_cols);
+    FftJob inv{(const u32* const*)s, (u32* const*)d, n_cols, log_size, log_size, true};
+    FftJob fwd{(const u32* const*)d, (u32* const*)e, n_cols, log_eval, log_size, true};
+    if (seam) {
+        inv.d_lde = (u32* const*)e; inv.n_add = n_add; inv.add_external = true;
+        if (n_add) inv.d_add = (const u32* const*)c.stage(add_cols_h, (size_t)n_add * n_cols);
+        for (u32 k = 0; k < n_add; k++) inv.add_log[k] = add_log_sizes[k];
+        fwd.seam_done = true;
+    }
+    FftPlan pi, pf;
+    fft_plan(pi, true, &inv, 1, c.d_tw, c.d_itw, c.tw_root_log);
+    fft_plan(pf, false, &fwd, 1, c.d_tw, c.d_itw, c.tw_root_log);
+    pi.d_groups = c.stage(pi.groups.data(), pi.groups.size());
+    pf.d_groups = c.stage(pf.groups.data(), pf.groups.size());
+    sb.end();
+    fft_run(c.stream, pi);
+    if (!seam)
+        for (u32 k = 0; k < n_add; k++)
+            for (u32 col = 0; col < n_cols; col++) accumulate(c.stream, coeff_cols_h[col], add_cols_h[(size_t)k * n_cols + col], 1u << add_log_sizes[k]);
+    fft_run(c.stream, pf);
+    BF_HIP(hipGetLastError());
+    return 0;
+    API_CATCH
+}
+
+int32_t bfhip_fft_seam_map(uint32_t log_size, uint32_t tw_root_log, uint32_t workgroup, uint32_t* coeff_rows, uint32_t* lde_rows, uint32_t* tw_inverse, uint32_t* tw_forward) {
+    API_TRY
+    if (!coeff_rows || !lde_rows || !tw_inverse || !tw_forward) throw HipError("null argument");
+    if (!fft_seam_covers(log_size, log_size + 1, true) || tw_root_log + 1 < log_size + 1 || tw_root_log > 30) throw HipError("the seam does not cover this size");
+    if (workgroup >= (1u << (log_size - 13))) throw HipError("workgroup out of range");
+    for (u32 m = 0; m < 128; m++) { coeff_rows[m] = seam_row_cell(log_size, workgroup, 0, m); for (u32 H = 0; H < 2; H++) lde_rows[128 * H + m] = seam_row_cell(log_size, workgroup, H, m); }
+    for (u32 i = 0; i < 127; i++) { tw_inverse[i] = seam_tw_index(1u << tw_root_log, 0, i); for (u32 H = 0; H < 2; H++) tw_forward[127 * H + i] = seam_tw_index(1u << tw_root_log, 1 + H, i); }
+    return 0;
+    API_CATCH
+}
+int32_t bfhip_fft_seam_plan(uint32_t log_size, uint32_t log_eval, uint32_t* launches, uint32_t capacity, uint32_t* n_launches) {
+    API_TRY
+    if (!launches || !n_launches) throw HipError("null argument");
+    if (log_size < 6 || log_eval < log_size || log_eval > 30) throw HipError("unsupported sizes");
+    const u32* const* fake = reinterpret_cast<const u32* const*>(uintptr_t(4096));
+    u32* const* fake_lde = reinterpret_cast<u32* const*>(uintptr_t(8192));
+    const bool seam = fft_seam_covers(log_size, log_eval, true);
+    FftJob inv{fake, (u32* const*)fake, 1, log_size, log_size, true}, fwd{fake, fake_lde, 1, log_eval, log_size, true};
+    if (seam) { inv.d_lde = fake_lde; fwd.seam_done = true; }
+    u32 n = 0;
+    for (int dir = 0; dir < 2; dir++) {
+        FftPlan plan;
+        fft_plan(plan, dir == 0, dir == 0 ? &inv : &fwd, 1, nullptr, nullptr, log_eval - 1);
+        for (const FftLaunch& L : plan.launches)
+            for (u32 g = 0; g < L.ngroups; g++) {
+                const PassArgs& a = plan.groups[L.first_group + g];
+                if (n < capacity) { u32* o = launches + 5 * n; o[0] = dir == 0; o[1] = (u32)L.kind; o[2] = a.lo; o[3] = a.k; o[4] = a.dst2 != nullptr; }
+                n++;
+            }
+    }
+    *n_launches = n;
+    return 0;
+    API_CATCH
+}
 
 int32_t bfhip_is_first_coeffs(bfhip_ctx* ctx, uint32_t log_min, uint32_t log_max, uint32_t* const* dst_cols_h) {
     API_CTX(ctx)
diff --git a/stwo-brainfuck_amd/csrc/fft.hip b/stwo-brainfuck_amd/csrc/fft.hip
--- a/stwo-brainfuck_amd/csrc/fft.hip
+++ b/stwo-brainfuck_amd/csrc/fft.hip
@@ -67,7 +67,7 @@
     hipLaunchKernelGGL(k_is_first_coeffs, dim3((lanes + 255) / 256), dim3(256), 0, stream, a, itw, 1u << tw_root_log);
 }
 
-enum { K_TILE12 = 0, K_STRIDED5 = 1, K_STRIDED6 = 2, K_PASS = 3, K_TINY = 4, K_STRIDED_K8 = 5, K_STRIDED_K9 = 6, K_STRIDED_K10 = 7, K_KINDS = 8 };
+enum { K_TILE12 = 0, K_STRIDED5 = 1, K_STRIDED6 = 2, K_PASS = 3, K_TINY = 4, K_STRIDED_K8 = 5, K_STRIDED_K9 = 6, K_STRIDED_K10 = 7, K_SEAM = 8, K_KINDS = 9 };
 struct BlockOfGroup { u32 g, tile, by; };
 template <bool INV> __device__ __forceinline__ void fft_tiny_body(const PassArgs& a, const BlockOfGroup& bg);
 __device__ __forceinline__ BlockOfGroup find_group(const PassArgs* __restrict__ groups, u32 ngroups) {
@@ -405,6 +405,134 @@
     }
 }
 
+template <int CL>
+__global__ void __launch_bounds__(4 << CL, 3) k_fft_seam(const PassArgs* __restrict__ groups, u32 ngroups) {
+    const BlockOfGroup bg = find_group(groups, ngroups);
+    const PassArgs a = groups[bg.g];
+    constexpr u32 C = 1u << CL, NT = 4u << CL;
+    __shared__ __attribute__((aligned(16))) u32 s_val[128 * C];
+    __shared__ u32 s_tw[3 * 128];
+    __shared__ u32 s_lane[NT];
+    const u32 lo = a.lo;
+    s_lane[threadIdx.x] = threadIdx.x;
+    u32 t = threadIdx.x;
+    static_assert(CL == 6, "kernels.h seam_row_cell: 64-cell rows");
+    const u32 base = seam_row_cell(a.log, bg.tile, 0, 0);
+    for (u32 e = t; e < 3 * 128; e += NT) {
+        const u32 set = e >> 7, i = e & 127u;
+        if (i == 127u) continue;
+        s_tw[e] = 2u * (set == 0 ? a.tw : a.tw2)[seam_tw_index(a.tw_total, set, i)];
+    }
+    const u32 col0 = bg.by * a.cols_per_block, col1 = min(a.ncols, col0 + a.cols_per_block);
+    const u32 sk = scale_shift(a.scale);
+    const unsigned char* __restrict__ add_log = groups[bg.g].add_log;
+    const bool adds = a.nadd != 0 && base < (1u << add_log[0]);
+    for (u32 col = col0; col < col1; col++) {
+        g_cu32p src = as_global(a.src[col]);
+        g_u32p dst = as_global(a.dst[col]);
+        g_u32p lde = as_global(a.dst2[col]);
+        __syncthreads();
+        t = s_lane[threadIdx.x];
+        const u32 l4 = 4 * (t & (C / 4 - 1)), r4 = t >> (CL - 2);
+        u32 as0[8], as1[8];
+#pragma unroll
+        for (int e = 0; e < 8; e++) as0[e] = as1[e] = 0;
+        u32 r[8][4];
+#pragma unroll
+        for (int q = 0; q < 8; q++) { uint4 v = ld16_stream(src + (base | ((8 * r4 + q) << lo) | l4)); r[q][0] = v.x; r[q][1] = v.y; r[q][2] = v.z; r[q][3] = v.w; }
+        if (adds) {
+            const u32 l = t & (C - 1), mlow = t >> CL, nadd = a.nadd;
+            auto cell = [&](u32 g, int e) -> u32 { return base | ((8 * e + mlow + 4 * g) << lo) | l; };
+            u32 x0[4][8], x1[4][8];
+#pragma unroll
+            for (int s = 0; s < 4; s++) {
+                const bool on = (u32)s < nadd;
+                const u32 n_s = on ? 1u << add_log[on ? s : 0] : 0u;
+                g_cu32p ap = as_global(a.add[(on ? s : 0) * a.ncols + col]);
+#pragma unroll
+                for (int e = 0; e < (8 >> s); e++) { x0[s][e] = cell(0, e) < n_s ? ap[cell(0, e)] : 0u; x1[s][e] = cell(1, e) < n_s ? ap[cell(1, e)] : 0u; }
+            }
+#pragma unroll
+            for (int s = 0; s < 4; s++)
+#pragma unroll
+                for (int e = 0; e < (8 >> s); e++) { as0[e] = m_add(as0[e], x0[s][e]); as1[e] = m_add(as1[e], x1[s][e]); }
+            for (u32 s = 4; s < nadd; s++) {
+                const u32 n_s = 1u << add_log[s];
+                if (base >= n_s) break;
+                g_cu32p ap = as_global(a.add[s * a.ncols + col]);
+                if (cell(0, 0) < n_s) as0[0] = m_add(as0[0], ap[cell(0, 0)]);
+                if (cell(1, 0) < n_s) as1[0] = m_add(as1[0], ap[cell(1, 0)]);
+            }
+        }
+        {
+#pragma unroll
+            for (int jl = 0; jl < 3; jl++)
+#pragma unroll
+                for (int b = 0; b < 4; b++) {
+                    const int q0 = ((b >> jl) << (jl + 1)) | (b & ((1 << jl) - 1));
+                    const u32 w = s_tw[128u - (128u >> jl) + ((8 * r4 + q0) >> (jl + 1))];
+#pragma unroll
+                    for (int j = 0; j < 4; j++) bfly<true>(r[q0][j], r[q0 | (1 << jl)][j], w);
+                }
+#pragma unroll
+            for (int q = 0; q < 8; q++) *reinterpret_cast<uint4*>(&s_val[C * (8 * r4 + q) + l4]) = make_uint4(r[q][0], r[q][1], r[q][2], r[q][3]);
+        }
+        __syncthreads();
+        u32 cf0[16], cf1[16];
+        auto coeffs = [&](u32 id, u32 (&v)[16], const u32 (&as)[8]) {
+            const u32 l = id & (C - 1), mlow = id >> CL;
+#pragma unroll
+            for (int e = 0; e < 16; e++) v[e] = s_val[C * (8 * e + mlow) + l];
+            radix16<true>(v, 4, [&](int jl, int pe) -> u32 { return s_tw[128u - (128u >> (3 + jl)) + pe]; });
+#pragma unroll
+            for (int e = 0; e < 16; e++) v[e] = m_mul_pow2(v[e], sk);
+            if (adds) {
+#pragma unroll
+                for (int e = 0; e < 8; e++) v[e] = m_add(v[e], as[e]);
+            }
+#pragma unroll
+            for (int e = 0; e < 16; e++) __builtin_nontemporal_store(v[e], dst + (base | ((8 * e + mlow) << lo) | l));
+        };
+        coeffs(t, cf0, as0);
+        __builtin_amdgcn_sched_barrier(0);
+        coeffs(t + NT, cf1, as1);
+#pragma unroll 1
+        for (u32 H = 0; H < 2; H++) {
+            const u32* __restrict__ tw = s_tw + 128 * (1 + H);
+            if (H) __syncthreads();
+            auto narrow_fwd = [&](u32 id, const u32 (&cf)[16]) {
+                const u32 l = id & (C - 1), mlow = id >> CL;
+                u32 v[16];
+#pragma unroll
+                for (int e = 0; e < 16; e++) v[e] = cf[e];
+                radix16<false>(v, 4, [&](int jl, int pe) -> u32 { return tw[128u - (128u >> (3 + jl)) + pe]; });
+#pragma unroll
+                for (int e = 0; e < 16; e++) s_val[C * (8 * e + mlow) + l] = v[e];
+            };
+            narrow_fwd(t, cf0);
+            __builtin_amdgcn_sched_barrier(0);
+            narrow_fwd(t + NT, cf1);
+            __builtin_amdgcn_sched_barrier(0);
+            __syncthreads();
+            u32 r[8][4];
+#pragma unroll
+            for (int q = 0; q < 8; q++) { uint4 v = *reinterpret_cast<uint4*>(&s_val[C * (8 * r4 + q) + l4]); r[q][0] = v.x; r[q][1] = v.y; r[q][2] = v.z; r[q][3] = v.w; }
+#pragma unroll
+            for (int jl = 2; jl >= 0; jl--)
+#pragma unroll
+                for (int b = 0; b < 4; b++) {
+                    const int q0 = ((b >> jl) << (jl + 1)) | (b & ((1 << jl) - 1));
+                    const u32 w = tw[128u - (128u >> jl) + ((8 * r4 + q0) >> (jl + 1))];
+#pragma unroll
+                    for (int j = 0; j < 4; j++) bfly<false>(r[q0][j], r[q0 | (1 << jl)][j], w);
+                }
+            const u32 obase = seam_row_cell(a.log, bg.tile, H, 0);
+#pragma unroll
+            for (int q = 0; q < 8; q++) st16(lde + (obase | ((8 * r4 + q) << lo) | l4), make_uint4(r[q][0], r[q][1], r[q][2], r[q][3]));
+        }
+    }
+}
+
 template <bool INV, class TW> __device__ __forceinline__ void radix16_range(u32 (&v)[16], int jl_lo, TW tw) {
 #pragma unroll
     for (int s = 0; s < 4; s++) {
@@ -521,7 +649,8 @@
 
 void fft_plan(FftPlan& plan, bool inverse, const FftJob* jobs, size_t njobs, const u32* tw, const u32* itw, u32 tw_root_log) {
     plan.inverse = inverse; plan.groups.clear(); plan.launches.clear(); plan.d_groups = nullptr;
-    struct Item { int pi, kind; PassArgs a; double bytes, alg; bool single = false; double bfly() const { return 0.5 * a.ncols * (double)(1u << a.log) * a.k; } };
+    struct Item { int pi, kind; PassArgs a; double bytes, alg; bool single = false; double bfly_fwd = 0.0;
+                  double bfly() const { return 0.5 * a.ncols * (double)(1u << a.log) * a.k + bfly_fwd; } };
     std::vector<Item> items;
     int max_np = 0;
     for (size_t ji = 0; ji < njobs; ji++) {
@@ -531,6 +660,9 @@
         PassArgs a{};
         a.ncols = ncols; a.log = log; a.circle = job.circle ? 1 : 0; a.tw = inverse ? itw : tw; a.tw_total = 1u << tw_root_log; a.scale = 1;
         const u32 nl = inverse ? log : (log > 5 && src_log < 2) ? 2u : src_log;
+        const bool seam = inverse && job.d_lde != nullptr;
+        if (seam && (!fft_seam_covers(log, log + 1, job.circle) || log + 1 > tw_root_log + 1 || job.n_add > 12)) throw std::runtime_error("fft_plan: the seam does not cover this job");
+        if (job.seam_done && (inverse || !fft_seam_covers(src_log, log, job.circle))) throw std::runtime_error("fft_plan: seam_done on a job the seam does not cover");
         if (log <= 5) {
             a.dst = job.d_dst; a.src = job.d_src; a.src_mask = (1u << src_log) - 1; a.lo = 0; a.k = nl;
             a.scale = inverse ? m_inv(1u << log) : 1;
@@ -551,6 +683,7 @@
             for (int pi = 0; pi < np; pi++) {
                 int p = inverse ? pi : np - 1 - pi;
                 bool first = pi == 0, last = pi == np - 1;
+                if (job.seam_done && first) continue;
                 a.src = first ? job.d_src : (const u32* const*)job.d_dst;
                 a.dst = job.d_dst;
                 a.src_mask = first ? ((1u << src_log) - 1) : 0xffffffffu;
@@ -565,6 +698,20 @@
                     a.lo = 0; a.k = k0; a.tile_log = 12; a.grid_x = ntiles;
                     PassArgs b = a; b.block0 = gy;
                     items.push_back({pi, K_TILE12, b, bytes, alg});
+                } else if (seam && last) {
+                    a.lo = k0 + 7 * (p - 1); a.k = 7;
+                    if (np != 3 || a.lo + 7 != log) throw std::runtime_error("fft_plan: the seam needs a three-pass plan");
+                    PassArgs b = a; b.grid_x = ntiles / 2; b.block0 = gy;
+                    b.dst2 = job.d_lde; b.tw2 = tw; b.add = job.d_add; b.nadd = job.n_add;
+                    double add_cells = 0.0;
+                    for (u32 s = 0; s < job.n_add; s++) {
+                        if (job.add_log[s] >= log || job.add_log[s] < 2 || (s && job.add_log[s] >= job.add_log[s - 1])) throw std::runtime_error("fft_plan: added sources must be smaller than the job, in descending sizes");
+                        b.add_log[s] = (unsigned char)job.add_log[s]; add_cells += (double)(1u << job.add_log[s]);
+                    }
+                    const double n_cells = (double)(1u << log);
+                    Item it{pi, K_SEAM, b, 4.0 * ncols * (4.0 * n_cells + add_cells), alg + 4.0 * ncols * (3.0 * n_cells) / np};
+                    it.bfly_fwd = 0.5 * ncols * 2.0 * n_cells * 7;
+                    items.push_back(it);
                 } else if (big_k) {
                     a.lo = 12; a.k = big_k;
                     const u32 cl = big_k == 10 ? 4 : 5;
@@ -619,6 +766,21 @@
         if (fuse && host_pi >= 0)
             for (auto& it : items)
                 if (it.single && (it.kind == K_PASS || it.kind == K_TINY)) { it.a.kind = (u32)it.kind; it.kind = K_TILE12; it.pi = host_pi; }
+    }
+    for (size_t ji = 0; ji < njobs; ji++) {
+        const FftJob& job = jobs[ji];
+        if (!inverse || !job.d_lde || !job.n_add || job.ncols == 0) continue;
+        int seam_pi = -1;
+        for (auto& it : items) if (it.kind == K_SEAM && it.a.dst2 == job.d_lde) seam_pi = it.pi;
+        for (u32 s = 0; s < job.n_add; s++) {
+            bool found = job.add_external;
+            for (auto& it : items) {
+                if (it.a.log != job.add_log[s] || !it.a.circle || it.a.dst == job.d_dst) continue;
+                found = true;
+                if (it.kind == K_SEAM || it.pi > seam_pi) throw std::runtime_error("fft_plan: an added source's transform would not precede the seam launch");
+            }
+            if (!found) throw std::runtime_error("fft_plan: an added source is not a job of this plan");
+        }
     }
     for (int pi = 0; pi < max_np; pi++)
         for (int kind = 0; kind < K_KINDS; kind++) {
@@ -684,6 +846,11 @@
                 if (inverse) hipLaunchKernelGGL((k_fft_stridedK<true, 10, 4>), grid, dim3(512), 0, stream, g, L.ngroups);
                 else hipLaunchKernelGGL((k_fft_stridedK<false, 10, 4>), grid, dim3(512), 0, stream, g, L.ngroups);
                 break; }
+            case K_SEAM: {
+                if (!inverse) throw std::runtime_error("fft_run: a seam launch in a forward plan");
+                ProfScope ps(stream, fft_prof_name("k_fft_seam", L), L.bytes, L.alg, false, L.bfly);
+                hipLaunchKernelGGL((k_fft_seam<6>), grid, dim3(256), 0, stream, g, L.ngroups);
+                break; }
             case K_PASS: {
                 ProfScope ps(stream, fft_prof_name(inverse ? "k_fft_pass<true>" : "k_fft_pass<false>", L), L.bytes, L.alg, false, L.bfly);
                 if (inverse) hipLaunchKernelGGL(k_fft_pass<true>, grid, dim3(FFT_THREADS), 0, stream, g, L.ngroups);
diff --git a/stwo-brainfuck_amd/csrc/kernels.h b/stwo-brainfuck_amd/csrc/kernels.h
--- a/stwo-brainfuck_amd/csrc/kernels.h
+++ b/stwo-brainfuck_amd/csrc/kernels.h
@@ -56,7 +56,18 @@
 #endif
 
 void gen_twiddles(hipStream_t stream, u32* d_tw, u32* d_itw, u32 R, const uint2* d_tlo, const uint2* d_thi);
-struct FftJob { const u32* const* d_src; u32* const* d_dst; u32 ncols, log, src_log; bool circle; };
+struct FftJob {
+    const u32* const* d_src; u32* const* d_dst; u32 ncols, log, src_log; bool circle;
+    u32* const* d_lde = nullptr; const u32* const* d_add = nullptr; u32 n_add = 0; u32 add_log[12] = {}; bool add_external = false;
+    bool seam_done = false;
+};
+inline bool fft_seam_covers(u32 log, u32 log_ext, bool circle) { return circle && log >= 23 && log <= 25 && log_ext == log + 1; }
+BF_HD u32 seam_row_cell(u32 log, u32 wg, u32 H, u32 m) { return (H << log) | (m << (log - 7)) | (wg << 6); }
+BF_HD u32 seam_tw_index(u32 tw_total, u32 set, u32 i) {
+    u32 j = 0; while (j < 6 && i >= 128u - (128u >> (j + 1))) j++;
+    const u32 q = i - (128u - (128u >> j));
+    return set == 0 ? tw_total - (2u << (6 - j)) + q : tw_total - (2u << (7 - j)) + ((set - 1) << (6 - j)) + q;
+}
 struct PassArgs {
     u32* const* dst;
     const u32* const* src;
@@ -71,6 +82,7 @@
     const u32* tw;
     u32 block0, grid_x;
     u32 kind;
+    u32* const* dst2; const u32* tw2; const u32* const* add; u32 nadd; unsigned char add_log[12];
 };
 struct FftLaunch { int kind; u32 first_group, ngroups, total_blocks; double bytes, alg, bfly; };
 struct FftPlan { bool inverse = false; std::vector<PassArgs> groups; std::vector<FftLaunch> launches; const PassArgs* d_groups = nullptr; };
diff --git a/stwo-brainfuck_amd/csrc/prover.h b/stwo-brainfuck_amd/csrc/prover.h
--- a/stwo-brainfuck_amd/csrc/prover.h
+++ b/stwo-brainfuck_amd/csrc/prover.h
@@ -28,7 +28,8 @@
     bool mine(u64 cell, u32 rank) const { return lc == 0 || (cell >> (log_size - lc)) == rank; }
 };
 struct DevMerkle { std::vector<u32*> layers; std::vector<u32> shifts; u32 max_log = 0; Hash32 root; int band_lo = 0, band_hi = -1; std::vector<DCol> cols; };
-struct DTree { std::vector<DCol> polys, evals, prev; std::vector<u32> owner; DevMerkle mk; };
+struct DTree { std::vector<DCol> polys, evals, prev; std::vector<u32> owner; DevMerkle mk;
+               bool seamed = false; };
 struct DSecure {
     u32* c[4]; u32 log_size; u32 lc = 0;
     bool mine(u64 cell, u32 rank) const { return lc == 0 || (cell >> (log_size - lc)) == rank; }
@@ -126,7 +127,11 @@
     BrainfuckProof prove(const std::function<const TraceInput&()>& get_input);
     void preflight(const TraceInput& in);
 
-    FftPlan fft_prepare(bool inverse, const std::vector<DCol>& src, const std::vector<DCol>& dst);
+    struct SeamAdds { u32 log = 0; std::vector<u32> add_log; std::vector<const u32*> ptrs; };
+    struct SeamSpec { const std::vector<DCol>* lde = nullptr; const SeamAdds* adds = nullptr; bool done = false; };
+    bool fft_seam_col(const DCol& poly) const;
+    FftPlan fft_prepare(bool inverse, const std::vector<DCol>& src, const std::vector<DCol>& dst, const SeamSpec& seam);
+    FftPlan fft_prepare(bool inverse, const std::vector<DCol>& src, const std::vector<DCol>& dst) { SeamSpec none; return fft_prepare(inverse, src, dst, none); }
     void fft_launch(const FftPlan& plan);
     void fft_cols(bool inverse, const std::vector<DCol>& src, const std::vector<DCol>& dst);
     template <class F> void stage_blocks(Mailbox* mbx, F&& f) {
diff --git a/stwo-brainfuck_amd/csrc/prover.hip b/stwo-brainfuck_amd/csrc/prover.hip
--- a/stwo-brainfuck_amd/csrc/prover.hip
+++ b/stwo-brainfuck_amd/csrc/prover.hip
@@ -429,7 +429,7 @@
         tm.fri = (now() - t0) - tm.quotients;
     }
 
-    c.last_proof_flags = (c.last_proof_flags & 48u) | (mb ? 1u : 0u) | (reuse && !shared ? 2u : 0u) | (shared ? 4u : 0u) | (replicate() ? 8u : 0u) | (preflight_ran ? 64u : 0u);
+    c.last_proof_flags = (c.last_proof_flags & 176u) | (mb ? 1u : 0u) | (reuse && !shared ? 2u : 0u) | (shared ? 4u : 0u) | (replicate() ? 8u : 0u) | (preflight_ran ? 64u : 0u);
     tm.total = now() - t_start;
     mark("done");
     print_marks();
diff --git a/stwo-brainfuck_amd/csrc/prover_commit.hip b/stwo-brainfuck_amd/csrc/prover_commit.hip
--- a/stwo-brainfuck_amd/csrc/prover_commit.hip
+++ b/stwo-brainfuck_amd/csrc/prover_commit.hip
@@ -3,10 +3,17 @@
 
 namespace bf {
 
-FftPlan HipProver::fft_prepare(bool inverse, const std::vector<DCol>& src, const std::vector<DCol>& dst) {
+#ifndef BF_FFT_SEAM
+#define BF_FFT_SEAM 1
+#endif
+bool HipProver::fft_seam_col(const DCol& poly) const {
+    return BF_FFT_SEAM && !sharded() && cfg.log_blowup == 1 && poly.shift == 0 && !poly.sliced() && fft_seam_covers(poly.log_size, poly.log_size + cfg.log_blowup, true);
+}
+FftPlan HipProver::fft_prepare(bool inverse, const std::vector<DCol>& src, const std::vector<DCol>& dst, const SeamSpec& seam) {
     std::map<std::pair<u32, u32>, std::vector<size_t>> groups;
     for (size_t i = 0; i < dst.size(); i++) groups[{dst[i].log_size, dst[i].shift}].push_back(i);
-    struct Job { size_t off, n; u32 log, src_log, sh; };
+    struct Job { size_t off, n; u32 log, src_log, sh; bool seam = false; size_t lde_off = 0, add_off = 0; };
+    if (seam.lde && (!inverse || seam.lde->size() != dst.size())) throw HipError("fft_prepare: the seam's LDE columns do not match the plan");
     std::vector<Job> jobs; std::vector<const u32*> ptrs;
     for (auto it = groups.rbegin(); it != groups.rend(); ++it) {
         const auto& idx = it->second;
@@ -17,6 +24,23 @@
             jobs.push_back({ptrs.size(), kv.second.size(), log, kv.first, sh});
             for (size_t i : kv.second) ptrs.push_back(src[i].ptr);
             for (size_t i : kv.second) ptrs.push_back(dst[i].ptr);
+            const size_t i0 = kv.second[0];
+            if (inverse ? (seam.lde && (*seam.lde)[i0].ptr && kv.first == log && fft_seam_col(dst[i0])) : (seam.done && fft_seam_col(src[i0]) && log == kv.first + cfg.log_blowup)) {
+                Job& j = jobs.back(); j.seam = true;
+                if (inverse) {
+                    j.lde_off = ptrs.size();
+                    for (size_t i : kv.second) {
+                        const DCol& e = (*seam.lde)[i];
+                        if (e.log_size != log + 1 || e.shift != 0 || !e.ptr) throw HipError("fft_prepare: a seam column's LDE storage has the wrong shape");
+                        ptrs.push_back(e.ptr);
+                    }
+                    if (seam.adds && seam.adds->log == log && !seam.adds->add_log.empty()) {
+                        if (seam.adds->ptrs.size() != seam.adds->add_log.size() * j.n) throw HipError("fft_prepare: the seam's added sources do not match its columns");
+                        j.add_off = ptrs.size();
+                        ptrs.insert(ptrs.end(), seam.adds->ptrs.begin(), seam.adds->ptrs.end());
+                    }
+                }
+            }
         }
     }
     FftPlan plan;
@@ -24,7 +48,15 @@
     StageBatch sb(c);
     const u32* const* d_ptrs = c.stage(ptrs.data(), ptrs.size());
     std::vector<FftJob> fj;
-    for (auto& j : jobs) fj.push_back({d_ptrs + j.off, (u32* const*)(d_ptrs + j.off + j.n), (u32)j.n, j.log - j.sh, j.src_log - j.sh, j.sh == 0});
+    for (auto& j : jobs) {
+        FftJob f{d_ptrs + j.off, (u32* const*)(d_ptrs + j.off + j.n), (u32)j.n, j.log - j.sh, j.src_log - j.sh, j.sh == 0};
+        if (j.seam && inverse) {
+            f.d_lde = (u32* const*)(d_ptrs + j.lde_off);
+            if (j.add_off) { f.d_add = d_ptrs + j.add_off; f.n_add = (u32)seam.adds->add_log.size(); for (u32 s = 0; s < f.n_add; s++) f.add_log[s] = seam.adds->add_log[s]; }
+            c.last_proof_flags |= 128u;
+        } else if (j.seam) f.seam_done = true;
+        fj.push_back(f);
+    }
     fft_plan(plan, inverse, fj.data(), fj.size(), c.d_tw, c.d_itw, c.tw_root_log);
     plan.d_groups = c.stage(plan.groups.data(), plan.groups.size());
     sb.end();
@@ -295,7 +327,9 @@
     t.evals.resize(n); t.prev.assign(n, DCol());
     u32 max_log = 0;
     for (size_t i = 0; i < n; i++) {
-        DCol e; e.log_size = t.polys[i].log_size + cfg.log_blowup; e.shift = t.polys[i].shift; e.ptr = c.alloc_u32(e.stored());
+        DCol e; e.log_size = t.polys[i].log_size + cfg.log_blowup; e.shift = t.polys[i].shift;
+        if (t.seamed) { if (t.evals[i].log_size != e.log_size || t.evals[i].shift != e.shift || !t.evals[i].ptr) throw HipError("commit: a seamed tree without its LDE storage"); e.ptr = t.evals[i].ptr; }
+        else e.ptr = c.alloc_u32(e.stored());
         t.evals[i] = e; max_log = std::max(max_log, e.log_size);
     }
     std::vector<DCol> src[2], pol[2], ev[2];
@@ -313,8 +347,10 @@
     {
         StageBatch sb(c);
         for (int w = 0; w < 2; w++) {
-            if (interp_src) fi[w] = fft_prepare(true, src[w], pol[w]);
-            fe[w] = fft_prepare(false, pol[w], ev[w]);
+            SeamSpec si, se;
+            si.lde = &ev[w]; se.done = interp_src != nullptr || t.seamed;
+            if (interp_src) fi[w] = fft_prepare(true, src[w], pol[w], si);
+            fe[w] = fft_prepare(false, pol[w], ev[w], se);
         }
         mp = merkle_plan(t.evals);
         sb.end();
diff --git a/stwo-brainfuck_amd/csrc/prover_oods.hip b/stwo-brainfuck_amd/csrc/prover_oods.hip
--- a/stwo-brainfuck_amd/csrc/prover_oods.hip
+++ b/stwo-brainfuck_amd/csrc/prover_oods.hip
@@ -90,12 +90,24 @@
             for (int w = 0; w < 4; w++) { DCol v; v.ptr = acc[log].c[w]; v.log_size = log; v.shift = 0; all_vals.push_back(v); }
         }
         if (logs.size() > 13) throw HipError("composition: too many distinct sizes");
-        fft_cols(true, all_vals, all_vals);
-        AccumulateSizes as{};
-        for (int w = 0; w < 4; w++) as.dst[w] = acc[logs[0]].c[w];
-        for (size_t k = 1; k < logs.size(); k++) { for (int w = 0; w < 4; w++) as.src[k - 1][w] = acc[logs[k]].c[w]; as.log[k - 1] = logs[k]; }
-        as.n = (u32)logs.size() - 1;
-        accumulate_sizes(c.stream, as);
+        if (fft_seam_col(all_vals[0])) {
+            std::vector<DCol> lde(all_vals.size());
+            SeamAdds adds; adds.log = logs[0];
+            for (int w = 0; w < 4; w++) { DCol e; e.log_size = logs[0] + cfg.log_blowup; e.shift = 0; e.ptr = c.alloc_u32(e.stored()); lde[w] = e; }
+            for (size_t k = 1; k < logs.size(); k++) { adds.add_log.push_back(logs[k]); for (int w = 0; w < 4; w++) adds.ptrs.push_back(acc[logs[k]].c[w]); }
+            SeamSpec ss; ss.lde = &lde; ss.adds = &adds;
+            c.stage_checkpoint();
+            fft_launch(fft_prepare(true, all_vals, all_vals, ss));
+            trees[3].evals.assign(lde.begin(), lde.begin() + 4);
+            trees[3].seamed = true;
+        } else {
+            fft_cols(true, all_vals, all_vals);
+            AccumulateSizes as{};
+            for (int w = 0; w < 4; w++) as.dst[w] = acc[logs[0]].c[w];
+            for (size_t k = 1; k < logs.size(); k++) { for (int w = 0; w < 4; w++) as.src[k - 1][w] = acc[logs[k]].c[w]; as.log[k - 1] = logs[k]; }
+            as.n = (u32)logs.size() - 1;
+            accumulate_sizes(c.stream, as);
+        }
         BF_HIP(hipGetLastError());
         trees[3].polys.assign(all_vals.begin(), all_vals.begin() + 4);
         trees[3].owner.assign(4, OWNER_ALL);
```
